# Alexander-H-Liu/End-to-end-ASR-Pytorch

Measured on AMD Instinct MI355X. Metric: audio frames/sec training (LAS+CTC, LibriSpeech 80-mel), higher is better.
Workload: dtype f32; 1 GPU; cfg3: {"B": 32, "T": 1600, "D": 80, "V": 5000, "L": 64}; global_batch=32, parallelism=dp1

## Files before the change

end-to-end-asr-pytorch_amd/_lib.py:

```python
import ctypes
import os

_HERE = os.path.dirname(os.path.abspath(__file__))
LIB_PATH = os.path.join(_HERE, "csrc", "libasrk.so")

c_int, c_i64, c_f32, c_vp, c_sz = (ctypes.c_int, ctypes.c_int64, ctypes.c_float, ctypes.c_void_p,
                                   ctypes.c_size_t)
c_f64 = ctypes.c_double

SIGNATURES = {
    "asrk_version": (c_int, []),
    "asrk_strerror": (ctypes.c_char_p, [c_int]),
    "asrk_init": (c_int, [c_int]),
    "asrk_profile_enable": (None, [c_int]),
    "asrk_profile_families": (None, [ctypes.c_uint]),
    "asrk_profile_reset": (None, []),
    "asrk_profile_get": (c_int, [c_int, ctypes.POINTER(ctypes.c_double), ctypes.POINTER(c_i64)]),
    "asrk_profile_get_work": (c_int, [c_int, ctypes.POINTER(ctypes.c_double)]),
    "asrk_gemm_f32": (c_int, [c_int, c_int, c_int, c_int, c_int, c_f32, c_vp, c_int, c_vp, c_int,
                              c_f32, c_vp, c_int, c_vp, c_vp, c_int, c_int, c_vp, c_sz, c_vp]),
    "asrk_gemm_ws_bytes": (c_sz, [c_int, c_int, c_int, c_int]),
    "asrk_gemm_takes_split": (c_int, [c_int, c_int, c_int, c_int]),
    "asrk_split_panel_bytes": (ctypes.c_size_t, [c_int, c_int, c_int]),
    "asrk_split_panel_f32": (c_int, [c_vp, c_int, c_int, c_int, c_int, c_vp, c_int, c_vp]),
    "asrk_gemm_panels_f32": (c_int, [c_int, c_int, c_int, c_f32, c_vp, c_int, c_int, c_int, c_int,
                                     c_vp, c_int, c_int, c_int, c_int, c_f32, c_vp, c_int, c_vp, c_vp, c_int, c_vp]),
    "asrk_gemm_panels_splitk_ws_bytes": (c_sz, [c_int, c_int, c_int]),
    "asrk_gemm_panels_splitk_f32": (c_int, [c_int, c_int, c_int, c_f32, c_vp, c_int, c_int, c_int, c_int,
                                            c_vp, c_int, c_int, c_int, c_int, c_f32, c_vp, c_int, c_vp, c_vp, c_int,
                                            c_vp, c_sz, c_int, c_vp]),
    "asrk_copy3d_f32": (c_int, [c_vp, c_vp, c_int, c_int, c_int, c_i64, c_i64, c_i64, c_i64, c_int,
                                c_vp]),
    "asrk_colsum_f32": (c_int, [c_vp, c_int, c_int, c_int, c_vp, c_int, c_vp]),
    "asrk_tanh_fwd_f32": (c_int, [c_vp, c_vp, c_i64, c_vp]),
    "asrk_tanh_bwd_f32": (c_int, [c_vp, c_vp, c_vp, c_i64, c_vp]),
    "asrk_log_softmax_fwd_f32": (c_int, [c_vp, c_vp, c_int, c_int, c_int, c_vp]),
    "asrk_log_softmax_bwd_f32": (c_int, [c_vp, c_vp, c_vp, c_int, c_int, c_int, c_vp]),
    "asrk_cross_entropy_fwd_f32": (c_int, [c_vp, c_int, c_int, c_int, c_vp, c_int, c_vp, c_vp, c_vp]),
    "asrk_cross_entropy_bwd_f32": (c_int, [c_vp, c_int, c_int, c_int, c_vp, c_int, c_vp, c_vp, c_vp,
                                           c_vp]),
    "asrk_ctc_prefix_score_f32": (c_int, [c_vp, c_vp, c_vp, c_vp, c_vp, c_vp, c_vp, c_int, c_int, c_int,
                                          c_int, c_int, c_int, c_f32, c_vp]),
    "asrk_ctc_prefix_score_multi_f32": (c_int, [c_vp, c_vp, c_vp, c_vp, c_vp, c_vp, c_vp, c_vp, c_vp, c_int, c_int,
                                                c_int, c_int, c_int, c_int, c_int, c_f32, c_vp]),
    "asrk_ctc_prefix_beam_ws_bytes": (c_sz, [c_int, c_int]),
    "asrk_ctc_prefix_beam_ws_offsets": (c_int, [c_int, c_int, c_int] + [ctypes.POINTER(c_i64)] * 6),
    "asrk_ctc_prefix_beam_f32": (c_int, [c_vp, c_int, c_int, c_vp, c_int, c_int, c_vp, c_f32, c_int, c_int, c_int,
                                         c_int, c_int, c_vp, c_sz, c_vp]),
    "asrk_ctc_prefix_beam_multi_ws_bytes": (c_sz, [c_int, c_int, c_int, ctypes.POINTER(c_sz)]),
    "asrk_ctc_prefix_beam_multi_f32": (c_int, [c_vp, c_i64, c_int, c_int, c_int, c_vp, c_int, c_int, c_vp, c_f32,
                                               c_vp, c_vp, c_int, c_vp, c_vp, c_vp, c_vp, c_sz, c_vp]),
    "asrk_fbank_frames_f32": (c_int, [c_vp, c_i64, c_vp, c_vp, c_int, c_int, c_int, c_int, c_f32, c_int,
                                      c_vp]),
    "asrk_power_spectrum_f32": (c_int, [c_vp, c_vp, c_i64, c_int, c_vp]),
    "asrk_log_floor_f32": (c_int, [c_vp, c_i64, c_f32, c_vp]),
    "asrk_delta_f32": (c_int, [c_vp, c_vp, c_vp, c_int, c_int, c_int, c_int, c_vp]),
    "asrk_cmvn_f32": (c_int, [c_vp, c_vp, c_int, c_int, c_f32, c_vp]),
    "asrk_transpose_f32": (c_int, [c_vp, c_vp, c_int, c_int, c_vp]),
    "asrk_fbank_frames_batch_f32": (c_int, [c_vp, c_int, c_i64, c_vp, c_vp, c_int, c_int, c_vp, c_vp, c_int, c_int,
                                            c_int, c_f32, c_f32, c_int, c_vp]),
    "asrk_delta_cmvn_batch_f32": (c_int, [c_vp, c_vp, c_int, c_int, c_vp, c_int, c_int, c_int, c_f32, c_vp, c_int,
                                          c_vp]),
    "asrk_fbank_logmel_batch_f32": (c_int, [c_vp, c_int, c_i64, c_vp, c_vp, c_int, c_int, c_vp, c_vp, c_vp, c_vp, c_vp,
                                            c_int, c_int, c_vp, c_int, c_int, c_int, c_f32, c_f32, c_int, c_f32, c_vp]),
    "asrk_spec_augment_f32": (c_int, [c_vp, c_vp, c_int, c_int, c_int, c_int, c_int, c_vp, c_vp, c_int, c_int, c_f32,
                                      c_vp]),
    "asrk_lstm_ws_bytes": (c_sz, []),
    "asrk_lstm_xchg_bytes": (c_sz, [c_int, c_int, c_int, c_int, c_int, c_int]),
    "asrk_lstm_plan_workgroups": (c_int, [c_int, c_int, c_int, c_int, c_int, c_int]),
    "asrk_lstm_rec_fwd_f32": (c_int, [c_vp, c_vp, c_vp, c_vp, c_vp, c_int, c_int, c_int, c_int,
                                      c_vp, c_int, c_vp, c_int, c_vp]),
    "asrk_lstm_rec_bwd_f32": (c_int, [c_vp, c_vp, c_vp, c_vp, c_vp, c_int, c_int, c_int, c_int,
                                      c_vp, c_int, c_vp, c_vp, c_int, c_vp]),
    "asrk_lstm_rec_fwd_pyr_f32": (c_int, [c_vp, c_vp, c_vp, c_vp, c_vp, c_int, c_int, c_int, c_int,
                                          c_vp, c_int, c_vp, c_vp, c_int, c_int, c_int, c_vp]),
    "asrk_lstm_rec_fwd_len_f32": (c_int, [c_vp, c_vp, c_vp, c_vp, c_vp, c_vp, c_int, c_int, c_int, c_int,
                                          c_vp, c_int, c_vp, c_vp, c_int, c_int, c_int, c_vp]),
    "asrk_lstm_rec_bwd_pyr_f32": (c_int, [c_vp, c_vp, c_vp, c_vp, c_vp, c_int, c_int, c_int, c_int,
                                          c_vp, c_int, c_vp, c_vp, c_int, c_int, c_int, c_vp]),
    "asrk_lstm_plan_is_bf": (c_int, [c_int, c_int, c_int, c_int, c_int, c_int]),
    "asrk_lstm_rec_fwd_pyr_panel_f32": (c_int, [c_vp, c_vp, c_vp, c_vp, c_vp, c_int, c_int, c_int, c_int,
                                                c_vp, c_int, c_vp, c_vp, c_int, c_int, c_vp, c_int, c_vp]),
    "asrk_lstm_rec_bwd_pyr_panel_f32": (c_int, [c_vp, c_vp, c_vp, c_vp, c_vp, c_int, c_int, c_int, c_int,
                                                c_vp, c_int, c_vp, c_vp, c_int, c_int, c_vp, c_vp, c_int, c_vp]),
    "asrk_gru_rec_fwd_f32": (c_int, [c_vp, c_vp, c_vp, c_vp, c_int, c_int, c_int, c_int,
                                     c_vp, c_int, c_vp, c_vp, c_int, c_int, c_int, c_vp]),
    "asrk_gru_rec_bwd_f32": (c_int, [c_vp, c_vp, c_vp, c_vp, c_vp, c_int, c_int, c_int, c_int,
                                     c_vp, c_int, c_vp, c_vp, c_int, c_int, c_int, c_vp]),
    "asrk_lstm_check_error": (c_int, [c_vp, c_vp]),
    "asrk_loc_conv_fwd_f32": (c_int, [c_vp, c_vp, c_vp, c_int, c_int, c_int, c_int, c_int, c_vp]),
    "asrk_loc_conv_bwd_f32": (c_int, [c_vp, c_vp, c_vp, c_vp, c_vp, c_int, c_int, c_int, c_int, c_int,
                                      c_vp]),
    "asrk_attn_energy_fwd_f32": (c_int, [c_int, c_vp, c_vp, c_vp, c_vp, c_vp, c_vp, c_vp, c_vp, c_vp,
                                         c_int, c_int, c_int, c_int, c_int, c_f32, c_vp]),
    "asrk_attn_energy_bwd_f32": (c_int, [c_int, c_vp, c_vp, c_vp, c_vp, c_vp, c_vp, c_vp, c_vp, c_vp,
                                         c_vp, c_vp, c_vp, c_vp, c_vp, c_int, c_int, c_int, c_int,
                                         c_int, c_f32, c_vp]),
    "asrk_attn_context_fwd_f32": (c_int, [c_vp, c_vp, c_vp, c_int, c_int, c_int, c_i64, c_vp]),
    "asrk_attn_context_bwd_f32": (c_int, [c_vp, c_vp, c_vp, c_int, c_int, c_int, c_i64, c_vp]),
    "asrk_lstm_cell_fwd_f32": (c_int, [c_vp, c_vp, c_vp, c_vp, c_int, c_int, c_vp]),
    "asrk_lstm_cell_bwd_f32": (c_int, [c_vp, c_vp, c_vp, c_vp, c_vp, c_vp, c_int, c_int, c_vp]),
    "asrk_gru_cell_fwd_f32": (c_int, [c_vp, c_vp, c_i64, c_i64, c_vp, c_i64, c_vp, c_i64, c_int, c_int, c_vp]),
    "asrk_gru_cell_bwd_f32": (c_int, [c_vp, c_vp, c_i64, c_i64, c_vp, c_i64, c_vp, c_i64, c_vp, c_vp, c_i64,
                                      c_int, c_int, c_vp]),
    "asrk_embedding_fwd_f32": (c_int, [c_vp, c_vp, c_vp, c_i64, c_int, c_int, c_vp]),
    "asrk_embedding_bwd_f32": (c_int, [c_vp, c_vp, c_vp, c_i64, c_int, c_int, c_vp]),
    "asrk_layer_norm_fwd_f32": (c_int, [c_vp, c_vp, c_vp, c_vp, c_vp, c_vp, c_int, c_int, c_f32, c_vp]),
    "asrk_layer_norm_bwd_f32": (c_int, [c_vp, c_vp, c_vp, c_vp, c_vp, c_vp, c_vp, c_vp, c_int, c_int,
                                        c_vp]),
    "asrk_dropout_f32": (c_int, [c_vp, c_vp, c_i64, c_f32, ctypes.c_uint64, ctypes.c_uint64, c_vp]),
    "asrk_adadelta_step_f32": (c_int, [c_vp, c_vp, c_vp, c_vp, c_i64, c_f64, c_f64, c_f64, c_vp, c_vp]),
    "asrk_adadelta_multi_f32": (c_int, [c_int, c_vp, c_vp, c_vp, c_vp, c_vp, c_f64, c_f64, c_f64, c_vp, c_vp]),
    "asrk_adam_multi_f32": (c_int, [c_int, c_vp, c_vp, c_vp, c_vp, c_vp, c_f64, c_f64, c_f64, c_f64, c_i64,
                                    c_vp, c_vp]),
    "asrk_adam_step_f32": (c_int, [c_vp, c_vp, c_vp, c_vp, c_i64, c_f64, c_f64, c_f64, c_f64, c_i64, c_vp,
                                   c_vp]),
    "asrk_token_crop_i64": (c_int, [c_vp, c_i64, c_int, c_int, c_i64, c_i64, c_int, c_vp, c_i64, c_vp, c_vp]),
    "asrk_edit_distance_i64": (c_int, [c_vp, c_i64, c_vp, c_vp, c_i64, c_vp, c_int, c_int, c_vp, c_vp]),
    "asrk_grad_norm_ws_bytes": (c_sz, [c_int, c_vp]),
    "asrk_grad_norm_multi_f32": (c_int, [c_int, c_vp, c_vp, c_f32, c_vp, c_vp, c_vp, c_sz, c_vp]),
    "asrk_fill_f32": (c_int, [c_vp, c_i64, c_f32, c_vp]),
    "asrk_topk_f32": (c_int, [c_vp, c_int, c_int, c_int, c_int, c_vp, c_vp, c_vp]),
    "asrk_beam_select_f32": (c_int, [c_vp] * 4 + [c_int] * 6 + [c_vp] * 19 + [c_vp]),
    "asrk_gather_rows_multi_f32": (c_int, [c_int, c_vp, c_vp, c_vp, c_vp, c_vp, c_vp, c_vp, c_int, c_vp]),
    "asrk_conv_out_size": (c_int, [c_int, c_int, c_int, c_int]),
    "asrk_im2col_f32": (c_int, [c_vp, c_vp] + [c_int] * 10 + [c_i64] * 4 + [c_vp]),
    "asrk_im2col_ld_f32": (c_int, [c_vp, c_vp] + [c_int] * 11 + [c_i64] * 4 + [c_vp]),
    "asrk_col2im_f32": (c_int, [c_vp, c_vp] + [c_int] * 10 + [c_i64] * 4 + [c_vp]),
    "asrk_im2col_cl_f32": (c_int, [c_vp, c_vp] + [c_int] * 10 + [c_i64] * 4 + [c_vp]),
    "asrk_col2im_cl_f32": (c_int, [c_vp, c_vp] + [c_int] * 10 + [c_i64] * 4 + [c_vp]),
    "asrk_conv_weight_reorder_f32": (c_int, [c_vp, c_vp, c_int, c_int, c_int, c_int, c_vp]),
    "asrk_conv3x3_supported": (c_int, [c_int] * 4),
    "asrk_conv3x3_weight_f32": (c_int, [c_vp, c_vp, c_int, c_int, c_int, c_vp]),
    "asrk_conv3x3_f32": (c_int, [c_vp] * 5 + [c_int] * 6 + [c_vp]),
    "asrk_conv3x3_wgrad_ws_bytes": (c_sz, [c_int] * 5),
    "asrk_conv3x3_wgrad_f32": (c_int, [c_vp] * 5 + [c_int] * 5 + [c_vp, c_sz, c_vp]),
    "asrk_conv3x3_first_supported": (c_int, [c_int] * 4),
    "asrk_conv3x3_first_f32": (c_int, [c_vp] * 4 + [c_int] * 5 + [c_i64] * 4 + [c_int, c_vp]),
    "asrk_conv3x3_len_f32": (c_int, [c_vp] * 5 + [c_int] * 6 + [c_vp]),
    "asrk_conv3x3_first_len_f32": (c_int, [c_vp] * 5 + [c_int] * 5 + [c_i64] * 4 + [c_int, c_vp]),
    "asrk_im2col_ld_len_f32": (c_int, [c_vp] * 3 + [c_int] * 11 + [c_i64] * 4 + [c_vp]),
    "asrk_im2col_cl_len_f32": (c_int, [c_vp] * 3 + [c_int] * 10 + [c_i64] * 4 + [c_vp]),
    "asrk_conv_zero_tail_f32": (c_int, [c_vp, c_vp, c_int, c_int, c_i64, c_vp]),
    "asrk_conv3x3_first_wgrad_ws_bytes": (c_sz, [c_int] * 5),
    "asrk_conv3x3_first_wgrad_f32": (c_int, [c_vp] * 5 + [c_int] * 5 + [c_i64] * 4 + [c_vp, c_sz, c_vp]),
    "asrk_relu_fwd_f32": (c_int, [c_vp, c_i64, c_vp]),
    "asrk_relu_bwd_f32": (c_int, [c_vp, c_vp, c_vp, c_i64, c_vp]),
    "asrk_maxpool2x2_fwd_f32": (c_int, [c_vp, c_vp, c_vp] + [c_int] * 4 + [c_i64] * 4 + [c_vp]),
    "asrk_maxpool2x2_bwd_f32": (c_int, [c_vp, c_vp, c_vp] + [c_int] * 4 + [c_i64] * 4 + [c_vp]),
    "asrk_speller_plan": (c_int, [c_vp, ctypes.POINTER(c_int), ctypes.POINTER(c_int)]),
    "asrk_speller_plan_info": (c_int, [c_vp, ctypes.POINTER(c_int)]),
    "asrk_speller_fwd_f32": (c_int, [c_vp, c_vp]),
    "asrk_speller_bwd_f32": (c_int, [c_vp, c_vp, c_vp]),
    "asrk_speller_step_f32": (c_int, [c_vp, c_int, c_vp, c_i64, c_vp, c_vp]),
    "asrk_speller_dvalue_f32": (c_int, [c_vp, c_i64, c_i64, c_vp, c_i64, c_i64, c_vp, c_int, c_int, c_int,
                                        c_int, c_vp]),
    "asrk_joint_score_f32": (c_int, [c_vp, c_vp, c_vp, c_vp, c_vp, c_vp, c_int, c_int, c_int, c_f64, c_f64,
                                     c_f64, c_vp]),
    "asrk_lstm_cell_fused_f32": (c_int, [c_vp, c_i64, c_int, c_vp, c_vp, c_vp, c_vp, c_vp, c_vp, c_vp, c_vp, c_int,
                                         c_int, c_vp]),
    "asrk_transpose_ld_f32": (c_int, [c_vp, c_i64, c_vp, c_i64, c_int, c_int, c_vp]),
    "asrk_flac_info": (c_int, [ctypes.c_char_p, ctypes.POINTER(c_int), ctypes.POINTER(c_int), ctypes.POINTER(c_int),
                               ctypes.POINTER(c_i64), c_vp]),
    "asrk_flac_decode_i32": (c_int, [ctypes.c_char_p, c_vp, c_i64, ctypes.POINTER(c_i64)]),
    "asrk_ctc_loss_fwd_f32": (c_int, [c_vp, c_i64, c_i64, c_int, c_int, c_int, c_vp, c_i64, c_int,
                                      c_vp, c_vp, c_int, c_vp, c_vp, c_vp, c_vp, c_vp]),
    "asrk_ctc_loss_bwd_f32": (c_int, [c_vp, c_i64, c_i64, c_int, c_int, c_int, c_vp, c_i64, c_int,
                                      c_vp, c_vp, c_int, c_vp, c_vp, c_vp, c_vp, c_vp, c_vp, c_i64,
                                      c_i64, c_vp]),
    "asrk_ctc_align_ws_bytes": (c_sz, [c_int, c_int, c_int, c_int]),
    "asrk_ctc_align_f32": (c_int, [c_vp, c_i64, c_i64, c_int, c_int, c_int, c_vp, c_i64, c_int, c_vp, c_vp, c_int,
                                   c_int, c_vp, c_vp, c_vp, c_vp, c_vp, c_vp, c_sz, c_vp]),
}

_lib = None


class AsrkError(RuntimeError):
    pass


def load():
    global _lib
    if _lib is not None:
        return _lib
    if not os.path.exists(LIB_PATH):
        raise AsrkError(
            "libasrk.so not found at %s - build it with `python __graft_entry__.py` "
            "(hipcc --offload-arch=gfx950). There is no CPU fallback for the product path." % LIB_PATH)
    try:
        import torch
    except ImportError:
        pass
    lib = ctypes.CDLL(LIB_PATH)
    for name, (res, args) in SIGNATURES.items():
        fn = getattr(lib, name)
        fn.restype = res
        fn.argtypes = args
    _lib = lib
    return lib


def strerror(rc):
    return load().asrk_strerror(int(rc)).decode()


def check(rc, what=""):
    if rc != 0:
        raise AsrkError("%s failed: %s (rc=%d)" % (what or "asrk call", strerror(rc), rc))
```

end-to-end-asr-pytorch_amd/csrc/core.cpp:

```cpp
#include "common.h"
#include "knobs.h"
#include <cstdlib>
#include <mutex>
#include <vector>

namespace {
struct DevInfo {
    int cu_count = 0;
    int lds_per_cu = 0;
    bool ok = false;
};
DevInfo g_dev[64];

struct ProfRec {
    hipEvent_t a, b;
    int id;
};
bool g_prof_on = false;
std::vector<ProfRec> g_pending;
double g_total_ms[PROF_NUM];
int64_t g_launches[PROF_NUM];
std::mutex g_mu;
hipEvent_t g_cur[PROF_NUM];
}

namespace {
AsrkKnobs g_knobs;
std::once_flag g_knobs_once;
int env_int(const char *name) {
    const char *e = getenv(name);
    return e ? atoi(e) : AsrkKnobs::UNSET;
}
int env_present(const char *name) { return getenv(name) ? 1 : AsrkKnobs::UNSET; }
void read_knobs() {
    AsrkKnobs &k = g_knobs;
    k.gemm_noskinny = env_present("ASRK_GEMM_NOSKINNY");
    k.skinny_sk = env_int("ASRK_SKINNY_SK");
    k.gemm_dbg = env_int("ASRK_GEMM_DBG");
    k.gemm_nofast = env_present("ASRK_GEMM_NOFAST");
    k.split_w256 = env_int("ASRK_SPLIT_W256");
    k.split_tail = env_int("ASRK_SPLIT_TAIL");
    k.fwd_mt = env_int("ASRK_FWD_MT");
    k.fwd_nt = env_int("ASRK_FWD_NT");
    k.rec_bf_mt4 = env_int("ASRK_REC_BF_MT4");
    k.bwd_ub = env_int("ASRK_BWD_UB");
    k.bwd_nt = env_int("ASRK_BWD_NT");
    k.fwd_poll = env_int("ASRK_FWD_POLL");
    k.fwd_presleep = env_int("ASRK_FWD_PRESLEEP");
    k.bwd_poll = env_int("ASRK_BWD_POLL");
    k.bwd_presleep = env_int("ASRK_BWD_PRESLEEP");
    k.dbg_noload = env_present("ASRK_DBG_NOLOAD");
    k.deterministic = env_int("ASRK_DETERMINISTIC");
}
}

const AsrkKnobs &asrk_knobs_() {
    std::call_once(g_knobs_once, read_knobs);
    return g_knobs;
}

extern "C" int asrk_version(void) { return 200; }

extern "C" const char *asrk_strerror(int rc) {
    switch (rc) {
        case ASRK_OK: return "ok";
        case ASRK_EINVAL: return "asrk: invalid argument";
        case ASRK_ESHAPE: return "asrk: shape not supported by the persistent gfx950 kernels";
        case ASRK_EWORKSPACE: return "asrk: workspace too small";
        case ASRK_EDEVICE: return "asrk: device lacks the CUs/LDS the persistent kernel needs";
        case ASRK_ETIMEOUT: return "asrk: in-kernel grid synchronisation timed out";
        default: break;
    }
    if (rc > 0) return hipGetErrorString((hipError_t)rc);
    return "asrk: unknown error";
}

extern "C" int asrk_init(int device) {
    if (device < 0 || device >= 64) return ASRK_EINVAL;
    (void)asrk_knobs_();
    if (!g_dev[device].ok) {
        hipDeviceProp_t prop;
        hipError_t e = hipGetDeviceProperties(&prop, device);
        if (e != hipSuccess) return (int)e > 0 ? -(1000 + (int)e) : ASRK_EDEVICE;
        g_dev[device].cu_count = prop.multiProcessorCount;
        g_dev[device].lds_per_cu = (int)prop.maxSharedMemoryPerMultiProcessor;
        g_dev[device].ok = true;
    }
    return g_dev[device].cu_count;
}

extern "C" int asrk_cu_count_(void) {
    int dev = 0;
    if (hipGetDevice(&dev) != hipSuccess) return 0;
    if (dev < 0 || dev >= 64) return 0;
    if (!g_dev[dev].ok) {
        if (asrk_init(dev) <= 0) return 0;
    }
    return g_dev[dev].cu_count;
}

static double g_work[PROF_NUM] = {0};

static unsigned g_prof_mask = 0xffffffffu;
extern "C" void asrk_profile_enable(int on) { g_prof_on = on != 0; }
extern "C" void asrk_profile_families(unsigned mask) { g_prof_mask = mask; }
static inline bool prof_live(int id) { return g_prof_on && id >= 0 && id < PROF_NUM && ((g_prof_mask >> id) & 1u); }

extern "C" void asrk_profile_reset(void) {
    std::lock_guard<std::mutex> lk(g_mu);
    for (auto &r : g_pending) {
        hipEventDestroy(r.a);
        hipEventDestroy(r.b);
    }
    g_pending.clear();
    for (int i = 0; i < PROF_NUM; ++i) {
        g_total_ms[i] = 0.0;
        g_launches[i] = 0;
        g_work[i] = 0.0;
    }
}

extern "C" void asrk_prof_work_(int id, double flops) {
    if (prof_live(id)) g_work[id] += flops;
}
extern "C" int asrk_profile_get_work(int id, double *flops) {
    if (id < 0 || id >= PROF_NUM || !flops) return ASRK_EINVAL;
    *flops = g_work[id];
    return ASRK_OK;
}

extern "C" void asrk_prof_begin_(int id, hipStream_t s) {
    if (!prof_live(id)) return;
    hipEvent_t a;
    if (hipEventCreate(&a) != hipSuccess) return;
    hipEventRecord(a, s);
    g_cur[id] = a;
}

extern "C" void asrk_prof_end_(int id, hipStream_t s) {
    if (!prof_live(id)) return;
    hipEvent_t b;
    if (hipEventCreate(&b) != hipSuccess) return;
    hipEventRecord(b, s);
    std::lock_guard<std::mutex> lk(g_mu);
    g_pending.push_back({g_cur[id], b, id});
}

extern "C" void asrk_prof_launches_(int id, int64_t n) {
    if (!prof_live(id)) return;
    std::lock_guard<std::mutex> lk(g_mu);
    g_launches[id] += n;
}

extern "C" int asrk_profile_get(int id, double *total_ms, int64_t *launches) {
    if (id < 0 || id >= PROF_NUM) return ASRK_EINVAL;
    std::lock_guard<std::mutex> lk(g_mu);
    for (auto &r : g_pending) {
        hipEventSynchronize(r.b);
        float ms = 0.f;
        if (hipEventElapsedTime(&ms, r.a, r.b) == hipSuccess) {
            g_total_ms[r.id] += ms;
            g_launches[r.id] += 1;
        }
        hipEventDestroy(r.a);
        hipEventDestroy(r.b);
    }
    g_pending.clear();
    if (total_ms) *total_ms = g_total_ms[id];
    if (launches) *launches = g_launches[id];
    return ASRK_OK;
}
```

end-to-end-asr-pytorch_amd/csrc/knobs.h:

```cpp
#pragma once

struct AsrkKnobs {
    static constexpr int UNSET = -0x7fffffff;
    int gemm_noskinny;
    int skinny_sk;
    int gemm_dbg;
    int gemm_nofast;
    int split_w256;
    int split_tail;
    int fwd_mt, fwd_nt;
    int rec_bf_mt4;
    int bwd_ub, bwd_nt;
    int fwd_poll, fwd_presleep;
    int bwd_poll, bwd_presleep;
    int dbg_noload;
    int deterministic;

    int get(int v, int dflt) const { return v == UNSET ? dflt : v; }
    bool is_set(int v) const { return v != UNSET; }
};

const AsrkKnobs &asrk_knobs_();
```

end-to-end-asr-pytorch_amd/csrc/speller.hip:

```cpp
#include "common.h"
#include "knobs.h"
#include <cstdlib>

namespace {

__device__ __forceinline__ float tanh_fast(float x) {
    const float e = __expf(2.f * x);
    return 1.f - __fdividef(2.f, e + 1.f);
}
__device__ __forceinline__ float sigmoid_fast(float x) { return __fdividef(1.f, 1.f + __expf(-x)); }

unsigned long long *g_sp_dbg = nullptr;
int g_sp_dbg_slots = 0;
inline unsigned long long *sp_slot(int step, int kid) {
    const long i = (long)step * 16 + kid;
    return (g_sp_dbg && i < g_sp_dbg_slots) ? g_sp_dbg + i * 16 : nullptr;
}
#define SP_STAMP(ph)                                                                                     \
    do {                                                                                                 \
        if (p.stamps && threadIdx.x == 0) {                                                              \
            if (blockIdx.x == 0 && blockIdx.y == 0) p.stamps[ph] = __builtin_readcyclecounter();         \
            else if (blockIdx.x == gridDim.x - 1 && blockIdx.y == gridDim.y - 1 && ((ph) == 0 || (ph) == 9)) \
                p.stamps[(ph) == 0 ? 12 : 13] = __builtin_readcyclecounter();                            \
        }                                                                                                \
    } while (0)

constexpr int SK_THREADS = 512, SK_WAVES = 8, SK_CH = 32;

struct SkSeg {
    const float *x;
    const float *w;
    long ldx, ldw;
    int klen;
    unsigned xbytes, wbytes;
};

enum { EPI_STORE = 0, EPI_TANH_BIAS = 1, EPI_LSTM_FWD = 2, EPI_LSTM_BWD = 3 };

struct SkArgs {
    SkSeg seg[3];
    int nseg, M, R, H;
    unsigned long long *stamps;
    float *out;
    long ldo;
    const float *bias;
    const float *pre, *b0, *b1;
    const float *c_prev;
    float *c_new, *h_new, *gates;
    float *h_bm;
    long h_bm_ld;
    const float *add0, *add1;
    long ld0, ld1;
    float *dG;
    const float *bc_prev, *bc_new;
    float *dc;
    int dc_valid;
    int gru;
};

template <int VEC>
__device__ __forceinline__ void load8(const float *row, int k, int klen, bool valid, float (&v)[8]) {
    if (VEC && valid && k + 8 <= klen) {
        const f32x4 a = *reinterpret_cast<const f32x4 *>(row + k);
        const f32x4 b = *reinterpret_cast<const f32x4 *>(row + k + 4);
        v[0] = a[0]; v[1] = a[1]; v[2] = a[2]; v[3] = a[3];
        v[4] = b[0]; v[5] = b[1]; v[6] = b[2]; v[7] = b[3];
        return;
    }
#pragma unroll
    for (int j = 0; j < 8; ++j) v[j] = (valid && k + j < klen) ? row[k + j] : 0.f;
}

template <int MT, int EPI, int VEC>
__global__ __launch_bounds__(SK_THREADS) void skinny_kernel(SkArgs p) {
    __shared__ float red[SK_WAVES][MT][4][64];
    const int tid = threadIdx.x, lane = tid & 63;
    const int wave = __builtin_amdgcn_readfirstlane(tid >> 6);
    const int slot = lane & 15, g = lane >> 4;
    SP_STAMP(0);
    int r;
    bool rvalid;
    if (EPI == EPI_LSTM_FWD) {
        const int u = blockIdx.x * 4 + (slot >> 2);
        r = (slot & 3) * p.H + u;
        rvalid = u < p.H;
    } else {
        r = blockIdx.x * 16 + slot;
        rvalid = r < p.R;
    }
    f32x4 acc[MT][2];
#pragma unroll
    for (int mt = 0; mt < MT; ++mt) acc[mt][0] = acc[mt][1] = f32x4{0.f, 0.f, 0.f, 0.f};

    float e_in[EPI == EPI_LSTM_BWD ? 36 : 13];
    const bool e_thr = tid < MT * 64;
    const int e_m = (tid >> 6) * 16 + (lane & 15);
    if (e_thr && e_m < p.M) {
        if (EPI == EPI_STORE || EPI == EPI_TANH_BIAS) {
#pragma unroll
            for (int q = 0; q < 4; ++q) {
                const int rr = blockIdx.x * 16 + (lane >> 4) * 4 + q;
                e_in[q] = (rr < p.R && p.bias) ? p.bias[rr] : 0.f;
            }
        } else if (EPI == EPI_LSTM_FWD) {
            const int u = blockIdx.x * 4 + (lane >> 4), H = p.H;
            if (u < H) {
#pragma unroll
                for (int q = 0; q < 4; ++q) {
                    const long col = (long)q * H + u;
                    e_in[q] = p.pre ? p.pre[(long)e_m * 4 * H + col] : 0.f;
                    e_in[4 + q] = p.b0 ? p.b0[col] : 0.f;
                    e_in[8 + q] = p.b1 ? p.b1[col] : 0.f;
                }
                e_in[12] = p.c_prev[(long)e_m * H + u];
            }
        } else {
            const int H = p.H;
#pragma unroll
            for (int q = 0; q < 4; ++q) {
                const int j = blockIdx.x * 16 + (lane >> 4) * 4 + q;
                if (j >= H) continue;
                const float *gr = p.dG + (long)e_m * 4 * H + j;
                e_in[q * 9 + 0] = p.add0 ? p.add0[(long)e_m * p.ld0 + j] : 0.f;
                e_in[q * 9 + 1] = p.add1 ? p.add1[(long)e_m * p.ld1 + j] : 0.f;
                e_in[q * 9 + 2] = gr[0];
                e_in[q * 9 + 3] = gr[H];
                e_in[q * 9 + 4] = gr[2 * (long)H];
                e_in[q * 9 + 5] = gr[3 * (long)H];
                e_in[q * 9 + 6] = p.bc_new[(long)e_m * H + j];
                e_in[q * 9 + 7] = p.dc_valid ? p.dc[(long)e_m * H + j] : 0.f;
                e_in[q * 9 + 8] = p.bc_prev[(long)e_m * H + j];
            }
        }
    }

    if (VEC == 2) {
        extern __shared__ __attribute__((aligned(16))) float stage_all[];
        constexpr int SROWS = 16 + MT * 16, SLD = 36, NX = 2 * MT;
        constexpr int NB = (MT <= 2 && EPI != EPI_LSTM_BWD) ? 4 : 2;
        constexpr unsigned OOB = 0x80000000u;
        float *st = stage_all + wave * SROWS * SLD;
        const int lrow = lane >> 3, lk = (lane & 7) * 4;
        const int n0 = (p.seg[0].klen + SK_CH - 1) / SK_CH;
        const int n1 = p.nseg > 1 ? (p.seg[1].klen + SK_CH - 1) / SK_CH : 0;
        const int n2 = p.nseg > 2 ? (p.seg[2].klen + SK_CH - 1) / SK_CH : 0;
        const int ntot = n0 + n1 + n2;
        const int mych = ntot > wave ? (ntot - wave + SK_WAVES - 1) / SK_WAVES : 0;
        auto sg = [](unsigned v) __attribute__((always_inline)) { return (unsigned)__builtin_amdgcn_readfirstlane((int)v); };
        auto sg64 = [sg](const float *ptr) __attribute__((always_inline)) {
            const unsigned long long a = reinterpret_cast<unsigned long long>(ptr);
            return ((unsigned long long)sg((unsigned)(a >> 32)) << 32) | sg((unsigned)a);
        };
        const bool has1 = p.nseg > 1, has2 = p.nseg > 2;
        const unsigned long long wp0 = sg64(p.seg[0].w), wp1 = sg64(p.seg[1].w), wp2 = sg64(p.seg[2].w);
        const unsigned long long xp0 = sg64(p.seg[0].x), xp1 = sg64(p.seg[1].x), xp2 = sg64(p.seg[2].x);
        const unsigned wb0 = sg(p.seg[0].wbytes), wb1 = sg(has1 ? p.seg[1].wbytes : 0u), wb2 = sg(has2 ? p.seg[2].wbytes : 0u);
        const unsigned xb0 = sg(p.seg[0].xbytes), xb1 = sg(has1 ? p.seg[1].xbytes : 0u), xb2 = sg(has2 ? p.seg[2].xbytes : 0u);
        const unsigned ldw0 = sg((unsigned)p.seg[0].ldw * 4u), ldw1 = sg((unsigned)p.seg[1].ldw * 4u), ldw2 = sg((unsigned)p.seg[2].ldw * 4u);
        const unsigned ldx0 = sg((unsigned)p.seg[0].ldx * 4u), ldx1 = sg((unsigned)p.seg[1].ldx * 4u), ldx2 = sg((unsigned)p.seg[2].ldx * 4u);
        const unsigned kl0 = sg((unsigned)p.seg[0].klen * 4u), kl1 = sg(has1 ? (unsigned)p.seg[1].klen * 4u : 0u),
                       kl2 = sg(has2 ? (unsigned)p.seg[2].klen * 4u : 0u);
        const int Mrows = (int)sg((unsigned)p.M);
        unsigned wrow[2];
        bool wok[2];
#pragma unroll
        for (int h = 0; h < 2; ++h) {
            const int sl = lrow + 8 * h;
            if (EPI == EPI_LSTM_FWD) {
                const int u = blockIdx.x * 4 + (sl >> 2);
                wrow[h] = (unsigned)((sl & 3) * p.H + u);
                wok[h] = u < p.H;
            } else {
                wrow[h] = (unsigned)(blockIdx.x * 16 + sl);
                wok[h] = (int)wrow[h] < p.R;
            }
        }
#define SK_ISSUE(i_, gw_, gx_)                                                                          \
    do {                                                                                                \
        const int c_ = wave + (i_) * SK_WAVES;                \
        const bool s1_ = c_ >= n0, s2_ = c_ >= n0 + n1;                                                 \
        const int base_ = s2_ ? n0 + n1 : (s1_ ? n0 : 0);                                               \
        const __amdgpu_buffer_rsrc_t rw_ = __builtin_amdgcn_make_buffer_rsrc(                           \
            reinterpret_cast<void *>(s2_ ? wp2 : (s1_ ? wp1 : wp0)), 0, (int)(s2_ ? wb2 : (s1_ ? wb1 : wb0)), 0x00020000); \
        const __amdgpu_buffer_rsrc_t rx_ = __builtin_amdgcn_make_buffer_rsrc(                           \
            reinterpret_cast<void *>(s2_ ? xp2 : (s1_ ? xp1 : xp0)), 0, (int)(s2_ ? xb2 : (s1_ ? xb1 : xb0)), 0x00020000); \
        const unsigned ldw_ = s2_ ? ldw2 : (s1_ ? ldw1 : ldw0), ldx_ = s2_ ? ldx2 : (s1_ ? ldx1 : ldx0); \
        const unsigned kl_ = s2_ ? kl2 : (s1_ ? kl1 : kl0);                                             \
        const unsigned kb_ = (unsigned)(c_ - base_) * (SK_CH * 4u) + (unsigned)lk * 4u;                 \
        const bool kin_ = kb_ < kl_;    \
        _Pragma("unroll") for (int h_ = 0; h_ < 2; ++h_) {                                              \
            const unsigned off_ = wrow[h_] * ldw_ + kb_;                                                \
            (gw_)[h_] = __builtin_amdgcn_raw_buffer_load_b128(rw_, (kin_ && wok[h_]) ? off_ : OOB, 0, 0); \
        }                                                                                               \
        _Pragma("unroll") for (int h_ = 0; h_ < NX; ++h_) {                                             \
            const unsigned m_ = (unsigned)(lrow + 8 * h_);                                              \
            const unsigned off_ = m_ * ldx_ + kb_;                                                      \
            (gx_)[h_] = __builtin_amdgcn_raw_buffer_load_b128(rx_, (kin_ && (int)m_ < Mrows) ? off_ : OOB, 0, 0); \
        }                                                                                               \
    } while (0)
        auto stage = [st, lrow, lk, slot, g](const u32x4 (&gw)[2], const u32x4 (&gx)[NX], f32x4 (&fw)[2], f32x4 (&fx)[MT][2]) __attribute__((always_inline)) {
            __builtin_amdgcn_wave_barrier();
#pragma unroll
            for (int h = 0; h < 2; ++h)
                *reinterpret_cast<u32x4 *>(st + (lrow + 8 * h) * SLD + lk) = gw[h];
#pragma unroll
            for (int h = 0; h < NX; ++h)
                *reinterpret_cast<u32x4 *>(st + (16 + lrow + 8 * h) * SLD + lk) = gx[h];
            __builtin_amdgcn_wave_barrier();
            fw[0] = *reinterpret_cast<const f32x4 *>(st + slot * SLD + 8 * g);
            fw[1] = *reinterpret_cast<const f32x4 *>(st + slot * SLD + 8 * g + 4);
#pragma unroll
            for (int mt = 0; mt < MT; ++mt) {
                fx[mt][0] = *reinterpret_cast<const f32x4 *>(st + (16 + mt * 16 + slot) * SLD + 8 * g);
                fx[mt][1] = *reinterpret_cast<const f32x4 *>(st + (16 + mt * 16 + slot) * SLD + 8 * g + 4);
            }
        };
        auto mfmas = [&acc](const f32x4 (&fw)[2], const f32x4 (&fx)[MT][2]) __attribute__((always_inline)) {
#pragma unroll
            for (int hh = 0; hh < 2; ++hh)
#pragma unroll
                for (int j = 0; j < 4; ++j)
#pragma unroll
                    for (int mt = 0; mt < MT; ++mt)
                        acc[mt][j & 1] = __builtin_amdgcn_mfma_f32_16x16x4f32(fw[hh][j], fx[mt][hh][j], acc[mt][j & 1], 0, 0, 0);
        };
        if (mych > 0) {
            u32x4 gw[NB][2], gx[NB][NX];
            f32x4 fw[2][2], fx[2][MT][2];
#pragma unroll
            for (int j = 0; j < NB; ++j) SK_ISSUE(j, gw[j], gx[j]);
            SP_STAMP(1);
            stage(gw[0], gx[0], fw[0], fx[0]);
            SP_STAMP(2);
            SK_ISSUE(NB, gw[0], gx[0]);
#define SK_STEP(u)                                                                                      \
    if (i0 + (u) >= mych) break;                                                                        \
    stage(gw[((u) + 1) % NB], gx[((u) + 1) % NB], fw[((u) + 1) & 1], fx[((u) + 1) & 1]);                \
    SK_ISSUE(i0 + (u) + 1 + NB, gw[((u) + 1) % NB], gx[((u) + 1) % NB]);                                \
    __builtin_amdgcn_sched_barrier(0);                                                                  \
    mfmas(fw[(u) & 1], fx[(u) & 1]);                                                                    \
    __builtin_amdgcn_sched_barrier(0);
            for (int i0 = 0; i0 < mych; i0 += NB) {
                SK_STEP(0)
                SK_STEP(1)
                if (NB > 2) {
                    SK_STEP(2)
                    SK_STEP(3)
                }
            }
#undef SK_STEP
#undef SK_ISSUE
        }
    } else {
    for (int s = 0; s < p.nseg; ++s) {
        const SkSeg sg = p.seg[s];
        const float *wrow = sg.w + (long)r * sg.ldw;
        const int nch = (sg.klen + SK_CH - 1) / SK_CH;
        for (int c = wave; c < nch; c += 2 * SK_WAVES) {
            const int k0 = c * SK_CH + 8 * g, k1 = k0 + SK_WAVES * SK_CH;
            float w0[8], w1[8], x0[MT][8], x1[MT][8];
            load8<VEC>(wrow, k0, sg.klen, rvalid, w0);
            load8<VEC>(wrow, k1, sg.klen, rvalid, w1);
#pragma unroll
            for (int mt = 0; mt < MT; ++mt) {
                const int m = mt * 16 + slot;
                load8<VEC>(sg.x + (long)m * sg.ldx, k0, sg.klen, m < p.M, x0[mt]);
                load8<VEC>(sg.x + (long)m * sg.ldx, k1, sg.klen, m < p.M, x1[mt]);
            }
#pragma unroll
            for (int j = 0; j < 8; ++j)
#pragma unroll
                for (int mt = 0; mt < MT; ++mt)
                    acc[mt][j & 1] = __builtin_amdgcn_mfma_f32_16x16x4f32(w0[j], x0[mt][j], acc[mt][j & 1], 0, 0, 0);
#pragma unroll
            for (int j = 0; j < 8; ++j)
#pragma unroll
                for (int mt = 0; mt < MT; ++mt)
                    acc[mt][j & 1] = __builtin_amdgcn_mfma_f32_16x16x4f32(w1[j], x1[mt][j], acc[mt][j & 1], 0, 0, 0);
        }
    }
    }
#pragma unroll
    for (int mt = 0; mt < MT; ++mt)
#pragma unroll
        for (int v = 0; v < 4; ++v) red[wave][mt][v][lane] = acc[mt][0][v] + acc[mt][1][v];
    SP_STAMP(3);
    __syncthreads();
    SP_STAMP(4);
    if (tid >= MT * 64) return;
    const int mt = tid >> 6;
    float v[4];
#pragma unroll
    for (int q = 0; q < 4; ++q) {
        float s = 0.f;
#pragma unroll
        for (int w = 0; w < SK_WAVES; ++w) s += red[w][mt][q][lane];
        v[q] = s;
    }
    const int m = mt * 16 + (lane & 15);
    if (m >= p.M) return;
    if (EPI == EPI_STORE || EPI == EPI_TANH_BIAS) {
#pragma unroll
        for (int q = 0; q < 4; ++q) {
            const int rr = blockIdx.x * 16 + (lane >> 4) * 4 + q;
            if (rr < p.R) {
                float y = v[q] + e_in[q];
                if (EPI == EPI_TANH_BIAS) y = tanh_fast(y);
                p.out[(long)m * p.ldo + rr] = y;
            }
        }
    } else if (EPI == EPI_LSTM_FWD) {
        const int u = blockIdx.x * 4 + (lane >> 4);
        if (u >= p.H) return;
        const int H = p.H;
        float a[4];
#pragma unroll
        for (int q = 0; q < 4; ++q) {
            const long col = (long)q * H + u;
            (void)col;
            a[q] = v[q] + e_in[q] + e_in[4 + q] + e_in[8 + q];
        }
        float hn;
        if (p.gru) {
            const float gr_ = sigmoid_fast(a[0]), gz = sigmoid_fast(a[1]), gn = tanh_fast(a[2] + gr_ * a[3]);
            hn = (1.f - gz) * gn + gz * e_in[12];
            if (p.gates) {
                float *gr = p.gates + (long)m * 4 * H + u;
                gr[0] = gr_; gr[H] = gz; gr[2 * (long)H] = gn; gr[3 * (long)H] = a[3];
            }
        } else {
            const float gi = sigmoid_fast(a[0]), gf = sigmoid_fast(a[1]), gg = tanh_fast(a[2]),
                        go = sigmoid_fast(a[3]);
            const float cn = gf * e_in[12] + gi * gg;
            hn = go * tanh_fast(cn);
            if (p.gates) {
                float *gr = p.gates + (long)m * 4 * H + u;
                gr[0] = gi; gr[H] = gf; gr[2 * (long)H] = gg; gr[3 * (long)H] = go;
            }
            p.c_new[(long)m * H + u] = cn;
        }
        p.h_new[(long)m * H + u] = hn;
        if (p.h_bm) p.h_bm[(long)m * p.h_bm_ld + u] = hn;
    } else {
        const int H = p.H;
#pragma unroll
        for (int q = 0; q < 4; ++q) {
            const int j = blockIdx.x * 16 + (lane >> 4) * 4 + q;
            if (j >= H) continue;
            float *gr = p.dG + (long)m * 4 * H + j;
            if (p.gru) {
                const float dh = v[q] + e_in[q * 9 + 0] + e_in[q * 9 + 1] + e_in[q * 9 + 7];
                const float r_ = e_in[q * 9 + 2], z_ = e_in[q * 9 + 3], n_ = e_in[q * 9 + 4], nh = e_in[q * 9 + 5];
                const float dnp = dh * (1.f - z_) * (1.f - n_ * n_);
                gr[0] = dnp * nh * r_ * (1.f - r_);
                gr[H] = dh * (e_in[q * 9 + 8] - n_) * z_ * (1.f - z_);
                gr[2 * (long)H] = dnp;
                gr[3 * (long)H] = dnp * r_;
                p.dc[(long)m * H + j] = dh * z_;
                continue;
            }
            const float dh = v[q] + e_in[q * 9 + 0] + e_in[q * 9 + 1];
            const float gi = e_in[q * 9 + 2], gf = e_in[q * 9 + 3], gg = e_in[q * 9 + 4], go = e_in[q * 9 + 5];
            const float tc = tanh_fast(e_in[q * 9 + 6]);
            const float dct = dh * go * (1.f - tc * tc) + e_in[q * 9 + 7];
            gr[0] = dct * gg * gi * (1.f - gi);
            gr[H] = dct * e_in[q * 9 + 8] * gf * (1.f - gf);
            gr[2 * (long)H] = dct * gi * (1.f - gg * gg);
            gr[3 * (long)H] = dh * tc * go * (1.f - go);
            p.dc[(long)m * H + j] = dct * gf;
        }
    }
    SP_STAMP(9);
}

inline bool al16(const void *q) { return (reinterpret_cast<uintptr_t>(q) & 15) == 0; }

template <int EPI>
int launch_skinny(const SkArgs &a, hipStream_t s) {
    if (a.M <= 0) return ASRK_OK;
    bool vec = true;
    for (int i = 0; i < a.nseg; ++i)
        vec = vec && al16(a.seg[i].x) && al16(a.seg[i].w) && a.seg[i].ldx % 4 == 0 && a.seg[i].ldw % 4 == 0 &&
              a.seg[i].klen % 4 == 0;
    const int blocks = (EPI == EPI_LSTM_FWD) ? asrk_div_up(a.H, 4) : asrk_div_up(a.R, 16);
    if (blocks <= 0) return ASRK_OK;
    for (int m0 = 0; m0 < a.M; m0 += 64) {
        SkArgs p = a;
        p.M = a.M - m0 < 64 ? a.M - m0 : 64;
        for (int i = 0; i < p.nseg; ++i) p.seg[i].x += (long)m0 * p.seg[i].ldx;
        bool small = true;
        const long wrows = (EPI == EPI_LSTM_FWD) ? 4L * p.H : (long)p.R;
        for (int i = 0; i < p.nseg; ++i) {
            const long wb = ((wrows - 1) * p.seg[i].ldw + p.seg[i].klen) * 4L;
            const long xb = ((long)(p.M - 1) * p.seg[i].ldx + p.seg[i].klen) * 4L;
            small = small && wb < (1L << 31) && xb < (1L << 31);
            p.seg[i].wbytes = (unsigned)wb;
            p.seg[i].xbytes = (unsigned)xb;
        }
        for (int i = p.nseg; i < 3; ++i) p.seg[i] = SkSeg{nullptr, nullptr, 0, 0, 0, 0u, 0u};
        if (p.out) p.out += (long)m0 * p.ldo;
        const long H4 = 4L * p.H, H1 = p.H;
        if (p.pre) p.pre += m0 * H4;
        if (p.c_prev) p.c_prev += m0 * H1;
        if (p.c_new) p.c_new += m0 * H1;
        if (p.h_new) p.h_new += m0 * H1;
        if (p.gates) p.gates += m0 * H4;
        if (p.h_bm) p.h_bm += (long)m0 * p.h_bm_ld;
        if (p.add0) p.add0 += (long)m0 * p.ld0;
        if (p.add1) p.add1 += (long)m0 * p.ld1;
        if (p.dG) p.dG += m0 * H4;
        if (p.bc_prev) p.bc_prev += m0 * H1;
        if (p.bc_new) p.bc_new += m0 * H1;
        if (p.dc) p.dc += m0 * H1;
        const int mt = p.M <= 16 ? 1 : (p.M <= 32 ? 2 : 4);
#define SK_LAUNCH_V(MT_, V_)                                                                        \
    do {                                                                                            \
        static AsrkLdsLatch latch_;                                                                 \
        const size_t lds = (size_t)SK_WAVES * (16 + MT_ * 16) * 36 * sizeof(float);                 \
        hipError_t e_ = asrk_max_lds_once(latch_, reinterpret_cast<const void *>(&skinny_kernel<MT_, EPI, V_>), (int)lds); \
        if (e_ != hipSuccess) return (int)e_;                                                       \
        hipLaunchKernelGGL((skinny_kernel<MT_, EPI, V_>), dim3(blocks), dim3(SK_THREADS), lds, s, p); \
    } while (0)
#define SK_LAUNCH(MT_)                                                                              \
    do {                                                                                            \
        if (vec && small) SK_LAUNCH_V(MT_, 2);                                                      \
        else hipLaunchKernelGGL((skinny_kernel<MT_, EPI, 0>), dim3(blocks), dim3(SK_THREADS), 0, s, p); \
    } while (0)
        if (mt == 1) SK_LAUNCH(1);
        else if (mt == 2) SK_LAUNCH(2);
        else SK_LAUNCH(4);
#undef SK_LAUNCH
#undef SK_LAUNCH_V
    }
    ASRK_LAUNCH_CHECK();
    return ASRK_OK;
}

__device__ __forceinline__ float maskf(float v, bool c) {
    return __uint_as_float(__float_as_uint(v) & (0u - (unsigned)c));
}
constexpr int RED_RS = 65;

struct AttArgs {
    const float *key, *q, *prev, *Wc, *Wp, *we, *be;
    const int64_t *lens;
    float *conv, *e;
    long prev_ld;
    int Te, A, K, ks, tpb, KP;
    float inv_temp;
    int kvb;
    const int *row_mem;
    unsigned long long *stamps;
};

__global__ __launch_bounds__(512) void attend_energy_kernel(AttArgs p) {
    extern __shared__ float sm[];
    const int b = blockIdx.x, t0 = blockIdx.y * p.tpb;
    const int nt = min(p.tpb, p.Te - t0);
    const int tid = threadIdx.x, lane = tid & 63, wave = __builtin_amdgcn_readfirstlane(tid >> 6);
    const int A = p.A, K = p.K, KP = p.KP, KW = 2 * p.ks + 1;
    float *s_prev = sm;
    float *s_wc = s_prev + p.tpb + 2 * p.ks;
    float *s_wp = s_wc + K * KW;
    float *s_c = s_wp + A * KP;
    float *s_q = s_c + p.tpb * K;
    float *s_we = s_q + A;
    const int bk = p.row_mem ? p.row_mem[b] : b * p.kvb;
    const int len = min((int)p.lens[bk], p.Te);
    for (int i = tid; i < nt + 2 * p.ks; i += 512) {
        const int t = t0 + i - p.ks;
        s_prev[i] = (t >= 0 && t < p.Te) ? p.prev[(long)b * p.prev_ld + t] : 0.f;
    }
    for (int i = tid; i < K * KW; i += 512) s_wc[i] = p.Wc[i];
    for (int i = tid; i < A * K; i += 512) {
        const int a = i / K, k = i - a * K;
        s_wp[a * KP + k] = p.Wp[i];
    }
    for (int i = tid; i < A; i += 512) {
        s_q[i] = p.q[(long)b * A + i];
        s_we[i] = p.we[i];
    }
    __syncthreads();
    for (int i = tid; i < nt * K; i += 512) {
        const int k = i / nt, tl = i - k * nt;
        const float *wr = s_wc + k * KW, *pr = s_prev + tl;
        float acc = 0.f;
        for (int j = 0; j < KW; ++j) acc += pr[j] * wr[j];
        s_c[tl * K + k] = acc;
        p.conv[((long)b * p.Te + t0 + tl) * K + k] = acc;
    }
    __syncthreads();
    const float be = p.be[0];
    constexpr int FRM = 4, NAM = 5;
    if (nt <= 8 * FRM && A <= 64 * NAM) {
        float kreg[FRM][NAM];
#pragma unroll
        for (int f = 0; f < FRM; ++f) {
            const int tl = wave + 8 * f, t = t0 + tl;
            const bool live = tl < nt && t < len;
            const float *kr = p.key + ((long)bk * p.Te + (live ? t : 0)) * A;
#pragma unroll
            for (int i = 0; i < NAM; ++i) {
                const int a = lane + 64 * i;
                kreg[f][i] = (live && a < A) ? kr[a] : 0.f;
            }
        }
#pragma unroll
        for (int f = 0; f < FRM; ++f) {
            const int tl = wave + 8 * f, t = t0 + tl;
            if (tl >= nt) break;
            if (t >= len) {
                if (lane == 0) p.e[(long)b * p.Te + t] = -INFINITY;
                continue;
            }
            const float *cr = s_c + tl * K;
            float part = 0.f;
#pragma unroll
            for (int i = 0; i < NAM; ++i) {
                const int a = lane + 64 * i;
                if (a < A) {
                    float u = 0.f;
                    for (int k = 0; k < K; ++k) u += s_wp[a * KP + k] * cr[k];
                    part += s_we[a] * tanh_fast(kreg[f][i] + s_q[a] + tanh_fast(u));
                }
            }
            part = wave_sum(part);
            if (lane == 0) p.e[(long)b * p.Te + t] = (part + be) * p.inv_temp;
        }
        return;
    }
    for (int tl = wave; tl < nt; tl += 8) {
        const int t = t0 + tl;
        if (t >= len) {
            if (lane == 0) p.e[(long)b * p.Te + t] = -INFINITY;
            continue;
        }
        const float *kr = p.key + ((long)bk * p.Te + t) * A;
        const float *cr = s_c + tl * K;
        float part = 0.f;
        for (int a = lane; a < A; a += 64) {
            float u = 0.f;
            for (int k = 0; k < K; ++k) u += s_wp[a * KP + k] * cr[k];
            part += s_we[a] * tanh_fast(kr[a] + s_q[a] + tanh_fast(u));
        }
        part = wave_sum(part);
        if (lane == 0) p.e[(long)b * p.Te + t] = (part + be) * p.inv_temp;
    }
}

__device__ __forceinline__ unsigned kdiv_of(int K) { return K > 1 ? 0xFFFFFFFFu / (unsigned)K + 1u : 0u; }
__device__ __forceinline__ int div_k(int i, unsigned kdiv) { return kdiv ? (int)__umulhi((unsigned)i, kdiv) : i; }

constexpr int AE_FR = 4, AE_NW = 4, AE_WPN = 8;
template <int NA, int KM>
__global__ __launch_bounds__(512) void attend_energy_kernel2(AttArgs p) {
    extern __shared__ float sm[];
    const int b = blockIdx.x, t0 = blockIdx.y * p.tpb;
    const int nt = min(p.tpb, p.Te - t0);
    const int tid = threadIdx.x, lane = tid & 63, wave = __builtin_amdgcn_readfirstlane(tid >> 6);
    const int A = p.A, K = p.K, KP = p.KP, Te = p.Te, ks = p.ks, KW = 2 * ks + 1, AK = A * K;
    float *s_wp = sm;
    float *red_w = s_wp + A * KP + wave * (16 * RED_RS + 16);
    float *cb_w = red_w + 16 * RED_RS;
    const unsigned kdiv = kdiv_of(K);
    const int bk = p.row_mem ? p.row_mem[b] : b * p.kvb;
    SP_STAMP(0);

    const int len_raw = (int)p.lens[bk];
    float kreg[AE_FR][NA], pw[AE_FR][AE_NW];
#pragma unroll
    for (int f = 0; f < AE_FR; ++f) {
// ... 191 lines not shown
        }
    }
#pragma unroll
    for (int j = 0; j < 4; ++j) s_part[wave * 256 + lane * 4 + j] = acc[j];
    SP_STAMP(3);
    __syncthreads();
    if (tid < 256) {
        const int d = blockIdx.y * 256 + tid;
        if (d < Dv) {
            float s = 0.f;
#pragma unroll
            for (int w = 0; w < 8; ++w) s += s_part[w * 256 + tid];
            p.ctx[(long)b * p.ctx_ld + d] = s;
        }
    }
    SP_STAMP(9);
}

constexpr int CG_MAXR = 4;
__global__ __launch_bounds__(512) void softmax_context_group_kernel(CtxArgs p, int RG) {
    extern __shared__ float sm[];
    const int g = blockIdx.x, tid = threadIdx.x, lane = tid & 63;
    const int wave = __builtin_amdgcn_readfirstlane(tid >> 6);
    const int Te = p.Te, Dv = p.Dv, TeP = (Te + 3) & ~3;
    const int b0 = g * RG;
    const int mem = p.row_mem ? p.row_mem[b0] : b0 * p.kvb;
    const int d0 = blockIdx.y * 256 + lane * 4;
    const float *vb = p.value + (long)mem * Te * Dv + min(d0, Dv - 4);
    int nr = 0;
    int rows[CG_MAXR];
#pragma unroll
    for (int j = 0; j < CG_MAXR; ++j) {
        rows[j] = wave + 8 * j;
        if (rows[j] < RG) nr = j + 1;
    }
#pragma unroll
    for (int j = 0; j < CG_MAXR; ++j) {
        if (j >= nr) break;
        const float *er = p.e + (long)(b0 + rows[j]) * Te;
        float *sa = sm + rows[j] * TeP;
        float mx = -INFINITY;
        for (int t = lane; t < Te; t += 64) mx = fmaxf(mx, er[t]);
        mx = wave_max(mx);
        float sum = 0.f;
        for (int t = lane; t < Te; t += 64) {
            const float x = __expf(er[t] - mx);
            sa[t] = x;
            sum += x;
        }
        sum = wave_sum(sum);
        const float inv = 1.f / sum;
        for (int t = lane; t < Te; t += 64) {
            const float a = sa[t] * inv;
            sa[t] = a;
            if (blockIdx.y == 0) p.attn[(long)(b0 + rows[j]) * p.attn_ld + t] = a;
        }
    }
    __builtin_amdgcn_wave_barrier();
    f32x4 acc[CG_MAXR];
#pragma unroll
    for (int j = 0; j < CG_MAXR; ++j) acc[j] = f32x4{0.f, 0.f, 0.f, 0.f};
    int t = 0;
    for (; t + 7 < Te; t += 8) {
        f32x4 v[8];
#pragma unroll
        for (int i = 0; i < 8; ++i) v[i] = *reinterpret_cast<const f32x4 *>(vb + (long)(t + i) * Dv);
#pragma unroll
        for (int j = 0; j < CG_MAXR; ++j) {
            if (j >= nr) break;
            const float *sa = sm + rows[j] * TeP + t;
#pragma unroll
            for (int i = 0; i < 8; ++i) {
                const float a = sa[i];
                acc[j][0] += a * v[i][0]; acc[j][1] += a * v[i][1]; acc[j][2] += a * v[i][2]; acc[j][3] += a * v[i][3];
            }
        }
    }
    for (; t < Te; ++t) {
        const f32x4 v = *reinterpret_cast<const f32x4 *>(vb + (long)t * Dv);
#pragma unroll
        for (int j = 0; j < CG_MAXR; ++j) {
            if (j >= nr) break;
            const float a = sm[rows[j] * TeP + t];
            acc[j][0] += a * v[0]; acc[j][1] += a * v[1]; acc[j][2] += a * v[2]; acc[j][3] += a * v[3];
        }
    }
    if (d0 < Dv) {
#pragma unroll
        for (int j = 0; j < CG_MAXR; ++j) {
            if (j >= nr) break;
            *reinterpret_cast<f32x4 *>(p.ctx + (long)(b0 + rows[j]) * p.ctx_ld + d0) = acc[j];
        }
    }
}

struct DattnArgs {
    const float *dctx, *value, *extra0, *extra1;
    const int64_t *lens;
    float *dattn;
    long dctx_ld, e0_ld, e1_ld;
    int Te, Dv;
    unsigned long long *stamps;
    int lens_div;
};

constexpr int DAT_ND = 8;
template <bool VEC>
__global__ __launch_bounds__(512) void dattn_kernel(DattnArgs p) {
    const int b = blockIdx.x, lane = threadIdx.x & 63;
    const int t = blockIdx.y * 8 + __builtin_amdgcn_readfirstlane(threadIdx.x >> 6);
    if (t >= p.Te) return;
    SP_STAMP(0);
    const int len_raw = (int)p.lens[b / (p.lens_div + 1)];
    const float *v = p.value + ((long)b * p.Te + t) * p.Dv;
    const float *g = p.dctx + (long)b * p.dctx_ld;
    float acc = 0.f;
    const float x0 = p.extra0 ? p.extra0[(long)b * p.e0_ld + t] : 0.f;
    const float x1 = p.extra1 ? p.extra1[(long)b * p.e1_ld + t] : 0.f;
    if (VEC) {
        f32x4 a[DAT_ND], c[DAT_ND];
#pragma unroll
        for (int i = 0; i < DAT_ND; ++i) {
            const int d = min(lane * 4 + 256 * i, p.Dv - 4);
            a[i] = *reinterpret_cast<const f32x4 *>(v + d);
            c[i] = *reinterpret_cast<const f32x4 *>(g + d);
        }
#pragma unroll
        for (int i = 0; i < DAT_ND; ++i)
            acc += maskf(a[i][0] * c[i][0] + a[i][1] * c[i][1] + a[i][2] * c[i][2] + a[i][3] * c[i][3],
                         lane * 4 + 256 * i < p.Dv);
        for (int d = lane * 4 + 256 * DAT_ND; d < p.Dv; d += 256) {
            const f32x4 aa = *reinterpret_cast<const f32x4 *>(v + d);
            const f32x4 cc = *reinterpret_cast<const f32x4 *>(g + d);
            acc += aa[0] * cc[0] + aa[1] * cc[1] + aa[2] * cc[2] + aa[3] * cc[3];
        }
    } else {
        for (int d = lane; d < p.Dv; d += 64) acc += v[d] * g[d];
    }
    SP_STAMP(1);
    acc = wave_sum(acc);
    SP_STAMP(2);
    if (lane == 0) p.dattn[(long)b * p.Te + t] = t < min(len_raw, p.Te) ? acc + x0 + x1 : 0.f;
    SP_STAMP(9);
}

struct EbArgs {
    const float *key, *q, *conv, *Wp, *we, *attn, *dattn;
    const int64_t *lens;
    float *dkey, *dconv, *dq_part, *dwe_part, *dWp_part, *dbe_part;
    long attn_ld;
    int Te, A, K, tpb, KP;
    float inv_temp;
    unsigned long long *stamps;
};

__global__ __launch_bounds__(512) void energy_bwd_kernel2(EbArgs p) {
    extern __shared__ float sm[];
    __shared__ float s_red[8];
    const int b = blockIdx.x, chunk = blockIdx.y, TC = gridDim.y, t0 = chunk * p.tpb;
    const int nt = min(p.tpb, p.Te - t0);
    const int tid = threadIdx.x, lane = tid & 63, wave = __builtin_amdgcn_readfirstlane(tid >> 6);
    const int A = p.A, K = p.K, KP = p.KP, Te = p.Te;
    float *s_q = sm;
    float *s_we = s_q + A;
    float *s_dwe = s_we + A;
    float *s_wp = s_dwe + A;
    float *s_c = s_wp + A * KP;
    float *s_de = s_c + p.tpb * K;
    float *s_du = s_de + p.tpb;
    float *s_dz = s_du + p.tpb * A;
    float *s_ez = s_dz + p.tpb * A;
    const int len = min((int)p.lens[b], Te);
    for (int i = tid; i < A; i += 512) {
        s_q[i] = p.q[(long)b * A + i];
        s_we[i] = p.we[i];
        s_dwe[i] = 0.f;
    }
    for (int i = tid; i < A * K; i += 512) {
        const int a = i / K, k = i - a * K;
        s_wp[a * KP + k] = p.Wp[i];
    }
    for (int i = tid; i < nt * K; i += 512) s_c[i] = p.conv[((long)b * Te + t0) * K + i];
    const float *ar = p.attn + (long)b * p.attn_ld, *dr = p.dattn + (long)b * Te;
    float dot = 0.f;
    for (int t = tid; t < len; t += 512) dot += ar[t] * dr[t];
    dot = wave_sum(dot);
    if (lane == 0) s_red[wave] = dot;
    __syncthreads();
    dot = 0.f;
#pragma unroll
    for (int w = 0; w < 8; ++w) dot += s_red[w];
    for (int i = tid; i < nt; i += 512) {
        const int t = t0 + i;
        s_de[i] = (t < len) ? ar[t] * (dr[t] - dot) * p.inv_temp : 0.f;
    }
    __syncthreads();
    const long blk = (long)b * TC + chunk;
    constexpr int WPN = 8;
    float old_wp[WPN], old_we = 0.f;
    const bool wp_regs = A * K <= 512 * WPN;
#pragma unroll
    for (int r = 0; r < WPN; ++r) {
        const int i = tid + 512 * r;
        old_wp[r] = (wp_regs && i < A * K) ? p.dWp_part[blk * A * K + i] : 0.f;
    }
    if (tid < A) old_we = p.dwe_part[blk * A + tid];
    for (int base = tid; base < nt * A; base += 512 * 4) {
        int tl4[4], a4[4];
        long ki4[4];
        bool ok4[4], live4[4];
        float kv[4], dk[4];
#pragma unroll
        for (int u = 0; u < 4; ++u) {
            const int i = base + 512 * u;
            ok4[u] = i < nt * A;
            tl4[u] = ok4[u] ? i / A : 0;
            a4[u] = ok4[u] ? i - tl4[u] * A : 0;
            live4[u] = ok4[u] && (t0 + tl4[u] < len);
            ki4[u] = ((long)b * Te + t0 + tl4[u]) * A + a4[u];
            kv[u] = live4[u] ? p.key[ki4[u]] : 0.f;
            dk[u] = live4[u] ? p.dkey[ki4[u]] : 0.f;
        }
#pragma unroll
        for (int u = 0; u < 4; ++u) {
            if (!ok4[u]) continue;
            const int i = base + 512 * u, tl = tl4[u], a = a4[u];
            float dz = 0.f, du = 0.f, ez = 0.f;
            if (live4[u]) {
                const float de = s_de[tl];
                const float *cr = s_c + tl * K;
                float uu = 0.f;
                for (int k = 0; k < K; ++k) uu += s_wp[a * KP + k] * cr[k];
                const float loc = tanh_fast(uu);
                const float z = tanh_fast(kv[u] + s_q[a] + loc);
                dz = de * s_we[a] * (1.f - z * z);
                du = dz * (1.f - loc * loc);
                p.dkey[ki4[u]] = dk[u] + dz;
                ez = de * z;
            }
            s_dz[i] = dz;
            s_du[i] = du;
            s_ez[i] = ez;
        }
    }
    __syncthreads();
    for (int i = tid; i < nt * K; i += 512) {
        const int tl = i / K, k = i - tl * K;
        const float *dur = s_du + tl * A;
        float acc = 0.f;
        for (int a = 0; a < A; ++a) acc += dur[a] * s_wp[a * KP + k];
        p.dconv[((long)b * Te + t0 + tl) * K + k] = acc;
    }
    if (wp_regs) {
#pragma unroll
        for (int r = 0; r < WPN; ++r) {
            const int i = tid + 512 * r;
            if (i < A * K) {
                const int a = i / K, k = i - a * K;
                float acc = 0.f;
                for (int tl = 0; tl < nt; ++tl) acc += s_du[tl * A + a] * s_c[tl * K + k];
                p.dWp_part[blk * A * K + i] = old_wp[r] + acc;
            }
        }
    } else {
        for (int i = tid; i < A * K; i += 512) {
            const int a = i / K, k = i - a * K;
            float acc = 0.f;
            for (int tl = 0; tl < nt; ++tl) acc += s_du[tl * A + a] * s_c[tl * K + k];
            p.dWp_part[blk * A * K + i] += acc;
        }
    }
    for (int a = tid; a < A; a += 512) {
        float acc = 0.f, ew = 0.f;
        for (int tl = 0; tl < nt; ++tl) {
            acc += s_dz[tl * A + a];
            ew += s_ez[tl * A + a];
        }
        p.dq_part[blk * A + a] = acc;
        p.dwe_part[blk * A + a] = (a == tid ? old_we : p.dwe_part[blk * A + a]) + ew;
    }
    if (tid == 0) {
        float acc = 0.f;
        for (int tl = 0; tl < nt; ++tl) acc += s_de[tl];
        p.dbe_part[blk] += acc;
    }
}

constexpr int EB_FR = 4, EB_WPN = 8, EB_NTE = 2;
template <int NA, int KM>
__global__ __launch_bounds__(512) void energy_bwd_kernel3(EbArgs p) {
    extern __shared__ float sm[];
    __shared__ float s_red8[8], s_be8[8];
    constexpr int AP = 64 * NA;
    const int b = blockIdx.x, chunk = blockIdx.y, TC = gridDim.y, t0 = chunk * p.tpb;
    const int nt = min(p.tpb, p.Te - t0);
    const int tid = threadIdx.x, lane = tid & 63, wave = __builtin_amdgcn_readfirstlane(tid >> 6);
    const int A = p.A, K = p.K, KP = p.KP, Te = p.Te, AK = A * K;
    float *s_wp = sm;
    float *s_c = s_wp + A * KP;
    float *s_du = s_c + p.tpb * KM;
    float *s_red = s_du + p.tpb * AP;
    const long blk = (long)b * TC + chunk;
    const unsigned kdiv = kdiv_of(K);

    SP_STAMP(0);
    const int len_raw = (int)p.lens[b];
    float kv[EB_FR][NA], dk[EB_FR][NA];
#pragma unroll
    for (int f = 0; f < EB_FR; ++f) {
        const int t = min(t0 + wave + 8 * f, Te - 1);
        const long row = ((long)b * Te + t) * A;
#pragma unroll
        for (int j = 0; j < NA; ++j) {
            const long idx = row + min(lane + 64 * j, A - 1);
            kv[f][j] = p.key[idx];
            dk[f][j] = p.dkey[idx];
        }
    }
    const float *ar = p.attn + (long)b * p.attn_ld, *dr = p.dattn + (long)b * Te;
    float a_e[EB_NTE], d_e[EB_NTE], a_f[EB_FR], d_f[EB_FR];
#pragma unroll
    for (int e = 0; e < EB_NTE; ++e) {
        const int t = min(tid + 512 * e, Te - 1);
        a_e[e] = ar[t];
        d_e[e] = dr[t];
    }
#pragma unroll
    for (int f = 0; f < EB_FR; ++f) {
        const int t = min(t0 + wave + 8 * f, Te - 1);
        a_f[f] = ar[t];
        d_f[f] = dr[t];
    }
    float wpst[EB_WPN], old_wp[EB_WPN];
#pragma unroll
    for (int r = 0; r < EB_WPN; ++r) {
        const int i = min(tid + 512 * r, AK - 1);
        wpst[r] = p.Wp[i];
        old_wp[r] = p.dWp_part[blk * AK + i];
    }
    const float old_we = p.dwe_part[blk * A + min(tid, A - 1)];
    const float old_be = p.dbe_part[blk];
    float cst;
    {
        const int tl = tid / KM, k = tid - tl * KM;
        cst = maskf(p.conv[((long)b * Te + min(t0 + tl, Te - 1)) * K + min(k, K - 1)], tl < nt && k < K);
    }
    float qv[NA], wev[NA];
#pragma unroll
    for (int j = 0; j < NA; ++j) {
        const int a = lane + 64 * j, ac = min(a, A - 1);
        qv[j] = p.q[(long)b * A + ac];
        wev[j] = maskf(p.we[ac], a < A);
    }
    SP_STAMP(1);
    const int len = min(len_raw, Te);
    float dot = 0.f;
#pragma unroll
    for (int e = 0; e < EB_NTE; ++e) dot += maskf(a_e[e] * d_e[e], tid + 512 * e < len);
    dot = wave_sum(dot);
    if (lane == 0) s_red8[wave] = dot;
#pragma unroll
    for (int r = 0; r < EB_WPN; ++r) {
        const int i = tid + 512 * r;
        if (i < AK) {
            const int a = div_k(i, kdiv), k = i - a * K;
            s_wp[a * KP + k] = wpst[r];
        }
    }
    if (tid < p.tpb * KM) s_c[tid] = cst;
    __syncthreads();
    SP_STAMP(2);
    dot = 0.f;
#pragma unroll
    for (int w = 0; w < 8; ++w) dot += s_red8[w];
    float de_f[EB_FR], de_sum = 0.f;
#pragma unroll
    for (int f = 0; f < EB_FR; ++f) {
        const int tl = wave + 8 * f;
        de_f[f] = maskf(a_f[f] * (d_f[f] - dot) * p.inv_temp, tl < nt && t0 + tl < len);
        de_sum += de_f[f];
    }
    if (lane == 0) s_be8[wave] = de_sum;
    float wp[NA][KM];
#pragma unroll
    for (int j = 0; j < NA; ++j) {
        const int ac = min(lane + 64 * j, A - 1);
#pragma unroll
        for (int k = 0; k < KM; ++k) {
            const float v = s_wp[ac * KP + min(k, K - 1)];
            wp[j][k] = (lane + 64 * j < A && k < K) ? v : 0.f;
        }
    }

    SP_STAMP(3);
    float dq_acc[NA], dwe_acc[NA];
#pragma unroll
    for (int j = 0; j < NA; ++j) dq_acc[j] = dwe_acc[j] = 0.f;
    float *red_w = s_red + wave * 16 * RED_RS;
#pragma unroll
    for (int f = 0; f < EB_FR; ++f) {
        const int tl = wave + 8 * f, t = t0 + tl;
        if (tl >= nt) break;
        const bool live = t < len;
        const float de = de_f[f];
        float c[KM], pk[KM];
#pragma unroll
        for (int k = 0; k < KM; ++k) {
            c[k] = s_c[tl * KM + k];
            pk[k] = 0.f;
        }
#pragma unroll
        for (int j = 0; j < NA; ++j) {
            const int a = lane + 64 * j;
            float uu = 0.f;
#pragma unroll
            for (int k = 0; k < KM; ++k) uu += wp[j][k] * c[k];
            const float loc = tanh_fast(uu);
            const float z = tanh_fast(kv[f][j] + qv[j] + loc);
            const float dz = de * wev[j] * (1.f - z * z);
            const float du = dz * (1.f - loc * loc);
            if (live && a < A) p.dkey[((long)b * Te + t) * A + a] = dk[f][j] + dz;
            dq_acc[j] += dz;
            dwe_acc[j] += (a < A) ? de * z : 0.f;
            s_du[tl * AP + a] = du;
#pragma unroll
            for (int k = 0; k < KM; ++k) pk[k] += du * wp[j][k];
        }
        __builtin_amdgcn_wave_barrier();
#pragma unroll
        for (int k = 0; k < KM; ++k) red_w[k * RED_RS + lane] = pk[k];
        __builtin_amdgcn_wave_barrier();
        const int rk = lane & 15, part = lane >> 4;
        float sum = 0.f;
        if (rk < KM) {
#pragma unroll
            for (int i = 0; i < 16; ++i) sum += red_w[rk * RED_RS + part * 16 + i];
        }
        sum += __shfl_xor(sum, 16, 64);
        sum += __shfl_xor(sum, 32, 64);
        if (lane < K) p.dconv[((long)b * Te + t) * K + lane] = sum;
    }
    SP_STAMP(4);
    __syncthreads();
    SP_STAMP(5);

    float *s_x = s_red;
#pragma unroll
    for (int j = 0; j < NA; ++j) {
        s_x[(wave * 2 + 0) * AP + lane + 64 * j] = dq_acc[j];
        s_x[(wave * 2 + 1) * AP + lane + 64 * j] = dwe_acc[j];
    }
#pragma unroll
    for (int r = 0; r < EB_WPN; ++r) {
        const int i = tid + 512 * r;
        if (i < AK) {
            const int a = div_k(i, kdiv), k = i - a * K;
            float acc = 0.f;
            for (int tl = 0; tl < nt; ++tl) acc += s_du[tl * AP + a] * s_c[tl * KM + k];
            p.dWp_part[blk * AK + i] = old_wp[r] + acc;
        }
    }
    SP_STAMP(6);
    __syncthreads();
    if (tid < A) {
        float dq = 0.f, dwe = 0.f;
#pragma unroll
        for (int w = 0; w < 8; ++w) {
            dq += s_x[(w * 2 + 0) * AP + tid];
            dwe += s_x[(w * 2 + 1) * AP + tid];
        }
        p.dq_part[blk * A + tid] = dq;
        p.dwe_part[blk * A + tid] = old_we + dwe;
    }
    if (tid == 0) {
        float acc = 0.f;
#pragma unroll
        for (int w = 0; w < 8; ++w) acc += s_be8[w];
        p.dbe_part[blk] = old_be + acc;
    }
    SP_STAMP(9);
}

struct DotArgs {
    const float *key, *q, *attn, *dattn;
    const int64_t *lens;
    float *e, *dkey, *dq_part;
    long attn_ld;
    int Te, A, lens_div, tpb;
    float inv_temp;
};

__global__ __launch_bounds__(512) void dot_energy_kernel(DotArgs p) {
    const int r = blockIdx.x, lane = threadIdx.x & 63;
    const int t = blockIdx.y * 8 + __builtin_amdgcn_readfirstlane(threadIdx.x >> 6);
    if (t >= p.Te) return;
    const int len_raw = (int)p.lens[r / p.lens_div];
    const float *k = p.key + ((long)r * p.Te + t) * p.A, *q = p.q + (long)r * p.A;
    float acc = 0.f;
    for (int a = lane; a < p.A; a += 64) acc += k[a] * q[a];
    acc = wave_sum(acc);
    if (lane == 0) p.e[(long)r * p.Te + t] = t < min(len_raw, p.Te) ? acc * p.inv_temp : -INFINITY;
}

constexpr int DOT_NA = 8;
__global__ __launch_bounds__(512) void dot_energy_bwd_kernel(DotArgs p) {
    __shared__ float s_red8[8];
    __shared__ float s_dq[8][64 * DOT_NA];
    const int r = blockIdx.x, chunk = blockIdx.y, TC = gridDim.y, t0 = chunk * p.tpb;
    const int nt = min(p.tpb, p.Te - t0);
    const int tid = threadIdx.x, lane = tid & 63, wave = __builtin_amdgcn_readfirstlane(tid >> 6);
    const int A = p.A, Te = p.Te;
    const int len = min((int)p.lens[r / p.lens_div], Te);
    const float *ar = p.attn + (long)r * p.attn_ld, *dr = p.dattn + (long)r * Te;
    float dot = 0.f;
    for (int t = tid; t < len; t += 512) dot += ar[t] * dr[t];
    dot = wave_sum(dot);
    if (lane == 0) s_red8[wave] = dot;
    __syncthreads();
    dot = 0.f;
#pragma unroll
    for (int w = 0; w < 8; ++w) dot += s_red8[w];
    float qv[DOT_NA], dq[DOT_NA];
#pragma unroll
    for (int j = 0; j < DOT_NA; ++j) {
        const int a = lane + 64 * j;
        qv[j] = a < A ? p.q[(long)r * A + a] : 0.f;
        dq[j] = 0.f;
    }
    for (int tl = wave; tl < nt; tl += 8) {
        const int t = t0 + tl;
        if (t >= len) continue;
        const float de = ar[t] * (dr[t] - dot) * p.inv_temp;
        const long row = ((long)r * Te + t) * A;
#pragma unroll
        for (int j = 0; j < DOT_NA; ++j) {
            const int a = lane + 64 * j;
            if (a < A) {
                dq[j] += de * p.key[row + a];
                p.dkey[row + a] += de * qv[j];
            }
        }
    }
#pragma unroll
    for (int j = 0; j < DOT_NA; ++j) s_dq[wave][lane + 64 * j] = dq[j];
    __syncthreads();
    for (int a = tid; a < A; a += 512) {
        float acc = 0.f;
#pragma unroll
        for (int w = 0; w < 8; ++w) acc += s_dq[w][a];
        p.dq_part[((long)r * TC + chunk) * A + a] = acc;
    }
}

struct CbArgs {
    const float *dconv, *prev, *Wc, *dq_part, *q;
    float *dprev, *dWc_part, *dq_pre;
    long prev_ld;
    int Te, K, ks, TC, A, nT, want_dprev;
    unsigned long long *stamps;
    int dq_only;
};

__global__ __launch_bounds__(256) void conv_bwd_kernel(CbArgs p) {
    extern __shared__ float sm[];
    const int b = blockIdx.x, y = p.dq_only ? p.nT + p.K : blockIdx.y, tid = threadIdx.x;
    const int Te = p.Te, K = p.K, ks = p.ks, KW = 2 * ks + 1;
    SP_STAMP(0);
    if (y < p.nT) {
        if (!p.want_dprev) return;
        const int s0 = y * 64, span = 64 + 2 * ks;
        float *sd = sm, *part = sm + K * span;
        float *s_w = part + 256;
        for (int i = tid; i < span * K; i += 256) {
            const int o = i / K, k = i - o * K;
            const int t = s0 + o - ks;
            sd[k * span + o] = (t >= 0 && t < Te) ? p.dconv[((long)b * Te + t) * K + k] : 0.f;
        }
        for (int i = tid; i < K * KW; i += 256) s_w[i] = p.Wc[i];
        __syncthreads();
        const int sl = tid & 63, w = __builtin_amdgcn_readfirstlane(tid >> 6);
        float acc = 0.f;
        for (int k = w; k < K; k += 4) {
            const float *wr = s_w + k * KW;
            const float *col = sd + k * span + sl + 2 * ks;
            for (int j = 0; j < KW; ++j) acc += col[-j] * wr[j];
        }
        part[w * 64 + sl] = acc;
        __syncthreads();
        if (tid < 64 && s0 + tid < Te)
            p.dprev[(long)b * Te + s0 + tid] = (part[tid] + part[64 + tid]) + (part[128 + tid] + part[192 + tid]);
        SP_STAMP(9);
    } else if (y < p.nT + K) {
        const int k = y - p.nT;
        float *s_dc = sm, *s_pv = sm + Te;
        float old[4];
#pragma unroll
        for (int r = 0; r < 4; ++r) {
            const int j = tid + 256 * r;
            old[r] = j < KW ? p.dWc_part[((long)b * K + k) * KW + j] : 0.f;
        }
        for (int t = tid; t < Te; t += 256) s_dc[t] = p.dconv[((long)b * Te + t) * K + k];
        for (int i = tid; i < Te + 2 * ks; i += 256) {
            const int t = i - ks;
            s_pv[i] = (t >= 0 && t < Te) ? p.prev[(long)b * p.prev_ld + t] : 0.f;
        }
        __syncthreads();
#pragma unroll
        for (int r = 0; r < 4; ++r) {
            const int j = tid + 256 * r;
            if (j < KW) {
                const float *pv = s_pv + j;
                float acc = 0.f;
                for (int t = 0; t < Te; ++t) acc += s_dc[t] * pv[t];
                p.dWc_part[((long)b * K + k) * KW + j] = old[r] + acc;
            }
        }
        for (int j = tid + 1024; j < KW; j += 256) {
            const float *pv = s_pv + j;
            float acc = 0.f;
            for (int t = 0; t < Te; ++t) acc += s_dc[t] * pv[t];
            p.dWc_part[((long)b * K + k) * KW + j] += acc;
        }
    } else {
        for (int a = tid; a < p.A; a += 256) {
            float acc = 0.f;
            for (int c = 0; c < p.TC; ++c) acc += p.dq_part[((long)b * p.TC + c) * p.A + a];
            const float qv = p.q[(long)b * p.A + a];
            p.dq_pre[(long)b * p.A + a] = acc * (1.f - qv * qv);
        }
        SP_STAMP(9);
    }
}

constexpr int DV_LC = 64;
__global__ __launch_bounds__(256) void dvalue_kernel(const float *__restrict__ attn, long attn_ld,
                                                     long attn_step, const float *__restrict__ dxh,
                                                     long step_ld, long row_ld, float *__restrict__ dvalue,
                                                     int L, int Te, int Dv) {
    extern __shared__ float s_at[];
    const int b = blockIdx.x, d = blockIdx.y * 256 + threadIdx.x;
    for (int l0 = 0; l0 < L; l0 += DV_LC) {
        const int nl = min(DV_LC, L - l0);
        __syncthreads();
        for (int i = threadIdx.x; i < nl * Te; i += 256) {
            const int l = i / Te, t = i - l * Te;
            s_at[i] = attn[(long)b * attn_ld + (long)(l0 + l) * attn_step + t];
        }
        for (int i = nl * Te + threadIdx.x; i < DV_LC * Te; i += 256) s_at[i] = 0.f;
        __syncthreads();
        if (d < Dv) {
            float g[DV_LC];
#pragma unroll
            for (int l = 0; l < DV_LC; ++l)
                g[l] = l < nl ? dxh[(long)(l0 + l) * step_ld + (long)b * row_ld + d] : 0.f;
            float *out = dvalue + (long)b * Te * Dv + d;
            for (int t = 0; t < Te; ++t) {
                float acc = 0.f;
#pragma unroll
                for (int l = 0; l < DV_LC; ++l) acc += s_at[l * Te + t] * g[l];
                if (l0 == 0) out[(long)t * Dv] = acc;
                else out[(long)t * Dv] += acc;
            }
        }
    }
}

__global__ __launch_bounds__(256) void joint_score_kernel(const float *__restrict__ att,
                                                          const int64_t *__restrict__ cand,
                                                          const float *__restrict__ psi,
                                                          const float *__restrict__ prev_ctc,
                                                          const float *__restrict__ lm, float *__restrict__ out,
                                                          int V, int C, float wa, float w_ctc, float w_lm,
                                                          float logzero) {
    const int r = blockIdx.x;
    const float *a = att + (long)r * V;
    const float *l = lm ? lm + (long)r * V : nullptr;
    float *o = out + (long)r * V;
    const bool ctc = cand != nullptr;
    const float wz = w_ctc * logzero;
    for (int v = threadIdx.x; v < V; v += 256) {
        float x = a[v];
        if (ctc) x = (v == 0) ? logzero : wa * x + wz;
        if (l) x = x + w_lm * l[v];
        o[v] = x;
    }
    if (!ctc) return;
    __syncthreads();
    for (int c = threadIdx.x; c < C; c += 256) {
        const int v = (int)cand[(long)r * C + c];
        if (v <= 0 || v >= V) continue;
        float x = wa * a[v] + w_ctc * (psi[(long)r * C + c] - prev_ctc[r]);
        if (l) x = x + w_lm * l[v];
        o[v] = x;
    }
}

__global__ __launch_bounds__(256) void transpose_ld_kernel(const float *__restrict__ in, long ldi,
                                                           float *__restrict__ out, long ldo, int rows,
                                                           int cols) {
    __shared__ float tile[32][33];
    const int tx = threadIdx.x & 31, ty = threadIdx.x >> 5;
    const int c0 = blockIdx.x * 32, r0 = blockIdx.y * 32;
    for (int i = ty; i < 32; i += 8)
        if (r0 + i < rows && c0 + tx < cols) tile[i][tx] = in[(long)(r0 + i) * ldi + c0 + tx];
    __syncthreads();
    for (int i = ty; i < 32; i += 8)
        if (c0 + i < cols && r0 + tx < rows) out[(long)(c0 + i) * ldo + r0 + tx] = tile[tx][i];
}

int pick_tpb(int B, int Te, int A, int K, size_t fixed_floats, size_t per_frame_floats, size_t budget, int wg_target = 512) {
    int tc = asrk_div_up(wg_target, B > 0 ? B : 1);
    if (tc > asrk_div_up(Te, 8)) tc = asrk_div_up(Te, 8);
    if (tc < 1) tc = 1;
    int tpb = asrk_div_up(Te, tc);
    if (tpb > 8) tpb = (tpb + 7) / 8 * 8;
    while (tpb > 1 && (fixed_floats + per_frame_floats * tpb) * sizeof(float) > budget) tpb = (tpb + 1) / 2;
    if ((fixed_floats + per_frame_floats * tpb) * sizeof(float) > budget) return 0;
    return tpb;
}

constexpr size_t LDS_BUDGET = 150 * 1024;

struct Plan {
    int tpb_f, tc_f, tpb_b, tc_b, KP, nT;
    size_t lds_f, lds_b, lds_ctx, lds_cb;
    int eb3_na, eb3_km;
    size_t lds_b3;
    int ae2_na, ae2_km;
    size_t lds_f2;
};

int make_plan(const asrk_speller_t &d, Plan &pl) {
    if (d.att_mode == 1) {
        pl = Plan{};
        pl.tpb_f = pl.tpb_b = 32;
        pl.tc_f = pl.tc_b = asrk_div_up(d.Te, 32);
        pl.KP = 1;
        pl.nT = asrk_div_up(d.Te, 64);
        pl.lds_ctx = ((size_t)std::max((d.Te + 3) & ~3, 8 * CTX_CF) + 8 * 256) * sizeof(float);
        pl.lds_cb = 256;
        return pl.lds_ctx > LDS_BUDGET ? ASRK_ESHAPE : ASRK_OK;
    }
    const int KW = 2 * d.ks + 1;
    pl.KP = (d.K % 2 == 0) ? d.K + 1 : d.K;
    const size_t fix_f = (size_t)2 * d.ks + (size_t)d.K * KW + (size_t)d.A * pl.KP + 2 * (size_t)d.A;
    const bool thin = d.A <= 320 && d.K <= 16 && d.A * d.K <= 512 * AE_WPN && 2 * d.ks + 1 <= 64 * AE_NW &&
                      d.Te <= 512 * EB_NTE;
    const int wg_dflt = thin ? 256 : 512;
    pl.tpb_f = pick_tpb(d.B, d.Te, d.A, d.K, fix_f, 1 + (size_t)d.K, LDS_BUDGET, wg_dflt);
    if (pl.tpb_f <= 0) return ASRK_ESHAPE;
    pl.tc_f = asrk_div_up(d.Te, pl.tpb_f);
    pl.lds_f = (fix_f + (size_t)(1 + d.K) * pl.tpb_f) * sizeof(float);
    const size_t fix_b = 3 * (size_t)d.A + (size_t)d.A * pl.KP;
    pl.tpb_b = pick_tpb(d.B, d.Te, d.A, d.K, fix_b, (size_t)d.K + 1 + 3 * (size_t)d.A, LDS_BUDGET, wg_dflt);
    if (pl.tpb_b <= 0) return ASRK_ESHAPE;
    pl.tc_b = asrk_div_up(d.Te, pl.tpb_b);
    pl.lds_b = (fix_b + ((size_t)d.K + 1 + 3 * (size_t)d.A) * pl.tpb_b) * sizeof(float);
    pl.ae2_na = pl.ae2_km = 0;
    pl.lds_f2 = 0;
    if (d.A <= 320 && d.K <= 16 && 2 * d.ks + 1 <= 64 * AE_NW && pl.tpb_f <= 8 * AE_FR && d.A * d.K <= 512 * AE_WPN) {
        pl.ae2_na = d.A <= 128 ? 2 : 5;
        pl.ae2_km = d.K <= 12 ? 12 : 16;
        pl.lds_f2 = ((size_t)d.A * pl.KP + 8 * (16 * RED_RS + 16)) * sizeof(float);
    }
    pl.eb3_na = pl.eb3_km = 0;
    pl.lds_b3 = 0;
    if (d.A <= 320 && d.K <= 16 && pl.tpb_b <= 8 * EB_FR && d.A * d.K <= 512 * EB_WPN && d.Te <= 512 * EB_NTE &&
        pl.tpb_b * (d.K <= 12 ? 12 : 16) <= 512) {
        pl.eb3_na = d.A <= 128 ? 2 : 5;
        pl.eb3_km = d.K <= 12 ? 12 : 16;
        pl.lds_b3 = ((size_t)d.A * pl.KP + (size_t)pl.tpb_b * (pl.eb3_km + 64 * pl.eb3_na) + 8 * 16 * RED_RS) * sizeof(float);
        if (pl.lds_b3 > LDS_BUDGET) pl.eb3_na = 0;
    }
    pl.lds_ctx = ((size_t)std::max((d.Te + 3) & ~3, 8 * CTX_CF) + 8 * 256) * sizeof(float);
    pl.nT = asrk_div_up(d.Te, 64);
    const size_t cb_data = ((size_t)d.K * (64 + 2 * d.ks) + 256 + (size_t)d.K * KW) * sizeof(float);
    const size_t cb_w = ((size_t)2 * d.Te + 2 * d.ks) * sizeof(float);
    pl.lds_cb = cb_data > cb_w ? cb_data : cb_w;
    if (pl.lds_ctx > LDS_BUDGET || pl.lds_cb > LDS_BUDGET) return ASRK_ESHAPE;
    return ASRK_OK;
}

static void launch_attend_energy(const AttArgs &a, const Plan &pl, int B, hipStream_t s) {
    const dim3 grid(B, pl.tc_f);
    if (!pl.ae2_na) hipLaunchKernelGGL(attend_energy_kernel, grid, dim3(512), pl.lds_f, s, a);
    else if (pl.ae2_na == 2 && pl.ae2_km == 12) hipLaunchKernelGGL((attend_energy_kernel2<2, 12>), grid, dim3(512), pl.lds_f2, s, a);
    else if (pl.ae2_na == 2) hipLaunchKernelGGL((attend_energy_kernel2<2, 16>), grid, dim3(512), pl.lds_f2, s, a);
    else if (pl.ae2_km == 12) hipLaunchKernelGGL((attend_energy_kernel2<5, 12>), grid, dim3(512), pl.lds_f2, s, a);
    else hipLaunchKernelGGL((attend_energy_kernel2<5, 16>), grid, dim3(512), pl.lds_f2, s, a);
}


int check_dims(const asrk_speller_t *d) {
    if (!d) return ASRK_EINVAL;
    if (d->B < 0 || d->Te <= 0 || d->A <= 0 || d->Dv <= 0 || (d->K <= 0 && d->att_mode == 0) || d->K < 0 ||
        d->ks < 0 || d->H <= 0 || d->E < 0 || d->L < 0 || d->temperature == 0.f)
        return ASRK_EINVAL;
    if (d->nlayer < 0 || d->nlayer > ASRK_SPELLER_MAX_LAYERS || (d->nlayer > 1 && d->cell != 0)) return ASRK_ESHAPE;
    if (d->att_mode != 0 && d->att_mode != 1) return ASRK_EINVAL;
    if (d->nhead < 0 || (d->nhead > 1 && d->att_mode != 1) || (d->att_mode == 1 && d->A > 64 * DOT_NA)) return ASRK_ESHAPE;
    return ASRK_OK;
}

inline int n_layers(const asrk_speller_t &d) { return d.nlayer > 1 ? d.nlayer : 1; }
inline int n_heads(const asrk_speller_t &d) { return d.nhead > 1 ? d.nhead : 1; }
inline float *h_of(const asrk_speller_t &d, int l) { return l == 0 ? d.h : d.hu[l - 1]; }
inline float *c_of(const asrk_speller_t &d, int l) { return l == 0 ? d.c : d.cu[l - 1]; }
inline float *g_of(const asrk_speller_t &d, int l) { return l == 0 ? d.gates : d.gu[l - 1]; }
inline bool upper_ok(const asrk_speller_t &d, bool fwd) {
    for (int l = 1; l < n_layers(d); ++l)
        if (!d.Wu_ih[l - 1] || !d.Wu_hh[l - 1] || !d.hu[l - 1] || !d.cu[l - 1] || !d.gu[l - 1] ||
            (fwd && (!d.bu_ih[l - 1] || !d.bu_hh[l - 1])))
            return false;
    return true;
}

template <typename T>
int set_lds(T kernel, size_t bytes) {
    ASRK_HIP(hipFuncSetAttribute(reinterpret_cast<const void *>(kernel),
                                 hipFuncAttributeMaxDynamicSharedMemorySize, (int)bytes));
    return ASRK_OK;
}

}

extern "C" void asrk_prof_launches_(int id, int64_t n);

extern "C" int asrk_transpose_ld_f32(const float *in, int64_t ldi, float *out, int64_t ldo, int rows,
                                     int cols, void *stream) {
    if (rows < 0 || cols < 0 || ldi < cols || ldo < rows) return ASRK_EINVAL;
    if (rows == 0 || cols == 0) return ASRK_OK;
    if (!in || !out) return ASRK_EINVAL;
    hipLaunchKernelGGL(transpose_ld_kernel, dim3(asrk_div_up(cols, 32), asrk_div_up(rows, 32)), dim3(256), 0,
                       (hipStream_t)stream, in, (long)ldi, out, (long)ldo, rows, cols);
    ASRK_LAUNCH_CHECK();
    return ASRK_OK;
}

extern "C" int asrk_speller_dvalue_f32(const float *attn, int64_t attn_ld, int64_t attn_step, const float *dxh,
                                       int64_t step_ld, int64_t row_ld, float *dvalue, int B, int L, int Te,
                                       int Dv, void *stream) {
    if (B < 0 || L <= 0 || Te <= 0 || Dv <= 0) return ASRK_EINVAL;
    if (B == 0) return ASRK_OK;
    if (!attn || !dxh || !dvalue) return ASRK_EINVAL;
    const size_t lds = (size_t)DV_LC * Te * sizeof(float);
    if (lds > LDS_BUDGET) return ASRK_ESHAPE;
    int rc = set_lds(dvalue_kernel, lds);
    if (rc) return rc;
    hipLaunchKernelGGL(dvalue_kernel, dim3(B, asrk_div_up(Dv, 256)), dim3(256), lds, (hipStream_t)stream, attn,
                       (long)attn_ld, (long)attn_step, dxh, (long)step_ld, (long)row_ld, dvalue, L, Te, Dv);
    ASRK_LAUNCH_CHECK();
    return ASRK_OK;
}

extern "C" void asrk_speller_set_debug_(void *buf, int slots) {
    g_sp_dbg = reinterpret_cast<unsigned long long *>(buf);
    g_sp_dbg_slots = slots;
}

extern "C" int asrk_speller_plan(const asrk_speller_t *d, int *tc_fwd, int *tc_bwd) {
    int rc = check_dims(d);
    if (rc) return rc;
    Plan pl;
    rc = make_plan(*d, pl);
    if (rc) return rc;
    if (tc_fwd) *tc_fwd = pl.tc_f;
    if (tc_bwd) *tc_bwd = pl.tc_b;
    return ASRK_OK;
}

extern "C" int asrk_speller_plan_info(const asrk_speller_t *d, int *info) {
    if (!info) return ASRK_EINVAL;
    int rc = check_dims(d);
    if (rc) return rc;
    Plan pl;
    rc = make_plan(*d, pl);
    if (rc) return rc;
    const int v[8] = {pl.ae2_na, pl.ae2_km, pl.eb3_na, pl.eb3_km, pl.tpb_f, pl.tpb_b, pl.KP, d->Dv % 4 == 0};
    for (int i = 0; i < 8; ++i) info[i] = v[i];
    return ASRK_OK;
}

static int speller_step_fwd(const asrk_speller_t &d, const Plan &pl, int t, const float *prev, long prev_ld,
                            const float *pre, const float *emb, hipStream_t s) {
    const int B = d.B, H = d.H, A = d.A, Te = d.Te, Dv = d.Dv, K = d.K;
    const long In = (long)d.E + Dv;
    const int NH = n_heads(d), BN = B * NH;
    float *q_t = d.q + (long)t * BN * A;
    const float *h_t = d.h + (long)t * B * H;
    if (d.Wq) {
        SkArgs a{};
        const int NL = n_layers(d);
        a.nseg = NL;
        for (int l = 0; l < NL; ++l)
            a.seg[l] = SkSeg{h_of(d, l) + (long)t * B * H, d.Wq + (long)l * H, (long)H, (long)NL * H, H};
        a.M = B; a.R = NH * A; a.H = H;
        a.out = q_t; a.ldo = (long)NH * A; a.bias = d.bq;
        a.stamps = sp_slot(t, 0);
        int rc = launch_skinny<EPI_TANH_BIAS>(a, s);
        if (rc) return rc;
    }
    if (d.att_mode == 1) {
        DotArgs a{d.key, q_t, nullptr, nullptr, d.lens, d.e_scratch, nullptr, nullptr, 0, Te, A, NH, 0,
                  1.f / d.temperature};
        hipLaunchKernelGGL(dot_energy_kernel, dim3(BN, asrk_div_up(Te, 8)), dim3(512), 0, s, a);
    } else {
        AttArgs a{d.key, q_t, prev, d.Wc, d.Wp, d.we, d.be, d.lens, d.conv + (long)t * B * Te * K, d.e_scratch,
                  prev_ld, Te, A, K, d.ks, pl.tpb_f, pl.KP, 1.f / d.temperature, d.shared_kv ? 0 : 1, d.row_mem};
        a.stamps = sp_slot(t, 1);
        launch_attend_energy(a, pl, B, s);
    }
    float *attn_t = d.attn + (long)t * d.attn_step;
    float *ctx_t = d.ctx + (long)t * B * Dv;
    float *ctxh_t = NH > 1 ? d.ctxh + (long)t * BN * Dv : ctx_t;
    {
        CtxArgs a{d.e_scratch, d.value, attn_t, ctxh_t, d.attn_ld, (long)Dv, Te, Dv, d.shared_kv ? 0 : 1, d.row_mem};
        a.stamps = sp_slot(t, 2);
        const bool vec = al16(d.value) && Dv % 4 == 0;
        const dim3 grid(BN, asrk_div_up(Dv, 256));
        const int RG = d.row_group;
        const size_t lds_g = (size_t)RG * ((Te + 3) & ~3) * sizeof(float);
        if (RG > 1 && RG <= 8 * CG_MAXR && NH == 1 && vec && B % RG == 0 && al16(ctxh_t) && Dv % 4 == 0 &&
            lds_g <= 64 * 1024 && !d.shared_kv && (B / RG) * asrk_div_up(Dv, 256) >= 64)
            hipLaunchKernelGGL(softmax_context_group_kernel, dim3(B / RG, asrk_div_up(Dv, 256)), dim3(512), lds_g, s, a, RG);
        else if (vec) hipLaunchKernelGGL(softmax_context_kernel<true>, grid, dim3(512), pl.lds_ctx, s, a);
        else hipLaunchKernelGGL(softmax_context_kernel<false>, grid, dim3(512), pl.lds_ctx, s, a);
    }
    if (NH > 1) {
        SkArgs a{};
        a.nseg = 1;
        a.seg[0] = SkSeg{ctxh_t, d.Wm, (long)NH * Dv, (long)NH * Dv, NH * Dv};
        a.M = B; a.R = Dv; a.H = H;
        a.out = ctx_t; a.ldo = Dv; a.bias = d.bm;
        int rc = launch_skinny<EPI_STORE>(a, s);
        if (rc) return rc;
    }
    if (!pre && !emb) return ASRK_OK;
    {
        SkArgs a{};
        int n = 0;
        if (emb) a.seg[n++] = SkSeg{emb, d.W_ih, (long)d.E, In, d.E};
        a.seg[n++] = SkSeg{ctx_t, d.W_ih + d.E, (long)Dv, In, Dv};
        a.seg[n++] = SkSeg{h_t, d.W_hh, (long)H, (long)H, H};
        a.nseg = n;
        a.M = B; a.R = 4 * H; a.H = H;
        a.pre = pre;
        a.b0 = emb ? d.b_ih : nullptr;
        a.b1 = emb ? d.b_hh : nullptr;
        a.gru = d.cell;
        a.c_prev = d.cell ? h_t : d.c + (long)t * B * H;
        a.c_new = d.cell ? nullptr : d.c + (long)(t + 1) * B * H;
        a.h_new = d.h + (long)(t + 1) * B * H;
        a.gates = d.gates ? d.gates + (long)t * B * 4 * H : nullptr;
        a.h_bm = (d.states && n_layers(d) == 1) ? d.states + (long)t * H : nullptr;
        a.h_bm_ld = (long)d.L * H;
        a.stamps = sp_slot(t, 3);
        int rc = launch_skinny<EPI_LSTM_FWD>(a, s);
        if (rc) return rc;
    }
    for (int l = 1; l < n_layers(d); ++l) {
        SkArgs a{};
        a.nseg = 2;
        a.seg[0] = SkSeg{h_of(d, l - 1) + (long)(t + 1) * B * H, d.Wu_ih[l - 1], (long)H, (long)H, H};
        a.seg[1] = SkSeg{h_of(d, l) + (long)t * B * H, d.Wu_hh[l - 1], (long)H, (long)H, H};
        a.M = B; a.R = 4 * H; a.H = H;
        a.b0 = d.bu_ih[l - 1];
        a.b1 = d.bu_hh[l - 1];
        a.c_prev = c_of(d, l) + (long)t * B * H;
        a.c_new = c_of(d, l) + (long)(t + 1) * B * H;
        a.h_new = h_of(d, l) + (long)(t + 1) * B * H;
        a.gates = g_of(d, l) + (long)t * B * 4 * H;
        a.h_bm = (d.states && l == n_layers(d) - 1) ? d.states + (long)t * H : nullptr;
        a.h_bm_ld = (long)d.L * H;
        int rc = launch_skinny<EPI_LSTM_FWD>(a, s);
        if (rc) return rc;
    }
    ASRK_LAUNCH_CHECK();
    return ASRK_OK;
}

static int prep_attrs(const Plan &pl) {
    int rc = set_lds(attend_energy_kernel, pl.lds_f);
    if (rc) return rc;
    if (pl.ae2_na) {
        rc = pl.ae2_na == 2 ? (pl.ae2_km == 12 ? set_lds(attend_energy_kernel2<2, 12>, pl.lds_f2) : set_lds(attend_energy_kernel2<2, 16>, pl.lds_f2))
                            : (pl.ae2_km == 12 ? set_lds(attend_energy_kernel2<5, 12>, pl.lds_f2) : set_lds(attend_energy_kernel2<5, 16>, pl.lds_f2));
        if (rc) return rc;
    }
    rc = set_lds(softmax_context_kernel<true>, pl.lds_ctx);
    if (rc) return rc;
    rc = set_lds(softmax_context_kernel<false>, pl.lds_ctx);
    if (rc) return rc;
    rc = set_lds(energy_bwd_kernel2, pl.lds_b);
    if (rc) return rc;
    if (pl.eb3_na) {
        rc = pl.eb3_na == 2 ? (pl.eb3_km == 12 ? set_lds(energy_bwd_kernel3<2, 12>, pl.lds_b3) : set_lds(energy_bwd_kernel3<2, 16>, pl.lds_b3))
                            : (pl.eb3_km == 12 ? set_lds(energy_bwd_kernel3<5, 12>, pl.lds_b3) : set_lds(energy_bwd_kernel3<5, 16>, pl.lds_b3));
        if (rc) return rc;
    }
    return set_lds(conv_bwd_kernel, pl.lds_cb);
}

extern "C" int asrk_speller_fwd_f32(const asrk_speller_t *d, void *stream) {
    int rc = check_dims(d);
    if (rc) return rc;
    if (d->B == 0 || d->L == 0) return ASRK_OK;
    const bool loc = d->att_mode == 0;
    if (!d->key || !d->value || !d->lens || !d->Wq || !d->W_ih ||
        !d->W_hh || !d->eproj || !d->q || !d->attn || !d->ctx || !d->h || (!d->c && !d->cell) ||
        !d->e_scratch || (d->cell != 0 && d->cell != 1) || !upper_ok(*d, true))
        return ASRK_EINVAL;
    if (loc && (!d->Wc || !d->Wp || !d->we || !d->be || !d->conv || !d->prev0)) return ASRK_EINVAL;
    if (n_heads(*d) > 1 && (!d->Wm || !d->ctxh)) return ASRK_EINVAL;
    if (!loc && (d->shared_kv || d->row_mem)) return ASRK_EINVAL;
    Plan pl;
    rc = make_plan(*d, pl);
    if (rc) return rc;
    rc = prep_attrs(pl);
    if (rc) return rc;
    hipStream_t s = (hipStream_t)stream;
    asrk_prof_begin_(PROF_SPELLER, s);
    for (int t = 0; t < d->L; ++t) {
        const float *prev = t == 0 ? d->prev0 : d->attn + (long)(t - 1) * d->attn_step;
        const long prev_ld = t == 0 ? d->Te : d->attn_ld;
        rc = speller_step_fwd(*d, pl, t, prev, prev_ld, d->eproj + (long)t * d->B * 4 * d->H, nullptr, s);
        if (rc) return rc;
    }
    asrk_prof_end_(PROF_SPELLER, s);
    asrk_prof_launches_(PROF_SPELLER, (3L + n_layers(*d) + (n_heads(*d) > 1)) * d->L - 1);
    return ASRK_OK;
}

extern "C" int asrk_speller_step_f32(const asrk_speller_t *d, int slot, const float *prev_att,
                                     int64_t prev_ld, const float *emb, void *stream) {
    int rc = check_dims(d);
    if (rc) return rc;
    if (d->B == 0) return ASRK_OK;
    if (slot < 0 || slot >= d->L) return ASRK_EINVAL;
    if (d->nlayer > 1 || d->att_mode != 0 || d->nhead > 1) return ASRK_ESHAPE;
    if (!d->key || !d->value || !d->lens || !d->Wc || !d->Wp || !d->we || !d->be || !d->q || !d->conv ||
        !d->attn || !d->ctx || !d->h || !d->e_scratch || !prev_att || (d->cell != 0 && d->cell != 1) || d->row_group < 0)
        return ASRK_EINVAL;
    if (!d->Wq && emb) return ASRK_EINVAL;
    if (emb && (!d->W_ih || !d->W_hh || !d->b_ih || !d->b_hh || (!d->c && !d->cell))) return ASRK_EINVAL;
    Plan pl;
    rc = make_plan(*d, pl);
    if (rc) return rc;
    rc = prep_attrs(pl);
    if (rc) return rc;
    hipStream_t s = (hipStream_t)stream;
    asrk_prof_begin_(PROF_SPELLER, s);
    rc = speller_step_fwd(*d, pl, slot, prev_att, (long)prev_ld, nullptr, emb, s);
    asrk_prof_end_(PROF_SPELLER, s);
    asrk_prof_launches_(PROF_SPELLER, 3);
    return rc;
}

extern "C" int asrk_joint_score_f32(const float *att_logp, const int64_t *cand, const float *psi,
                                    const float *prev_ctc, const float *lm_logp, float *out, int n, int V,
                                    int C, double ctc_weight, double lm_weight, double logzero, void *stream) {
    if (n < 0 || V <= 0 || C < 0) return ASRK_EINVAL;
    if (n == 0) return ASRK_OK;
    if (!att_logp || !out || out == att_logp) return ASRK_EINVAL;
    if (cand && (!psi || !prev_ctc)) return ASRK_EINVAL;
    hipLaunchKernelGGL(joint_score_kernel, dim3(n), dim3(256), 0, (hipStream_t)stream, att_logp, cand, psi,
                       prev_ctc, lm_logp, out, V, C, (float)(1.0 - ctc_weight), (float)ctc_weight,
                       (float)lm_weight, (float)logzero);
    ASRK_LAUNCH_CHECK();
    return ASRK_OK;
}

extern "C" int asrk_lstm_cell_fused_f32(const float *x, int64_t ldx, int In, const float *h, const float *c,
                                        const float *W_ih, const float *W_hh, const float *b_ih,
                                        const float *b_hh, float *h_out, float *c_out, int B, int H,
                                        void *stream) {
    if (B < 0 || H <= 0 || In <= 0 || ldx < In) return ASRK_EINVAL;
    if (B == 0) return ASRK_OK;
    if (!x || !h || !c || !W_ih || !W_hh || !h_out || !c_out) return ASRK_EINVAL;
    SkArgs a{};
    a.nseg = 2;
    a.seg[0] = SkSeg{x, W_ih, (long)ldx, (long)In, In};
    a.seg[1] = SkSeg{h, W_hh, (long)H, (long)H, H};
    a.M = B; a.R = 4 * H; a.H = H;
    a.b0 = b_ih; a.b1 = b_hh;
    a.c_prev = c; a.c_new = c_out; a.h_new = h_out;
    hipStream_t s = (hipStream_t)stream;
    asrk_prof_begin_(PROF_CELL, s);
    const int rc = launch_skinny<EPI_LSTM_FWD>(a, s);
    asrk_prof_end_(PROF_CELL, s);
    return rc;
}

extern "C" int asrk_speller_bwd_f32(const asrk_speller_t *d, const asrk_speller_bwd_t *g, void *stream) {
    int rc = check_dims(d);
    if (rc) return rc;
    if (!g) return ASRK_EINVAL;
    if (d->B == 0 || d->L == 0) return ASRK_OK;
    const bool loc = d->att_mode == 0;
    if (!d->key || !d->value || !d->lens || !d->Wq || !d->q ||
        !d->attn || !d->gates || !d->h || (!d->c && !d->cell) || (d->cell != 0 && d->cell != 1) ||
        !g->dstates || !g->WT || !g->WqT ||
        !g->dkey || !g->dxh || !g->dq_pre || !g->dattn || !g->dq_part || !g->dc || !upper_ok(*d, false))
        return ASRK_EINVAL;
    if (loc && (!d->Wc || !d->Wp || !d->we || !d->conv || !d->prev0 || !g->dprev || !g->dconv || !g->dwe_part ||
                !g->dWp_part || !g->dbe_part || !g->dWc_part))
        return ASRK_EINVAL;
    if (n_heads(*d) > 1 && (!g->WmT || !g->dctxh)) return ASRK_EINVAL;
    for (int l = 1; l < n_layers(*d); ++l)
        if (!g->WuT[l - 1] || !g->dxu[l - 1] || !g->dcu[l - 1]) return ASRK_EINVAL;
    if (d->shared_kv || d->row_mem) return ASRK_EINVAL;
    Plan pl;
    rc = make_plan(*d, pl);
    if (rc) return rc;
    if (g->tc != pl.tc_b) return ASRK_EWORKSPACE;
    rc = prep_attrs(pl);
    if (rc) return rc;
    hipStream_t s = (hipStream_t)stream;
    const int B = d->B, H = d->H, A = d->A, Te = d->Te, Dv = d->Dv, K = d->K, L = d->L;
    const long XH = (long)Dv + H;
    asrk_prof_begin_(PROF_SPELLER, s);
    const int NL = n_layers(*d), top = NL - 1, NH = n_heads(*d), BN = B * NH;
    auto cell_bwd = [&](int l, int st, const float *dq_pre_next, const float *add0, long ld0, int stamp_t) {
        SkArgs a{};
        a.nseg = dq_pre_next ? 1 : 0;
        if (dq_pre_next) a.seg[0] = SkSeg{dq_pre_next, g->WqT + (long)l * H * NH * A, (long)NH * A, (long)NH * A, NH * A};
        a.M = B; a.R = H; a.H = H;
        a.add0 = add0; a.ld0 = ld0;
        if (l == top) { a.add1 = g->dstates + (long)st * H; a.ld1 = (long)L * H; }
        else { a.add1 = g->dxu[l] + (long)st * B * 2 * H; a.ld1 = 2L * H; }
        a.dG = g_of(*d, l) + (long)st * B * 4 * H;
        a.gru = d->cell;
        a.bc_prev = (d->cell ? d->h : c_of(*d, l)) + (long)st * B * H;
        a.bc_new = d->cell ? a.bc_prev : c_of(*d, l) + (long)(st + 1) * B * H;
        a.dc = l == 0 ? g->dc : g->dcu[l - 1];
        a.dc_valid = dq_pre_next ? 1 : 0;
        if (stamp_t >= 0 && l == 0) a.stamps = sp_slot(stamp_t, 8);
        return launch_skinny<EPI_LSTM_BWD>(a, s);
    };
    auto upper_dx = [&](int l, int st) {
        SkArgs a{};
        a.nseg = 1;
        a.seg[0] = SkSeg{g_of(*d, l) + (long)st * B * 4 * H, g->WuT[l - 1], 4L * H, 4L * H, 4 * H};
        a.M = B; a.R = 2 * H; a.H = H;
        a.out = g->dxu[l - 1] + (long)st * B * 2 * H; a.ldo = 2L * H;
        return launch_skinny<EPI_STORE>(a, s);
    };
    for (int l = top; l >= 0; --l) {
        rc = cell_bwd(l, L - 1, nullptr, nullptr, 0, -1);
        if (rc) return rc;
        if (l >= 1) {
            rc = upper_dx(l, L - 1);
            if (rc) return rc;
        }
    }
    for (int t = L - 1; t >= 0; --t) {
        float *dG_t = d->gates + (long)t * B * 4 * H;
        float *dxh_t = g->dxh + (long)t * B * XH;
        {
            SkArgs a{};
            a.nseg = 1;
            a.seg[0] = SkSeg{dG_t, g->WT, 4L * H, 4L * H, 4 * H};
            a.M = B; a.R = (int)XH; a.H = H;
            a.out = dxh_t; a.ldo = XH;
            a.stamps = sp_slot(t, 4);
            rc = launch_skinny<EPI_STORE>(a, s);
            if (rc) return rc;
        }
        const float *attn_t = d->attn + (long)t * d->attn_step;
        const float *dctx_rows = dxh_t;
        long dctx_ld = XH;
        if (NH > 1) {
            SkArgs a{};
            a.nseg = 1;
            a.seg[0] = SkSeg{dxh_t, g->WmT, XH, (long)Dv, Dv};
            a.M = B; a.R = NH * Dv; a.H = H;
            float *dctxh_t = g->dctxh + (long)t * BN * Dv;
            a.out = dctxh_t; a.ldo = (long)NH * Dv;
            rc = launch_skinny<EPI_STORE>(a, s);
            if (rc) return rc;
            dctx_rows = dctxh_t;
            dctx_ld = Dv;
        }
        {
            DattnArgs a{dctx_rows, d->value, g->dattn_seq ? g->dattn_seq + (long)t * d->attn_step : nullptr,
                        (loc && t + 1 < L) ? g->dprev : nullptr, d->lens, g->dattn, dctx_ld, d->attn_ld, (long)Te, Te, Dv};
            a.stamps = sp_slot(t, 5);
            a.lens_div = NH - 1;
            const bool vec = al16(d->value) && al16(dctx_rows) && Dv % 4 == 0 && dctx_ld % 4 == 0;
            const dim3 grid(BN, asrk_div_up(Te, 8));
            if (vec) hipLaunchKernelGGL(dattn_kernel<true>, grid, dim3(512), 0, s, a);
            else hipLaunchKernelGGL(dattn_kernel<false>, grid, dim3(512), 0, s, a);
        }
        const float *q_t = d->q + (long)t * BN * A;
        float *dq_pre_t = g->dq_pre + (long)t * BN * A;
        if (!loc) {
            DotArgs a{d->key, q_t, attn_t, g->dattn, d->lens, nullptr, g->dkey, g->dq_part, d->attn_ld, Te, A, NH,
                      pl.tpb_b, 1.f / d->temperature};
            hipLaunchKernelGGL(dot_energy_bwd_kernel, dim3(BN, pl.tc_b), dim3(512), 0, s, a);
            CbArgs c{nullptr, nullptr, nullptr, g->dq_part, q_t, nullptr, nullptr, dq_pre_t, 0, Te, 0, 0, pl.tc_b, A,
                     0, 0};
            c.dq_only = 1;
            hipLaunchKernelGGL(conv_bwd_kernel, dim3(BN, 1), dim3(256), pl.lds_cb, s, c);
        } else {
        const float *conv_t = d->conv + (long)t * B * Te * K;
        {
            EbArgs a{d->key, q_t, conv_t, d->Wp, d->we, attn_t, g->dattn, d->lens, g->dkey, g->dconv,
                     g->dq_part, g->dwe_part, g->dWp_part, g->dbe_part, d->attn_ld, Te, A, K, pl.tpb_b,
                     pl.KP, 1.f / d->temperature};
            a.stamps = sp_slot(t, 6);
            const dim3 grid(B, pl.tc_b);
            if (!pl.eb3_na) hipLaunchKernelGGL(energy_bwd_kernel2, grid, dim3(512), pl.lds_b, s, a);
            else if (pl.eb3_na == 2 && pl.eb3_km == 12) hipLaunchKernelGGL((energy_bwd_kernel3<2, 12>), grid, dim3(512), pl.lds_b3, s, a);
            else if (pl.eb3_na == 2) hipLaunchKernelGGL((energy_bwd_kernel3<2, 16>), grid, dim3(512), pl.lds_b3, s, a);
            else if (pl.eb3_km == 12) hipLaunchKernelGGL((energy_bwd_kernel3<5, 12>), grid, dim3(512), pl.lds_b3, s, a);
            else hipLaunchKernelGGL((energy_bwd_kernel3<5, 16>), grid, dim3(512), pl.lds_b3, s, a);
        }
        {
            const float *prev = t == 0 ? d->prev0 : d->attn + (long)(t - 1) * d->attn_step;
            CbArgs a{g->dconv, prev, d->Wc, g->dq_part, q_t, g->dprev, g->dWc_part, dq_pre_t,
                     t == 0 ? (long)Te : d->attn_ld, Te, K, d->ks, pl.tc_b, A, pl.nT, t > 0 ? 1 : 0};
            a.stamps = sp_slot(t, 7);
            hipLaunchKernelGGL(conv_bwd_kernel, dim3(B, pl.nT + K + 1), dim3(256), pl.lds_cb, s, a);
        }
        }
        if (t > 0) {
            for (int l = top; l >= 0; --l) {
                const float *hh = l == 0 ? dxh_t + Dv : g->dxu[l - 1] + (long)t * B * 2 * H + H;
                rc = cell_bwd(l, t - 1, dq_pre_t, hh, l == 0 ? XH : 2L * H, t);
                if (rc) return rc;
                if (l >= 1) {
                    rc = upper_dx(l, t - 1);
                    if (rc) return rc;
                }
            }
        }
        ASRK_LAUNCH_CHECK();
    }
    asrk_prof_end_(PROF_SPELLER, s);
    asrk_prof_launches_(PROF_SPELLER, (5L + 2 * (NL - 1) + (NH > 1)) * L - 1);
    return ASRK_OK;
}
```

end-to-end-asr-pytorch_amd/speller_ops.py:

```python
import ctypes
import os

import torch
from torch.autograd import Function

from . import _lib
from . import ops
from .ops import _L, _p, _stream, _f32c, _require_gpu, gemm, colsum, copy3d

c_int, c_i64, c_f32, c_vp = ctypes.c_int, ctypes.c_int64, ctypes.c_float, ctypes.c_void_p


class SpellerT(ctypes.Structure):
    _fields_ = ([(n, c_int) for n in ("B", "Te", "A", "Dv", "K", "ks", "H", "E", "L")]
                + [("temperature", c_f32), ("shared_kv", c_int)]
                + [(n, c_vp) for n in ("key", "value", "lens", "Wq", "bq", "Wc", "Wp", "we", "be", "W_ih",
                                       "W_hh", "b_ih", "b_hh", "eproj", "q", "conv", "attn")]
                + [("attn_ld", c_i64), ("attn_step", c_i64)]
                + [(n, c_vp) for n in ("ctx", "gates", "h", "c", "states", "e_scratch", "prev0", "row_mem")]
                + [("cell", c_int), ("nlayer", c_int)]
                + [(n, c_vp * 2) for n in ("Wu_ih", "Wu_hh", "bu_ih", "bu_hh", "hu", "cu", "gu")]
                + [("att_mode", c_int), ("nhead", c_int), ("Wm", c_vp), ("bm", c_vp), ("ctxh", c_vp)]
                + [("row_group", c_int)])


class SpellerBwdT(ctypes.Structure):
    _fields_ = ([(n, c_vp) for n in ("dstates", "dattn_seq", "WT", "WqT", "dkey", "dxh", "dq_pre", "dattn",
                                     "dprev", "dconv", "dq_part", "dwe_part", "dWp_part", "dbe_part",
                                     "dWc_part", "dc")]
                + [("tc", c_int)]
                + [(n, c_vp * 2) for n in ("WuT", "dxu", "dcu")]
                + [("WmT", c_vp), ("dctxh", c_vp)])


def _ptr(t):
    return t.data_ptr() if t is not None else None


MAX_LOOP_LAYERS = 3


def supported_train_loop(attention, decoder, training):
    if supported_loop(attention, decoder):
        return True
    if os.environ.get('ASRK_SPELLER', '1') == '0':
        return False
    att_ok = (attention.mode == 'loc' and attention.num_head == 1) or (attention.mode == 'dot' and attention.dim <= 512)
    dec_ok = decoder.layer == 1 or (decoder.enable_cell and decoder.layer <= MAX_LOOP_LAYERS
                                    and not (training and decoder.dropout > 0))
    return att_ok and dec_ok


def _set_slots(field, tensors):
    for i, t in enumerate(tensors):
        field[i] = _ptr(t)


def supported_loop(attention, decoder):
    if os.environ.get('ASRK_SPELLER', '1') == '0':
        return False
    return attention.mode == 'loc' and attention.num_head == 1 and decoder.layer == 1


def stack_gru_params(w_ih, w_hh, b_ih, b_hh):
    H = w_hh.shape[1]
    z = lambda *shape: torch.zeros(shape, dtype=w_ih.dtype, device=w_ih.device)
    return (torch.cat([w_ih, z(H, w_ih.shape[1])], 0), torch.cat([w_hh[:2 * H], z(H, H), w_hh[2 * H:]], 0),
            torch.cat([b_ih, z(H)], 0), torch.cat([b_hh[:2 * H], z(H), b_hh[2 * H:]], 0))


def uniform_attention(lens, Te):
    idx = torch.arange(Te, device=lens.device).unsqueeze(0)
    valid = (idx < lens.unsqueeze(1)).to(torch.float32)
    return (valid / lens.clamp(min=1).to(torch.float32).unsqueeze(1)).contiguous()


def transpose_into(src, ldi, rows, cols, dst, ldo):
    _lib.check(_L().asrk_transpose_ld_f32(_p(src), ldi, _p(dst), ldo, rows, cols, _stream()), "transpose")


class SpellerLoopFn(Function):

    @staticmethod
    def forward(ctx, key, value, lens, sos_emb, teacher_emb, Wq, bq, Wc, Wp, we, be, W_ih, W_hh, b_ih,
                b_hh, L, temperature, cell=0, nhead=1, Wm=None, bm=None, *upper):
        _require_gpu(key)
        lib = _L()
        dev = key.device
        key, value = _f32c(key), _f32c(value)
        NH = int(nhead)
        dot = Wc is None
        BN, Te, A = key.shape
        B = BN // NH
        Dv = value.shape[2]
        Wq, bq = _f32c(Wq), _f32c(bq)
        Wc, Wp, we, be = (None,) * 4 if dot else tuple(_f32c(t) for t in (Wc, Wp, we, be))
        Wm, bm = (_f32c(Wm), _f32c(bm)) if NH > 1 else (None, None)
        W_ih, W_hh, b_ih, b_hh = (_f32c(t) for t in (W_ih, W_hh, b_ih, b_hh))
        H = W_hh.shape[1]
        E = W_ih.shape[1] - Dv
        K, ks = (0, 0) if dot else (Wc.shape[0], (Wc.shape[2] - 1) // 2)
        upper = [_f32c(t) for t in upper]
        NL = 1 + len(upper) // 4
        if ((not dot and (Wc.shape[1] != 1 or Wp.shape != (A, K) or we.numel() != A or NH != 1))
                or BN != B * NH or value.shape[0] != BN or Wq.shape != (NH * A, NL * H) or E <= 0
                or (NH > 1 and Wm.shape != (Dv, NH * Dv))
                or len(upper) % 4 or NL > MAX_LOOP_LAYERS or (NL > 1 and cell != 0)
                or any(upper[4 * i].shape != (4 * H, H) or upper[4 * i + 1].shape != (4 * H, H) for i in range(NL - 1))):
            raise _lib.AsrkError("speller loop: unsupported attention/decoder shapes")
        lens = lens.to(device=dev, dtype=torch.int64).contiguous()
        f = dict(dtype=torch.float32, device=dev)
        emb_tm = torch.empty((L, B, E), **f)
        copy3d(_f32c(sos_emb), emb_tm, 1, B, E, 0, E, 0, E)
        if L > 1:
            te = _f32c(teacher_emb)
            copy3d(te, emb_tm[1:], L - 1, B, E, E, te.shape[1] * E, B * E, E)
        eproj = torch.empty((L * B, 4 * H), **f)
        gemm(0, 1, L * B, 4 * H, E, emb_tm, E, W_ih, E + Dv, eproj, 4 * H, bias=b_ih, bias2=b_hh)

        tape = dict(q=torch.empty((L, B, NH * A), **f), conv=torch.empty((L, B, Te, K) if not dot else (1,), **f),
                    ctxh=torch.empty((L, B, NH * Dv) if NH > 1 else (1,), **f),
                    ctx=torch.empty((L, B, Dv), **f), gates=torch.empty((L, B, 4 * H), **f),
                    h=torch.empty((L + 1, B, H), **f),
                    c=torch.empty((L + 1, B, H) if cell == 0 else (1,), **f))
        _lib.check(_L().asrk_fill_f32(_p(tape['h'][0]), tape['h'][0].numel(), 0.0, _stream()), 'fill')
        if cell == 0:
            _lib.check(_L().asrk_fill_f32(_p(tape['c'][0]), tape['c'][0].numel(), 0.0, _stream()), 'fill')
        up_tape = [dict(h=torch.empty((L + 1, B, H), **f), c=torch.empty((L + 1, B, H), **f),
                        g=torch.empty((L, B, 4 * H), **f)) for _ in range(NL - 1)]
        for ut in up_tape:
            for n_ in ('h', 'c'):
                _lib.check(_L().asrk_fill_f32(_p(ut[n_][0]), ut[n_][0].numel(), 0.0, _stream()), 'fill')
        states = torch.empty((B, L, H), **f)
        att_seq = torch.empty((B, NH, L, Te), **f)
        e_scratch = torch.empty((BN, Te), **f)
        prev0 = uniform_attention(lens, Te) if not dot else torch.empty((1,), **f)
        d = SpellerT(B, Te, A, Dv, K, ks, H, E, L, float(temperature), 0,
                     _ptr(key), _ptr(value), _ptr(lens), _ptr(Wq), _ptr(bq), _ptr(Wc), _ptr(Wp), _ptr(we),
                     _ptr(be), _ptr(W_ih), _ptr(W_hh), _ptr(b_ih), _ptr(b_hh), _ptr(eproj), _ptr(tape['q']),
                     _ptr(tape['conv']), _ptr(att_seq), L * Te, Te, _ptr(tape['ctx']), _ptr(tape['gates']),
                     _ptr(tape['h']), _ptr(tape['c']) if cell == 0 else None, _ptr(states), _ptr(e_scratch),
                     _ptr(prev0))
        d.cell = int(cell)
        d.nlayer = NL
        d.att_mode, d.nhead = (1 if dot else 0), NH
        d.Wm, d.bm, d.ctxh = _ptr(Wm), _ptr(bm), (_ptr(tape['ctxh']) if NH > 1 else None)
        _set_slots(d.Wu_ih, upper[0::4]); _set_slots(d.Wu_hh, upper[1::4])
        _set_slots(d.bu_ih, upper[2::4]); _set_slots(d.bu_hh, upper[3::4])
        _set_slots(d.hu, [u['h'] for u in up_tape]); _set_slots(d.cu, [u['c'] for u in up_tape])
        _set_slots(d.gu, [u['g'] for u in up_tape])
        _lib.check(lib.asrk_speller_fwd_f32(ctypes.byref(d), _stream()), "speller_fwd")
        ctx.cell = int(cell)
        ctx.nlayer = NL
        ctx.nhead, ctx.dot = NH, dot
        ctx.merge = (Wm, tape['ctxh']) if NH > 1 else None
        ctx.dims = (B, Te, A, Dv, K, ks, H, E, L, float(temperature), teacher_emb.shape[1])
        ctx.save_for_backward(key, value, lens, emb_tm, Wq, bq, Wc, Wp, we, be, W_ih, W_hh, tape['q'],
                              tape['conv'], tape['ctx'], tape['gates'], tape['h'], tape['c'], att_seq, prev0,
                              *upper[0::4], *upper[1::4], *[u[n_] for n_ in ('h', 'c', 'g') for u in up_tape])
        ctx.weight_refs = tuple(t_ for t_ in (Wq, bq, Wc, Wp, we, be, W_ih, W_hh, b_ih, b_hh, Wm, bm) + tuple(upper)
                                if t_ is not None)
        ctx.consumed = False
        return states, att_seq

    @staticmethod
    def backward(ctx, dstates, datt_seq):
        lib = _L()
        saved = ctx.saved_tensors
        (key, value, lens, emb_tm, Wq, bq, Wc, Wp, we, be, W_ih, W_hh, q, conv, ctx_all, gates, h, c,
         att_seq, prev0) = saved[:20]
        NL = ctx.nlayer
        nu = NL - 1
        Wu_ih, Wu_hh = saved[20:20 + nu], saved[20 + nu:20 + 2 * nu]
        hu, cu, gu = (saved[20 + (2 + i) * nu:20 + (3 + i) * nu] for i in range(3))
        if ctx.consumed:
            raise RuntimeError("SpellerLoopFn: backward twice (the gate tape is reused in place)")
        ctx.consumed = True
        B, Te, A, Dv, K, ks, H, E, L, temperature, Lt = ctx.dims
        NH, dot = ctx.nhead, ctx.dot
        BN, NA = B * NH, NH * A
        dev = key.device
        f = dict(dtype=torch.float32, device=dev)
        In, XH, KW = E + Dv, Dv + H, 2 * ks + 1
        dstates = _f32c(dstates) if dstates is not None else ops.zeros((B, L, H), dev)
        datt = _f32c(datt_seq) if datt_seq is not None else None
        d = SpellerT(B, Te, A, Dv, K, ks, H, E, L, temperature, 0,
                     _ptr(key), _ptr(value), _ptr(lens), _ptr(Wq), _ptr(bq), _ptr(Wc), _ptr(Wp), _ptr(we),
                     _ptr(be), _ptr(W_ih), _ptr(W_hh), None, None, None, _ptr(q), _ptr(conv), _ptr(att_seq),
                     L * Te, Te, _ptr(ctx_all), _ptr(gates), _ptr(h), _ptr(c) if ctx.cell == 0 else None, None, None,
                     _ptr(prev0))
        d.cell = ctx.cell
        d.nlayer = NL
        d.att_mode, d.nhead = (1 if dot else 0), NH
        _set_slots(d.Wu_ih, Wu_ih); _set_slots(d.Wu_hh, Wu_hh)
        _set_slots(d.hu, hu); _set_slots(d.cu, cu); _set_slots(d.gu, gu)
        tc = c_int(0)
        _lib.check(lib.asrk_speller_plan(ctypes.byref(d), None, ctypes.byref(tc)), "speller_plan")
        tc = tc.value
        WT = torch.empty((XH, 4 * H), **f)
        transpose_into(W_ih[:, E:], In, 4 * H, Dv, WT, 4 * H)
        transpose_into(W_hh, H, 4 * H, H, WT[Dv:], 4 * H)
        WqT = torch.empty((NL * H, NA), **f)
        transpose_into(Wq, NL * H, NA, NL * H, WqT, NA)
        WmT = dctxh = None
        if NH > 1:
            Wm, ctxh_all = ctx.merge
            WmT = torch.empty((NH * Dv, Dv), **f)
            transpose_into(Wm, NH * Dv, Dv, NH * Dv, WmT, Dv)
            dctxh = torch.empty((L, B, NH * Dv), **f)
        WuT = []
        for l in range(nu):
            wt = torch.empty((2 * H, 4 * H), **f)
            transpose_into(Wu_ih[l], H, 4 * H, H, wt, 4 * H)
            transpose_into(Wu_hh[l], H, 4 * H, H, wt[H:], 4 * H)
            WuT.append(wt)
        dxu = [torch.empty((L, B, 2 * H), **f) for _ in range(nu)]
        dcu = [torch.empty((B, H), **f) for _ in range(nu)]
        dkey = ops.zeros((BN, Te, A), dev)
        dwe_part = dWp_part = dbe_part = dWc_part = None
        if not dot:
            dwe_part = ops.zeros((B * tc, A), dev)
            dWp_part = ops.zeros((B * tc, A * K), dev)
            dbe_part = ops.zeros((B * tc,), dev)
            dWc_part = ops.zeros((B, K * KW), dev)
        dxh = torch.empty((L, B, XH), **f)
        dq_pre = torch.empty((L, B, NA), **f)
        scratch = [torch.empty(s, **f) for s in ((BN, Te), (B, Te), (B, Te, max(K, 1)), (BN * tc, A), (B, H))]
        g = SpellerBwdT(_ptr(dstates), _ptr(datt), _ptr(WT), _ptr(WqT), _ptr(dkey), _ptr(dxh), _ptr(dq_pre),
                        _ptr(scratch[0]), _ptr(scratch[1]), _ptr(scratch[2]), _ptr(scratch[3]),
                        _ptr(dwe_part), _ptr(dWp_part), _ptr(dbe_part), _ptr(dWc_part), _ptr(scratch[4]), tc)
        _set_slots(g.WuT, WuT); _set_slots(g.dxu, dxu); _set_slots(g.dcu, dcu)
        g.WmT, g.dctxh = _ptr(WmT), _ptr(dctxh)
        _lib.check(lib.asrk_speller_bwd_f32(ctypes.byref(d), ctypes.byref(g), _stream()), "speller_bwd")
        dG = gates.view(L * B, 4 * H)
        LB = L * B

        dvalue = torch.empty((BN, Te, Dv), **f)
        dcr, dcr_step, dcr_ld = (dxh, B * XH, XH) if NH == 1 else (dctxh, BN * Dv, Dv)
        rc = lib.asrk_speller_dvalue_f32(_p(att_seq), L * Te, Te, _p(dcr), dcr_step, dcr_ld, _p(dvalue), BN, L, Te,
                                         Dv, _stream())
        if rc == -2:
            att_rows = att_seq.view(BN, L, Te)
            for r in range(BN):
                src = dxh[:, r] if NH == 1 else dctxh.view(L, BN, Dv)[:, r]
                gemm(1, 0, Te, Dv, L, att_rows[r], Te, src, dcr_step, dvalue[r], Dv)
        else:
            _lib.check(rc, "speller_dvalue")
        demb = torch.empty((L, B, E), **f)
        gemm(0, 0, LB, E, 4 * H, dG, 4 * H, W_ih, In, demb, E)
        dsos = demb[0]
        dteacher = ops.zeros((B, Lt, E), dev)
        if L > 1:
            copy3d(demb[1:], dteacher, L - 1, B, E, B * E, E, E, Lt * E)

        def weight_grads():
            dW_ih = torch.empty((4 * H, In), **f)
            gemm(1, 0, 4 * H, E, LB, dG, 4 * H, emb_tm, E, dW_ih, In)
            gemm(1, 0, 4 * H, Dv, LB, dG, 4 * H, ctx_all, Dv, dW_ih[:, E:], In)
            dW_hh = torch.empty((4 * H, H), **f)
            gemm(1, 0, 4 * H, H, LB, dG, 4 * H, h, H, dW_hh, H)
            db = torch.empty((4 * H,), **f)
            colsum(dG, LB, 4 * H, 4 * H, db)
            dWq = torch.empty((NA, NL * H), **f)
            for l, hl in enumerate((h,) + tuple(hu)):
                gemm(1, 0, NA, H, LB, dq_pre, NA, hl, H, dWq[:, l * H:], NL * H)
            dbq = torch.empty((NA,), **f)
            colsum(dq_pre, LB, NA, NA, dbq)
            if dot:
                dWc = dWp = dwe = dbe = None
            else:
                dWp = torch.empty((A * K,), **f)
                colsum(dWp_part, B * tc, A * K, A * K, dWp)
                dwe = torch.empty((A,), **f)
                colsum(dwe_part, B * tc, A, A, dwe)
                dbe = torch.empty((1,), **f)
                colsum(dbe_part, B * tc, 1, 1, dbe)
                dWc = torch.empty((K * KW,), **f)
                colsum(dWc_part, B, K * KW, K * KW, dWc)
                dWc, dWp, dwe = dWc.view(K, 1, KW), dWp.view(A, K), dwe.view(we.shape)
            dWm = dbm = None
            if NH > 1:
                dWm = torch.empty((Dv, NH * Dv), **f)
                gemm(1, 0, Dv, NH * Dv, LB, dxh, XH, ctxh_all, NH * Dv, dWm, NH * Dv)
                dbm = torch.empty((Dv,), **f)
                colsum(dxh, LB, Dv, XH, dbm)
            out = [dWq, dbq, dWc, dWp, dwe, dbe, dW_ih, dW_hh, db, db.clone(), dWm, dbm]
            for l in range(nu):
                dGl = gu[l].view(LB, 4 * H)
                below = (h if l == 0 else hu[l - 1])[1:]
                dWi = torch.empty((4 * H, H), **f)
                gemm(1, 0, 4 * H, H, LB, dGl, 4 * H, below, H, dWi, H)
                dWh = torch.empty((4 * H, H), **f)
                gemm(1, 0, 4 * H, H, LB, dGl, 4 * H, hu[l], H, dWh, H)
                dbl = torch.empty((4 * H,), **f)
                colsum(dGl, LB, 4 * H, 4 * H, dbl)
                out += [dWi, dWh, dbl, dbl.clone()]
            return out

        if ops._can_defer(*ctx.weight_refs) and ops._defer_beside_bptt():
            used = tuple(t_ for t_ in (dG, emb_tm, ctx_all, h, dq_pre, dWp_part, dwe_part, dbe_part, dWc_part, dxh)
                         if t_ is not None) + tuple(hu) + tuple(gu) + ((ctx.merge[1],) if NH > 1 else ())
            with ops._SideStream(dev, used, background=False) as side:
                wg = weight_grads()
                side.keep(*[t_ for t_ in wg if t_ is not None])
        else:
            wg = weight_grads()
        return (dkey, dvalue, None, dsos, dteacher, *wg[:10], None, None, None, None, wg[10], wg[11], *wg[12:])


class SpellerStepper:

    def __init__(self, attention, decoder, key, value, lens, n, shared):
        _require_gpu(key)
        al = attention.att_layer
        self.key, self.value = _f32c(key), _f32c(value)
        self.lens = lens.to(device=key.device, dtype=torch.int64).contiguous()
        params = [p.detach() for p in decoder.layers.layer_params(0)]
        self.gru = not decoder.enable_cell
        if self.gru:
            params = stack_gru_params(*params)
        w_ih, w_hh, b_ih, b_hh = (_f32c(p) for p in params)
        self.w = [_f32c(t.detach()) for t in (attention.proj_q.weight, attention.proj_q.bias, al.loc_conv.weight,
                                              al.loc_proj.weight, al.gen_energy.weight, al.gen_energy.bias)]
        self.w += [w_ih, w_hh, b_ih, b_hh]
        _, Te, A = self.key.shape
        Dv, H = self.value.shape[2], w_hh.shape[1]
        E = w_ih.shape[1] - Dv
        K, ks = self.w[2].shape[0], (self.w[2].shape[2] - 1) // 2
        f = dict(dtype=torch.float32, device=key.device)
        self.n, self.Te, self.H, self.Dv = n, Te, H, Dv
        self.q = torch.empty((1, n, A), **f)
        self.conv = torch.empty((1, n, Te, K), **f)
        self.attn = torch.empty((n, 1, Te), **f)
        self.ctx = torch.empty((1, n, Dv), **f)
        self.h = torch.empty((2, n, H), **f)
        self.c = torch.empty((2, n, H), **f)
        self.e = torch.empty((n, Te), **f)
        self.d = SpellerT(n, Te, A, Dv, K, ks, H, E, 1, float(al.temperature), 1 if shared else 0,
                          _ptr(self.key), _ptr(self.value), _ptr(self.lens), *[_ptr(t) for t in self.w], None,
                          _ptr(self.q), _ptr(self.conv), _ptr(self.attn), Te, Te, _ptr(self.ctx), None,
                          _ptr(self.h), _ptr(self.c), None, _ptr(self.e), None)
        self.d.cell = 1 if self.gru else 0

    def step(self, emb, prev_att):
        emb, prev = _f32c(emb), _f32c(prev_att)
        _lib.check(_L().asrk_speller_step_f32(ctypes.byref(self.d), 0, _p(prev), self.Te, _p(emb), _stream()),
                   "speller_step")
        return self.attn, self.ctx[0], self.h[1], self.c[1]


class MultiSpellerStepper:

    def __init__(self, attention, decoder, key, value, lens, capacity, row_group=0):
        _require_gpu(key)
        al = attention.att_layer
        self.key, self.value = _f32c(key), _f32c(value)
        self.lens = lens.to(device=key.device, dtype=torch.int64).contiguous()
        params = [p.detach() for p in decoder.layers.layer_params(0)]
        self.gru = not decoder.enable_cell
        if self.gru:
            params = stack_gru_params(*params)
        w_ih, w_hh, b_ih, b_hh = (_f32c(p) for p in params)
        self.w = [_f32c(t.detach()) for t in (attention.proj_q.weight, attention.proj_q.bias, al.loc_conv.weight,
                                              al.loc_proj.weight, al.gen_energy.weight, al.gen_energy.bias)]
        self.w += [w_ih, w_hh, b_ih, b_hh]
        _, Te, A = self.key.shape
        Dv, H = self.value.shape[2], w_hh.shape[1]
        E = w_ih.shape[1] - Dv
        K, ks = self.w[2].shape[0], (self.w[2].shape[2] - 1) // 2
        f = dict(dtype=torch.float32, device=key.device)
        n = capacity
        self.cap, self.Te, self.H, self.Dv = n, Te, H, Dv
        self.q = torch.empty((n, A), **f)
        self.conv = torch.empty((n, Te, K), **f)
        self.ctx = torch.empty((n, Dv), **f)
        self.e = torch.empty((n, Te), **f)
        self.d = SpellerT(n, Te, A, Dv, K, ks, H, E, 1, float(al.temperature), 0,
                          _ptr(self.key), _ptr(self.value), _ptr(self.lens), *[_ptr(t) for t in self.w], None,
                          _ptr(self.q), _ptr(self.conv), None, Te, Te, _ptr(self.ctx), None,
                          None, None, None, _ptr(self.e), None, None)
        self.d.cell = 1 if self.gru else 0
        self.d.row_group = int(row_group)

    def step(self, row_mem, emb, prev_att, h_in, c_in, parent=None, state=None):
        n = int(row_mem.shape[0])
        if n > self.cap:
# ... 67 lines not shown
```

include/asrk.h:

```cpp
#ifndef ASRK_H
#define ASRK_H

#include <stddef.h>
#include <stdint.h>

#ifdef __cplusplus
extern "C" {
#endif

#define ASRK_OK 0
#define ASRK_EINVAL (-1)
#define ASRK_ESHAPE (-2)
#define ASRK_EWORKSPACE (-3)
#define ASRK_EDEVICE (-4)
#define ASRK_ETIMEOUT (-5)

int asrk_version(void);
const char *asrk_strerror(int rc);
int asrk_init(int device);

void asrk_profile_enable(int on);
void asrk_profile_families(unsigned mask);
void asrk_profile_reset(void);
int asrk_profile_get(int id, double *total_ms, int64_t *launches);
// ... 35 lines not shown
                                int a_row0, int a_k0, const void *B_panel, int b_rows, int b_K, int b_row0, int b_k0,
                                float beta, float *C, int ldc, const float *bias, const float *bias2, int splitk,
                                void *ws, size_t ws_bytes, int flags, void *stream);

int asrk_copy3d_f32(const float *src, float *dst, int n0, int n1, int n2,
                    int64_t s_stride0, int64_t s_stride1, int64_t d_stride0, int64_t d_stride1,
                    int accumulate, void *stream);

int asrk_colsum_f32(const float *X, int M, int N, int ldx, float *out, int accumulate,
                    void *stream);

int asrk_tanh_fwd_f32(const float *x, float *y, int64_t n, void *stream);
int asrk_tanh_bwd_f32(const float *y, const float *dy, float *dx, int64_t n, void *stream);

int asrk_log_softmax_fwd_f32(const float *x, float *y, int rows, int cols, int ld,
                             void *stream);
int asrk_log_softmax_bwd_f32(const float *y, const float *dy, float *dx, int rows, int cols,
                             int ld, void *stream);

int asrk_topk_f32(const float *x, int rows, int cols, int ld, int k, float *values,
                  int64_t *indices, void *stream);

int asrk_token_crop_i64(const int64_t *ids, int64_t ld, int B, int T, int64_t pad_idx, int64_t eos_idx,
                        int ignore_repeat, int64_t *out, int64_t ld_out, int32_t *out_len, void *stream);
int asrk_edit_distance_i64(const int64_t *a, int64_t lda, const int32_t *a_len, const int64_t *b, int64_t ldb,
                           const int32_t *b_len, int B, int max_b_len, int32_t *dist, void *stream);

int asrk_cross_entropy_fwd_f32(const float *logits, int rows, int V, int ld,
                               const int64_t *targets, int ignore_index, float *row_lse,
                               float *sums, void *stream);
int asrk_cross_entropy_bwd_f32(const float *logits, int rows, int V, int ld,
                               const int64_t *targets, int ignore_index, const float *row_lse,
                               const float *gscale, float *dlogits, void *stream);

size_t asrk_lstm_ws_bytes(void);
#define ASRK_REC_F32_MFMA 1
#define ASRK_REC_REARM 2
#define ASRK_REC_BWD_NO_DG 4
size_t asrk_lstm_xchg_bytes(int T, int B, int H, int ndir, int backward, int flags);
int asrk_lstm_plan_workgroups(int T, int B, int H, int ndir, int backward, int flags);
int asrk_lstm_rec_fwd_f32(float *G, const float *whh_f, const float *whh_r, float *Y, float *C,
                          int T, int B, int H, int ndir, void *xchg, int xchg_prefilled, void *ws,
                          int flags, void *stream);
int asrk_lstm_rec_fwd_pyr_f32(float *G, const float *whh_f, const float *whh_r, float *Y, float *C,
                              int T, int B, int H, int ndir, void *xchg, int xchg_prefilled, void *ws,
                              float *Y2, int pyr_mode, int pyr_rate, int flags, void *stream);
int asrk_lstm_rec_bwd_pyr_f32(float *gates, const float *whh_f, const float *whh_r, const float *C,
                              const float *dY, int T, int B, int H, int ndir, void *xchg,
                              int xchg_prefilled, void *ws, float *db, int pyr_mode, int pyr_rate,
                              int flags, void *stream);
int asrk_lstm_plan_is_bf(int T, int B, int H, int ndir, int backward, int flags);
int asrk_lstm_rec_fwd_pyr_panel_f32(float *G, const float *whh_f, const float *whh_r, float *Y, float *C,
                                    int T, int B, int H, int ndir, void *xchg, int xchg_prefilled, void *ws,
                                    float *Y2, int pyr_mode, int pyr_rate, void *x2_panel, int flags, void *stream);
int asrk_lstm_rec_bwd_pyr_panel_f32(float *gates, const float *whh_f, const float *whh_r, const float *C,
                                    const float *dY, int T, int B, int H, int ndir, void *xchg,
                                    int xchg_prefilled, void *ws, float *db, int pyr_mode, int pyr_rate,
                                    void *dg_panel, void *dgt_panel, int flags, void *stream);
int asrk_lstm_rec_fwd_len_f32(float *G, const float *whh_f, const float *whh_r, float *Y, float *C,
                              const int64_t *lens, int T, int B, int H, int ndir, void *xchg,
                              int xchg_prefilled, void *ws, float *Y2, int pyr_mode, int pyr_rate, int flags,
                              void *stream);
int asrk_gru_rec_fwd_f32(float *G, const float *whh_f, const float *whh_r, float *Y, int T, int B, int H,
                         int ndir, void *xchg, int xchg_prefilled, void *ws, float *Y2, int pyr_mode,
                         int pyr_rate, int flags, void *stream);
int asrk_gru_rec_bwd_f32(float *gates, const float *whh_f, const float *whh_r, const float *Y,
                         const float *dY, int T, int B, int H, int ndir, void *xchg, int xchg_prefilled,
                         void *ws, float *db, int pyr_mode, int pyr_rate, int flags, void *stream);
int asrk_lstm_rec_bwd_f32(float *gates, const float *whh_f, const float *whh_r, const float *C,
                          const float *dY, int T, int B, int H, int ndir, void *xchg,
                          int xchg_prefilled, void *ws, float *db, int flags, void *stream);
int asrk_lstm_check_error(void *ws, void *stream);

size_t asrk_ctc_prefix_beam_ws_bytes(int beam, int T);
int asrk_ctc_prefix_beam_ws_offsets(int beam, int T, int buf, int64_t *nb_off, int64_t *len_off, int64_t *tok_off,
                                    int64_t *parent_off, int64_t *last_off, int64_t *gidx_off);
int asrk_ctc_prefix_beam_f32(const float *ctc, int T, int V, const unsigned char *allowed, int beam, int cand,
                             const float *lm, float lm_weight, int t0, int t1, int cur_buf, int init,
                             int lm_step_follows, void *ws, size_t ws_bytes, void *stream);
size_t asrk_ctc_prefix_beam_multi_ws_bytes(int U, int beam, int Tmax, size_t *slab_stride);
int asrk_ctc_prefix_beam_multi_f32(const float *ctc, int64_t ctc_row_stride, int U, int Tmax, int V,
                                   const unsigned char *allowed, int beam, int cand, const float *lm, float lm_weight,
                                   const int *frames, const int *t_start, int j, int *out_parent, int *out_last,
                                   int *out_gidx, void *ws, size_t ws_bytes, void *stream);

int asrk_loc_conv_fwd_f32(const float *prev_att, const float *Wc, float *c, int B, int N, int T,
                          int K, int ks, void *stream);
int asrk_loc_conv_bwd_f32(const float *dc, const float *prev_att, const float *Wc,
                          float *dprev_att, float *dWc_acc, int B, int N, int T, int K, int ks,
                          void *stream);
int asrk_attn_energy_fwd_f32(int loc, const float *key, const float *q, const float *c,
                             const float *Wp, const float *we, const float *be,
                             const int64_t *lens, float *attn, float *e_scratch, int B, int N, int T,
                             int A, int K, float temperature, void *stream);
int asrk_attn_energy_bwd_f32(int loc, const float *key, const float *q, const float *c,
                             const float *Wp, const float *we, const int64_t *lens,
                             const float *attn, const float *dattn, float *dkey_acc, float *dq,
                             float *dc, float *dWp_acc, float *dwe_acc, float *dbe_acc, int B,
                             int N, int T, int A, int K, float temperature, void *stream);
int asrk_attn_context_fwd_f32(const float *attn, const float *value, float *ctx, int BN, int T,
                              int Dv, int64_t ctx_stride, void *stream);
int asrk_attn_context_bwd_f32(const float *dctx, const float *value, float *dattn, int BN, int T,
                              int Dv, int64_t dctx_stride, void *stream);

int asrk_lstm_cell_fwd_f32(float *gates, const float *c_prev, float *c, float *h, int B, int H,
                           void *stream);
int asrk_lstm_cell_bwd_f32(float *gates, const float *c_prev, const float *c, const float *dh,
                           const float *dc_in, float *dc_prev, int B, int H, void *stream);

int asrk_gru_cell_fwd_f32(float *gi, const float *gh, int64_t ldi, int64_t ldh, const float *h_prev,
                          int64_t ldp, float *h_new, int64_t ldn, int B, int H, void *stream);
int asrk_gru_cell_bwd_f32(float *gi, float *gh, int64_t ldi, int64_t ldh, const float *h_prev,
                          int64_t ldp, const float *dh, int64_t ldd, const float *dh2, float *dh_prev,
                          int64_t ldo, int B, int H, void *stream);

int asrk_embedding_fwd_f32(const int64_t *idx, const float *W, float *out, int64_t n, int D, int V,
                           void *stream);
int asrk_embedding_bwd_f32(const int64_t *idx, const float *dout, float *dW_acc, int64_t n, int D,
                           int V, void *stream);

typedef struct asrk_speller {
    int B, Te, A, Dv, K, ks, H, E, L;
    float temperature;
    int shared_kv;
    const float *key, *value;
    const int64_t *lens;
    const float *Wq, *bq, *Wc, *Wp, *we, *be, *W_ih, *W_hh, *b_ih, *b_hh;
    const float *eproj;
    float *q, *conv, *attn;
    int64_t attn_ld, attn_step;
    float *ctx, *gates, *h, *c, *states, *e_scratch;
    const float *prev0;
    const int *row_mem;
    int cell;
    int nlayer;
    const float *Wu_ih[2], *Wu_hh[2], *bu_ih[2], *bu_hh[2];
    float *hu[2], *cu[2], *gu[2];
    int att_mode, nhead;
    const float *Wm, *bm;
    float *ctxh;
    int row_group;
} asrk_speller_t;
#define ASRK_SPELLER_MAX_LAYERS 3

typedef struct asrk_speller_bwd {
    const float *dstates, *dattn_seq, *WT, *WqT;
    float *dkey, *dxh, *dq_pre, *dattn, *dprev, *dconv, *dq_part, *dwe_part, *dWp_part, *dbe_part,
        *dWc_part, *dc;
    int tc;
    const float *WuT[2];
    float *dxu[2], *dcu[2];
    const float *WmT;
    float *dctxh;
} asrk_speller_bwd_t;

int asrk_speller_plan(const asrk_speller_t *dims, int *tc_fwd, int *tc_bwd);
int asrk_speller_plan_info(const asrk_speller_t *dims, int *info);
int asrk_speller_fwd_f32(const asrk_speller_t *p, void *stream);
int asrk_speller_bwd_f32(const asrk_speller_t *p, const asrk_speller_bwd_t *g, void *stream);
int asrk_speller_step_f32(const asrk_speller_t *p, int slot, const float *prev_att, int64_t prev_ld,
                          const float *emb, void *stream);
int asrk_speller_dvalue_f32(const float *attn, int64_t attn_ld, int64_t attn_step, const float *dxh,
                            int64_t step_ld, int64_t row_ld, float *dvalue, int B, int L, int Te, int Dv,
                            void *stream);
int asrk_joint_score_f32(const float *att_logp, const int64_t *cand, const float *psi,
                         const float *prev_ctc, const float *lm_logp, float *out, int n, int V, int C,
                         double ctc_weight, double lm_weight, double logzero, void *stream);
int asrk_lstm_cell_fused_f32(const float *x, int64_t ldx, int In, const float *h, const float *c,
                             const float *W_ih, const float *W_hh, const float *b_ih,
                             const float *b_hh, float *h_out, float *c_out, int B, int H, void *stream);
int asrk_transpose_ld_f32(const float *in, int64_t ldi, float *out, int64_t ldo, int rows, int cols,
                          void *stream);

int asrk_layer_norm_fwd_f32(const float *x, const float *weight, const float *bias, float *y,
                            float *mean, float *rstd, int rows, int cols, float eps, void *stream);
int asrk_layer_norm_bwd_f32(const float *x, const float *weight, const float *dy, const float *mean,
                            const float *rstd, float *dx, float *dweight, float *dbias, int rows,
                            int cols, void *stream);
int asrk_dropout_f32(const float *x, float *y, int64_t n, float p, uint64_t seed, uint64_t offset,
                     void *stream);

int asrk_beam_select_f32(const float *topv, const int64_t *topi, const float *psi, const int64_t *cand, int U, int B, int C,
                         int t, int lmax, int fcap, const int *min_len, const int *max_len, int *alive, double *ssum,
                         int *utt_done, int64_t *prev_token, int64_t *parent, int64_t *col, float *pctc, int *hist_tok,
                         float *hist_sc, int *hist_par, int *fin_count, int *fin_kind, int *fin_t, int *fin_row,
                         float *fin_term, double *fin_ssum, int *live_utts, void *stream);

int asrk_gather_rows_multi_f32(int nseg, const float *const *src, float *const *dst, const int *row_floats, const int *mul,
                               const int *use_col, const int64_t *parent, const int64_t *col, int n, void *stream);

int asrk_conv_out_size(int in, int k, int stride, int pad);
int asrk_im2col_f32(const float *x, float *col, int B, int H, int W, int C, int KH, int KW, int SH, int SW,
                    int PH, int PW, int64_t sb, int64_t sh, int64_t sw, int64_t sc, void *stream);
int asrk_col2im_f32(const float *dcol, float *dx, int B, int H, int W, int C, int KH, int KW, int SH,
                    int SW, int PH, int PW, int64_t sb, int64_t sh, int64_t sw, int64_t sc, void *stream);
int asrk_im2col_ld_f32(const float *x, float *col, int ldcol, int B, int H, int W, int C, int KH, int KW, int SH, int SW,
                       int PH, int PW, int64_t sb, int64_t sh, int64_t sw, int64_t sc, void *stream);
int asrk_im2col_cl_f32(const float *x, float *col, int B, int H, int W, int C, int KH, int KW, int SH, int SW,
                       int PH, int PW, int64_t sb, int64_t sh, int64_t sw, int64_t sc, void *stream);
int asrk_col2im_cl_f32(const float *dcol, float *dx, int B, int H, int W, int C, int KH, int KW, int SH,
                       int SW, int PH, int PW, int64_t sb, int64_t sh, int64_t sw, int64_t sc, void *stream);
int asrk_conv_weight_reorder_f32(const float *src, float *dst, int Cout, int Cin, int KK, int inverse, void *stream);
int asrk_conv3x3_supported(int H, int W, int C, int Cout);
int asrk_conv3x3_weight_f32(const float *w, float *wf, int Cout, int Cin, int transpose, void *stream);
int asrk_conv3x3_f32(const float *x, const float *xmask, const float *wf, const float *bias, float *y, int B, int H, int W,
                     int C, int Cout, int relu, void *stream);
size_t asrk_conv3x3_wgrad_ws_bytes(int B, int H, int W, int C, int Cout);
int asrk_conv3x3_wgrad_f32(const float *x, const float *dy, const float *ymask, float *dw, float *db, int B, int H, int W,
                           int C, int Cout, void *ws, size_t ws_bytes, void *stream);
int asrk_conv3x3_first_supported(int H, int W, int C, int Cout);
int asrk_conv3x3_first_f32(const float *x, const float *w, const float *bias, float *y, int B, int H, int W, int C, int Cout,
                           int64_t sb, int64_t sh, int64_t sw, int64_t sc, int relu, void *stream);
size_t asrk_conv3x3_first_wgrad_ws_bytes(int B, int H, int W, int C, int Cout);
int asrk_conv3x3_first_wgrad_f32(const float *x, const float *dy, const float *ymask, float *dw, float *db, int B, int H,
                                 int W, int C, int Cout, int64_t sb, int64_t sh, int64_t sw, int64_t sc, void *ws,
                                 size_t ws_bytes, void *stream);
int asrk_conv3x3_len_f32(const float *x, const float *wf, const float *bias, float *y, const int64_t *hlen, int B, int H,
                         int W, int C, int Cout, int relu, void *stream);
int asrk_conv3x3_first_len_f32(const float *x, const float *w, const float *bias, float *y, const int64_t *hlen, int B, int H,
                               int W, int C, int Cout, int64_t sb, int64_t sh, int64_t sw, int64_t sc, int relu,
                               void *stream);
int asrk_im2col_ld_len_f32(const float *x, float *col, const int64_t *hlen, int ldcol, int B, int H, int W, int C, int KH,
                           int KW, int SH, int SW, int PH, int PW, int64_t sb, int64_t sh, int64_t sw, int64_t sc,
                           void *stream);
int asrk_im2col_cl_len_f32(const float *x, float *col, const int64_t *hlen, int B, int H, int W, int C, int KH, int KW,
                           int SH, int SW, int PH, int PW, int64_t sb, int64_t sh, int64_t sw, int64_t sc, void *stream);
int asrk_conv_zero_tail_f32(float *y, const int64_t *hlen, int B, int H, int64_t row, void *stream);
int asrk_relu_fwd_f32(float *x, int64_t n, void *stream);
int asrk_relu_bwd_f32(const float *y, const float *dy, float *dx, int64_t n, void *stream);
int asrk_maxpool2x2_fwd_f32(const float *x, float *y, uint8_t *idx, int B, int H, int W, int C,
                            int64_t osb, int64_t osh, int64_t osw, int64_t osc, void *stream);
int asrk_maxpool2x2_bwd_f32(const float *dy, const uint8_t *idx, float *dx, int B, int H, int W, int C,
                            int64_t osb, int64_t osh, int64_t osw, int64_t osc, void *stream);

int asrk_adadelta_step_f32(float *param, const float *grad, float *square_avg, float *acc_delta,
                           int64_t n, double lr, double rho, double eps, const float *clip_coef,
                           void *stream);
int asrk_adam_step_f32(float *param, const float *grad, float *exp_avg, float *exp_avg_sq, int64_t n,
                       double lr, double beta1, double beta2, double eps, int64_t step,
                       const float *clip_coef, void *stream);
int asrk_adadelta_multi_f32(int count, float *const *params, const float *const *grads,
                            float *const *square_avg, float *const *acc_delta, const int64_t *numel,
                            double lr, double rho, double eps, const float *clip_coef, void *stream);
int asrk_adam_multi_f32(int count, float *const *params, const float *const *grads,
                        float *const *exp_avg, float *const *exp_avg_sq, const int64_t *numel,
                        double lr, double beta1, double beta2, double eps, int64_t step,
                        const float *clip_coef, void *stream);

size_t asrk_grad_norm_ws_bytes(int count, const int64_t *numel);
int asrk_grad_norm_multi_f32(int count, const float *const *grads, const int64_t *numel, float max_norm,
                             float *norm_out, float *coef_out, void *ws, size_t ws_bytes, void *stream);
int asrk_fill_f32(float *x, int64_t n, float value, void *stream);

int asrk_fbank_frames_f32(const float *wave, int64_t n_samples, const float *window, float *frames,
                          int m, int win, int shift, int ldf, float preemph, int remove_dc,
                          void *stream);
int asrk_power_spectrum_f32(const float *spec, float *power, int64_t m, int nb, void *stream);
int asrk_log_floor_f32(float *x, int64_t n, float eps, void *stream);
int asrk_delta_f32(const float *x, const float *filters, float *y, int C, int D, int T, int L,
                   void *stream);
int asrk_cmvn_f32(const float *x, float *y, int rows, int T, float eps, void *stream);
int asrk_transpose_f32(const float *x, float *y, int rows, int cols, void *stream);
int asrk_fbank_frames_batch_f32(const void *wave, int sample_bytes, int64_t ld_wave, const int64_t *n_samples_host,
                                const int64_t *frame_off, int B, int max_m, const float *window, float *frames,
                                int win, int shift, int ldf, float scale, float preemph, int remove_dc,
                                void *stream);
int asrk_delta_cmvn_batch_f32(const float *mel, const int64_t *frame_off, int B, int D, const float *filters, int C,
                              int L, int apply_cmvn, float eps, float *out, int Tmax, void *stream);
int asrk_fbank_logmel_batch_f32(const void *wave, int sample_bytes, int64_t ld_wave, const int64_t *n_samples_host,
                                const int64_t *frame_off, int B, int max_m, const float *window, const float *tw_fft,
                                const float *tw_unpack, const float *melT, const int *mel_range, int nmel, int ld_mel,
                                float *mel, int win, int shift, int log2n, float scale, float preemph, int remove_dc,
                                float eps, void *stream);

int asrk_spec_augment_f32(const float *x, float *y, int B, int T, int ld, int D, int C, const int64_t *lens,
                          const int32_t *params, int n_fmask, int n_tmask, float fill, void *stream);

int asrk_ctc_loss_fwd_f32(const float *lp, int64_t stride_t, int64_t stride_b, int T, int B,
                          int V, const int64_t *targets, int64_t tgt_stride, int Lmax,
                          const int64_t *input_lengths, const int64_t *target_lengths,
                          int blank, float *alpha, float *beta, float *lpg, float *nll,
                          void *stream);
int asrk_ctc_loss_bwd_f32(const float *lp, int64_t stride_t, int64_t stride_b, int T, int B,
                          int V, const int64_t *targets, int64_t tgt_stride, int Lmax,
                          const int64_t *input_lengths, const int64_t *target_lengths,
                          int blank, const float *alpha, const float *beta, const float *lpg,
                          const float *nll, const float *gscale, float *grad, int64_t g_stride_t,
                          int64_t g_stride_b, void *stream);

#define ASRK_ALIGN_BP_AUTO 0
#define ASRK_ALIGN_BP_LDS 1
#define ASRK_ALIGN_BP_GLOBAL 2
size_t asrk_ctc_align_ws_bytes(int B, int T, int Lmax, int flags);
int asrk_ctc_align_f32(const float *lp, int64_t stride_t, int64_t stride_b, int T, int B, int V,
                       const int64_t *targets, int64_t tgt_stride, int Lmax, const int64_t *input_lengths,
                       const int64_t *target_lengths, int blank, int flags, int32_t *states, int32_t *tokens,
                       int32_t *spans, float *score, int64_t *stamps, void *ws, size_t ws_bytes, void *stream);

int asrk_ctc_prefix_score_f32(const float *x, const float *r_prev, const int *prefix_len,
                              const int *last_char, const int *candidates, float *psi,
                              float *r_out, int n, int C, int T, int V, int blank, int eos,
                              float logzero, void *stream);
int asrk_ctc_prefix_score_multi_f32(const float *x, const int *row_mem, const int *mem_len, const float *r_prev,
                                    const int *prefix_len, const int *last_char, const int *candidates,
                                    float *psi, float *r_out, int n, int C, int T, int V, int U, int blank,
                                    int eos, float logzero, void *stream);

int asrk_flac_info(const char *path, int *sample_rate, int *channels, int *bits_per_sample,
                   int64_t *total_samples, uint8_t *md5_16);
int asrk_flac_decode_i32(const char *path, int32_t *out, int64_t capacity_samples,
// ... 7 lines not shown
```

Before: 532,300 frames/s.

## Fuse speller backward dattn into energy-bwd and LSTM cell into conv-bwd kernel

Folds the per-step dattn computation (value·dctx dot products) into energy_bwd_kernel3 through a FUSE template path. It also merges the LSTM cell backward skinny GEMM with conv_bwd into a single cell_conv_kernel launch, using ticket counters to finish dq_pre in the last block. The aim is to cut per-timestep kernel launches and intermediate dattn traffic in the sequential speller backward loop. In exchange it adds ticket-based cross-block coordination, more register pressure in the fused kernels, and a fallback knob.

Result: no change. 534,700 frames/s, median of 6 (+0.5%).

```diff
diff --git a/end-to-end-asr-pytorch_amd/_lib.py b/end-to-end-asr-pytorch_amd/_lib.py
--- a/end-to-end-asr-pytorch_amd/_lib.py
+++ b/end-to-end-asr-pytorch_amd/_lib.py
@@ -150,6 +150,7 @@
     "asrk_maxpool2x2_bwd_f32": (c_int, [c_vp, c_vp, c_vp] + [c_int] * 4 + [c_i64] * 4 + [c_vp]),
     "asrk_speller_plan": (c_int, [c_vp, ctypes.POINTER(c_int), ctypes.POINTER(c_int)]),
     "asrk_speller_plan_info": (c_int, [c_vp, ctypes.POINTER(c_int)]),
+    "asrk_speller_bwd_plan_info": (c_int, [c_vp, ctypes.POINTER(c_int)]),
     "asrk_speller_fwd_f32": (c_int, [c_vp, c_vp]),
     "asrk_speller_bwd_f32": (c_int, [c_vp, c_vp, c_vp]),
     "asrk_speller_step_f32": (c_int, [c_vp, c_int, c_vp, c_i64, c_vp, c_vp]),
diff --git a/end-to-end-asr-pytorch_amd/csrc/core.cpp b/end-to-end-asr-pytorch_amd/csrc/core.cpp
--- a/end-to-end-asr-pytorch_amd/csrc/core.cpp
+++ b/end-to-end-asr-pytorch_amd/csrc/core.cpp
@@ -50,6 +50,7 @@
     k.bwd_poll = env_int("ASRK_BWD_POLL");
     k.bwd_presleep = env_int("ASRK_BWD_PRESLEEP");
     k.dbg_noload = env_present("ASRK_DBG_NOLOAD");
+    k.speller_bwd_fuse = env_int("ASRK_SPELLER_BWD_FUSE");
     k.deterministic = env_int("ASRK_DETERMINISTIC");
 }
 }
diff --git a/end-to-end-asr-pytorch_amd/csrc/knobs.h b/end-to-end-asr-pytorch_amd/csrc/knobs.h
--- a/end-to-end-asr-pytorch_amd/csrc/knobs.h
+++ b/end-to-end-asr-pytorch_amd/csrc/knobs.h
@@ -14,6 +14,7 @@
     int fwd_poll, fwd_presleep;
     int bwd_poll, bwd_presleep;
     int dbg_noload;
+    int speller_bwd_fuse;
     int deterministic;
 
     int get(int v, int dflt) const { return v == UNSET ? dflt : v; }
diff --git a/end-to-end-asr-pytorch_amd/csrc/speller.hip b/end-to-end-asr-pytorch_amd/csrc/speller.hip
--- a/end-to-end-asr-pytorch_amd/csrc/speller.hip
+++ b/end-to-end-asr-pytorch_amd/csrc/speller.hip
@@ -16,14 +16,16 @@
     const long i = (long)step * 16 + kid;
     return (g_sp_dbg && i < g_sp_dbg_slots) ? g_sp_dbg + i * 16 : nullptr;
 }
-#define SP_STAMP(ph)                                                                                     \
+#define SP_STAMP_AT(ph, first_, last_)                                                                   \
     do {                                                                                                 \
         if (p.stamps && threadIdx.x == 0) {                                                              \
-            if (blockIdx.x == 0 && blockIdx.y == 0) p.stamps[ph] = __builtin_readcyclecounter();         \
-            else if (blockIdx.x == gridDim.x - 1 && blockIdx.y == gridDim.y - 1 && ((ph) == 0 || (ph) == 9)) \
+            if (first_) p.stamps[ph] = __builtin_readcyclecounter();                                     \
+            else if ((last_) && ((ph) == 0 || (ph) == 9))                                                \
                 p.stamps[(ph) == 0 ? 12 : 13] = __builtin_readcyclecounter();                            \
         }                                                                                                \
     } while (0)
+#define SP_STAMP(ph) \
+    SP_STAMP_AT(ph, blockIdx.x == 0 && blockIdx.y == 0, blockIdx.x == gridDim.x - 1 && blockIdx.y == gridDim.y - 1)
 
 constexpr int SK_THREADS = 512, SK_WAVES = 8, SK_CH = 32;
 
@@ -71,21 +73,22 @@
     for (int j = 0; j < 8; ++j) v[j] = (valid && k + j < klen) ? row[k + j] : 0.f;
 }
 
+#define SK_STAMP(ph) SP_STAMP_AT(ph, bx == 0, bx == nbx - 1)
 template <int MT, int EPI, int VEC>
-__global__ __launch_bounds__(SK_THREADS) void skinny_kernel(SkArgs p) {
+__device__ __forceinline__ void skinny_body(const SkArgs &p, const int bx, const int nbx) {
     __shared__ float red[SK_WAVES][MT][4][64];
     const int tid = threadIdx.x, lane = tid & 63;
     const int wave = __builtin_amdgcn_readfirstlane(tid >> 6);
     const int slot = lane & 15, g = lane >> 4;
-    SP_STAMP(0);
+    SK_STAMP(0);
     int r;
     bool rvalid;
     if (EPI == EPI_LSTM_FWD) {
-        const int u = blockIdx.x * 4 + (slot >> 2);
+        const int u = bx * 4 + (slot >> 2);
         r = (slot & 3) * p.H + u;
         rvalid = u < p.H;
     } else {
-        r = blockIdx.x * 16 + slot;
+        r = bx * 16 + slot;
         rvalid = r < p.R;
     }
     f32x4 acc[MT][2];
@@ -99,11 +102,11 @@
         if (EPI == EPI_STORE || EPI == EPI_TANH_BIAS) {
 #pragma unroll
             for (int q = 0; q < 4; ++q) {
-                const int rr = blockIdx.x * 16 + (lane >> 4) * 4 + q;
+                const int rr = bx * 16 + (lane >> 4) * 4 + q;
                 e_in[q] = (rr < p.R && p.bias) ? p.bias[rr] : 0.f;
             }
         } else if (EPI == EPI_LSTM_FWD) {
-            const int u = blockIdx.x * 4 + (lane >> 4), H = p.H;
+            const int u = bx * 4 + (lane >> 4), H = p.H;
             if (u < H) {
 #pragma unroll
                 for (int q = 0; q < 4; ++q) {
@@ -118,7 +121,7 @@
             const int H = p.H;
 #pragma unroll
             for (int q = 0; q < 4; ++q) {
-                const int j = blockIdx.x * 16 + (lane >> 4) * 4 + q;
+                const int j = bx * 16 + (lane >> 4) * 4 + q;
                 if (j >= H) continue;
                 const float *gr = p.dG + (long)e_m * 4 * H + j;
                 e_in[q * 9 + 0] = p.add0 ? p.add0[(long)e_m * p.ld0 + j] : 0.f;
@@ -167,11 +170,11 @@
         for (int h = 0; h < 2; ++h) {
             const int sl = lrow + 8 * h;
             if (EPI == EPI_LSTM_FWD) {
-                const int u = blockIdx.x * 4 + (sl >> 2);
+                const int u = bx * 4 + (sl >> 2);
                 wrow[h] = (unsigned)((sl & 3) * p.H + u);
                 wok[h] = u < p.H;
             } else {
-                wrow[h] = (unsigned)(blockIdx.x * 16 + sl);
+                wrow[h] = (unsigned)(bx * 16 + sl);
                 wok[h] = (int)wrow[h] < p.R;
             }
         }
@@ -229,9 +232,9 @@
             f32x4 fw[2][2], fx[2][MT][2];
 #pragma unroll
             for (int j = 0; j < NB; ++j) SK_ISSUE(j, gw[j], gx[j]);
-            SP_STAMP(1);
+            SK_STAMP(1);
             stage(gw[0], gx[0], fw[0], fx[0]);
-            SP_STAMP(2);
+            SK_STAMP(2);
             SK_ISSUE(NB, gw[0], gx[0]);
 #define SK_STEP(u)                                                                                      \
     if (i0 + (u) >= mych) break;                                                                        \
@@ -284,9 +287,9 @@
     for (int mt = 0; mt < MT; ++mt)
 #pragma unroll
         for (int v = 0; v < 4; ++v) red[wave][mt][v][lane] = acc[mt][0][v] + acc[mt][1][v];
-    SP_STAMP(3);
+    SK_STAMP(3);
     __syncthreads();
-    SP_STAMP(4);
+    SK_STAMP(4);
     if (tid >= MT * 64) return;
     const int mt = tid >> 6;
     float v[4];
@@ -302,7 +305,7 @@
     if (EPI == EPI_STORE || EPI == EPI_TANH_BIAS) {
 #pragma unroll
         for (int q = 0; q < 4; ++q) {
-            const int rr = blockIdx.x * 16 + (lane >> 4) * 4 + q;
+            const int rr = bx * 16 + (lane >> 4) * 4 + q;
             if (rr < p.R) {
                 float y = v[q] + e_in[q];
                 if (EPI == EPI_TANH_BIAS) y = tanh_fast(y);
@@ -310,7 +313,7 @@
             }
         }
     } else if (EPI == EPI_LSTM_FWD) {
-        const int u = blockIdx.x * 4 + (lane >> 4);
+        const int u = bx * 4 + (lane >> 4);
         if (u >= p.H) return;
         const int H = p.H;
         float a[4];
@@ -345,7 +348,7 @@
         const int H = p.H;
 #pragma unroll
         for (int q = 0; q < 4; ++q) {
-            const int j = blockIdx.x * 16 + (lane >> 4) * 4 + q;
+            const int j = bx * 16 + (lane >> 4) * 4 + q;
             if (j >= H) continue;
             float *gr = p.dG + (long)m * 4 * H + j;
             if (p.gru) {
@@ -370,53 +373,73 @@
             p.dc[(long)m * H + j] = dct * gf;
         }
     }
-    SP_STAMP(9);
+    SK_STAMP(9);
+}
+#undef SK_STAMP
+
+template <int MT, int EPI, int VEC>
+__global__ __launch_bounds__(SK_THREADS) void skinny_kernel(SkArgs p) {
+    skinny_body<MT, EPI, VEC>(p, blockIdx.x, gridDim.x);
 }
 
 inline bool al16(const void *q) { return (reinterpret_cast<uintptr_t>(q) & 15) == 0; }
 
-template <int EPI>
-int launch_skinny(const SkArgs &a, hipStream_t s) {
-    if (a.M <= 0) return ASRK_OK;
+inline bool sk_vec_ok(const SkArgs &a) {
     bool vec = true;
     for (int i = 0; i < a.nseg; ++i)
         vec = vec && al16(a.seg[i].x) && al16(a.seg[i].w) && a.seg[i].ldx % 4 == 0 && a.seg[i].ldw % 4 == 0 &&
               a.seg[i].klen % 4 == 0;
+    return vec;
+}
+
+template <int EPI>
+bool sk_pass_args(const SkArgs &a, int m0, SkArgs &p) {
+    p = a;
+    p.M = a.M - m0 < 64 ? a.M - m0 : 64;
+    for (int i = 0; i < p.nseg; ++i) p.seg[i].x += (long)m0 * p.seg[i].ldx;
+    bool small = true;
+    const long wrows = (EPI == EPI_LSTM_FWD) ? 4L * p.H : (long)p.R;
+    for (int i = 0; i < p.nseg; ++i) {
+        const long wb = ((wrows - 1) * p.seg[i].ldw + p.seg[i].klen) * 4L;
+        const long xb = ((long)(p.M - 1) * p.seg[i].ldx + p.seg[i].klen) * 4L;
+        small = small && wb < (1L << 31) && xb < (1L << 31);
+        p.seg[i].wbytes = (unsigned)wb;
+        p.seg[i].xbytes = (unsigned)xb;
+    }
+    for (int i = p.nseg; i < 3; ++i) p.seg[i] = SkSeg{nullptr, nullptr, 0, 0, 0, 0u, 0u};
+    if (p.out) p.out += (long)m0 * p.ldo;
+    const long H4 = 4L * p.H, H1 = p.H;
+    if (p.pre) p.pre += m0 * H4;
+    if (p.c_prev) p.c_prev += m0 * H1;
+    if (p.c_new) p.c_new += m0 * H1;
+    if (p.h_new) p.h_new += m0 * H1;
+    if (p.gates) p.gates += m0 * H4;
+    if (p.h_bm) p.h_bm += (long)m0 * p.h_bm_ld;
+    if (p.add0) p.add0 += (long)m0 * p.ld0;
+    if (p.add1) p.add1 += (long)m0 * p.ld1;
+    if (p.dG) p.dG += m0 * H4;
+    if (p.bc_prev) p.bc_prev += m0 * H1;
+    if (p.bc_new) p.bc_new += m0 * H1;
+    if (p.dc) p.dc += m0 * H1;
+    return small;
+}
+inline int sk_mt(int M) { return M <= 16 ? 1 : (M <= 32 ? 2 : 4); }
+inline size_t sk_lds(int mt) { return (size_t)SK_WAVES * (16 + mt * 16) * 36 * sizeof(float); }
+
+template <int EPI>
+int launch_skinny(const SkArgs &a, hipStream_t s) {
+    if (a.M <= 0) return ASRK_OK;
+    const bool vec = sk_vec_ok(a);
     const int blocks = (EPI == EPI_LSTM_FWD) ? asrk_div_up(a.H, 4) : asrk_div_up(a.R, 16);
     if (blocks <= 0) return ASRK_OK;
     for (int m0 = 0; m0 < a.M; m0 += 64) {
-        SkArgs p = a;
-        p.M = a.M - m0 < 64 ? a.M - m0 : 64;
-        for (int i = 0; i < p.nseg; ++i) p.seg[i].x += (long)m0 * p.seg[i].ldx;
-        bool small = true;
-        const long wrows = (EPI == EPI_LSTM_FWD) ? 4L * p.H : (long)p.R;
-        for (int i = 0; i < p.nseg; ++i) {
-            const long wb = ((wrows - 1) * p.seg[i].ldw + p.seg[i].klen) * 4L;
-            const long xb = ((long)(p.M - 1) * p.seg[i].ldx + p.seg[i].klen) * 4L;
-            small = small && wb < (1L << 31) && xb < (1L << 31);
-            p.seg[i].wbytes = (unsigned)wb;
-            p.seg[i].xbytes = (unsigned)xb;
-        }
-        for (int i = p.nseg; i < 3; ++i) p.seg[i] = SkSeg{nullptr, nullptr, 0, 0, 0, 0u, 0u};
-        if (p.out) p.out += (long)m0 * p.ldo;
-        const long H4 = 4L * p.H, H1 = p.H;
-        if (p.pre) p.pre += m0 * H4;
-        if (p.c_prev) p.c_prev += m0 * H1;
-        if (p.c_new) p.c_new += m0 * H1;
-        if (p.h_new) p.h_new += m0 * H1;
-        if (p.gates) p.gates += m0 * H4;
-        if (p.h_bm) p.h_bm += (long)m0 * p.h_bm_ld;
-        if (p.add0) p.add0 += (long)m0 * p.ld0;
-        if (p.add1) p.add1 += (long)m0 * p.ld1;
-        if (p.dG) p.dG += m0 * H4;
-        if (p.bc_prev) p.bc_prev += m0 * H1;
-        if (p.bc_new) p.bc_new += m0 * H1;
-        if (p.dc) p.dc += m0 * H1;
-        const int mt = p.M <= 16 ? 1 : (p.M <= 32 ? 2 : 4);
+        SkArgs p;
+        const bool small = sk_pass_args<EPI>(a, m0, p);
+        const int mt = sk_mt(p.M);
 #define SK_LAUNCH_V(MT_, V_)                                                                        \
     do {                                                                                            \
         static AsrkLdsLatch latch_;                                                                 \
-        const size_t lds = (size_t)SK_WAVES * (16 + MT_ * 16) * 36 * sizeof(float);                 \
+        const size_t lds = sk_lds(MT_);                                                             \
         hipError_t e_ = asrk_max_lds_once(latch_, reinterpret_cast<const void *>(&skinny_kernel<MT_, EPI, V_>), (int)lds); \
         if (e_ != hipSuccess) return (int)e_;                                                       \
         hipLaunchKernelGGL((skinny_kernel<MT_, EPI, V_>), dim3(blocks), dim3(SK_THREADS), lds, s, p); \
@@ -914,7 +937,35 @@
     int Te, A, K, tpb, KP;
     float inv_temp;
     unsigned long long *stamps;
+    const float *dctx, *value, *ctx, *extra0, *extra1;
+    long dctx_ld, e0_ld, e1_ld;
+    int Dv, has0, has1;
+    int *tickets;
+    float *dq_pre;
 };
+
+__device__ __forceinline__ void dq_pre_store(const float *dq_part, const float *q, float *dq_pre, int b, int TC, int A, int a) {
+    float acc = 0.f;
+    for (int c = 0; c < TC; ++c) acc += dq_part[((long)b * TC + c) * A + a];
+    const float qv = q[(long)b * A + a];
+    dq_pre[(long)b * A + a] = acc * (1.f - qv * qv);
+}
+
+__device__ __forceinline__ void vrow_load(const float *v, int lane, int Dv, f32x4 (&a)[8]) {
+#pragma unroll
+    for (int i = 0; i < 8; ++i) a[i] = *reinterpret_cast<const f32x4 *>(v + min(lane * 4 + 256 * i, Dv - 4));
+}
+__device__ __forceinline__ float dot4(const f32x4 a, const f32x4 c) {
+    return __builtin_fmaf(a[3], c[3], __builtin_fmaf(a[2], c[2], __builtin_fmaf(a[1], c[1], a[0] * c[0])));
+}
+__device__ __forceinline__ float vrow_dot(const f32x4 (&a)[8], const f32x4 (&c)[8], const float *v, const float *g, int lane, int Dv) {
+    float acc = 0.f;
+#pragma unroll
+    for (int i = 0; i < 8; ++i) acc += maskf(dot4(a[i], c[i]), lane * 4 + 256 * i < Dv);
+    for (int d = lane * 4 + 256 * 8; d < Dv; d += 256)
+        acc += dot4(*reinterpret_cast<const f32x4 *>(v + d), *reinterpret_cast<const f32x4 *>(g + d));
+    return wave_sum(acc);
+}
 
 __global__ __launch_bounds__(512) void energy_bwd_kernel2(EbArgs p) {
     extern __shared__ float sm[];
@@ -1048,11 +1099,13 @@
     }
 }
 
-constexpr int EB_FR = 4, EB_WPN = 8, EB_NTE = 2;
-template <int NA, int KM>
+constexpr int EB_FR = 4, EB_WPN = 8, EB_NTE = 2, EB_VF = 2;
+static_assert(DAT_ND == 8, "vrow_load / vrow_dot stage 8 pieces per lane");
+template <int NA, int KM, bool FUSE>
 __global__ __launch_bounds__(512) void energy_bwd_kernel3(EbArgs p) {
     extern __shared__ float sm[];
     __shared__ float s_red8[8], s_be8[8];
+    __shared__ int s_last;
     constexpr int AP = 64 * NA;
     const int b = blockIdx.x, chunk = blockIdx.y, TC = gridDim.y, t0 = chunk * p.tpb;
     const int nt = min(p.tpb, p.Te - t0);
@@ -1066,6 +1119,17 @@
     const unsigned kdiv = kdiv_of(K);
 
     SP_STAMP(0);
+    constexpr int NROW = EB_FR + 1;
+    const float *gp = p.dctx + (long)b * p.dctx_ld;
+    f32x4 cg[DAT_ND], vr[EB_VF][DAT_ND];
+    float rdot[NROW];
+#define EB_VROW(r_) ((r_) == 0 ? p.ctx + (long)b * p.Dv \
+                             : p.value + ((long)b * p.Te + min(t0 + wave + 8 * ((r_) - 1), p.Te - 1)) * p.Dv)
+    if (FUSE) {
+        vrow_load(gp, lane, p.Dv, cg);
+#pragma unroll
+        for (int r = 0; r < EB_VF; ++r) vrow_load(EB_VROW(r), lane, p.Dv, vr[r]);
+    }
     const int len_raw = (int)p.lens[b];
     float kv[EB_FR][NA], dk[EB_FR][NA];
 #pragma unroll
@@ -1079,19 +1143,43 @@
             dk[f][j] = p.dkey[idx];
         }
     }
-    const float *ar = p.attn + (long)b * p.attn_ld, *dr = p.dattn + (long)b * Te;
+    const float *ar = p.attn + (long)b * p.attn_ld;
     float a_e[EB_NTE], d_e[EB_NTE], a_f[EB_FR], d_f[EB_FR];
-#pragma unroll
-    for (int e = 0; e < EB_NTE; ++e) {
-        const int t = min(tid + 512 * e, Te - 1);
-        a_e[e] = ar[t];
-        d_e[e] = dr[t];
-    }
-#pragma unroll
-    for (int f = 0; f < EB_FR; ++f) {
-        const int t = min(t0 + wave + 8 * f, Te - 1);
-        a_f[f] = ar[t];
-        d_f[f] = dr[t];
+    if (FUSE) {
+        const float *x0 = p.extra0 + (long)b * p.e0_ld, *x1 = p.extra1 + (long)b * p.e1_ld;
+        float u_e[EB_NTE], u_f[EB_FR];
+#pragma unroll
+        for (int e = 0; e < EB_NTE; ++e) {
+            const int t = min(tid + 512 * e, Te - 1);
+            a_e[e] = ar[t];
+            d_e[e] = x0[t];
+            u_e[e] = x1[t];
+        }
+#pragma unroll
+        for (int f = 0; f < EB_FR; ++f) {
+            const int t = min(t0 + wave + 8 * f, Te - 1);
+            a_f[f] = ar[t];
+            d_f[f] = x0[t];
+            u_f[f] = x1[t];
+        }
+#pragma unroll
+        for (int e = 0; e < EB_NTE; ++e) d_e[e] = maskf(d_e[e], p.has0 != 0) + maskf(u_e[e], p.has1 != 0);
+#pragma unroll
+        for (int f = 0; f < EB_FR; ++f) d_f[f] = maskf(d_f[f], p.has0 != 0) + maskf(u_f[f], p.has1 != 0);
+    } else {
+        const float *dr = p.dattn + (long)b * Te;
+#pragma unroll
+        for (int e = 0; e < EB_NTE; ++e) {
+            const int t = min(tid + 512 * e, Te - 1);
+            a_e[e] = ar[t];
+            d_e[e] = dr[t];
+        }
+#pragma unroll
+        for (int f = 0; f < EB_FR; ++f) {
+            const int t = min(t0 + wave + 8 * f, Te - 1);
+            a_f[f] = ar[t];
+            d_f[f] = dr[t];
+        }
     }
     float wpst[EB_WPN], old_wp[EB_WPN];
 #pragma unroll
@@ -1114,6 +1202,16 @@
         qv[j] = p.q[(long)b * A + ac];
         wev[j] = maskf(p.we[ac], a < A);
     }
+    if (FUSE) {
+#pragma unroll
+        for (int r = 0; r < NROW; ++r) {
+            rdot[r] = vrow_dot(vr[r % EB_VF], cg, EB_VROW(r), gp, lane, p.Dv);
+            if (r + EB_VF < NROW) vrow_load(EB_VROW(r + EB_VF), lane, p.Dv, vr[r % EB_VF]);
+        }
+#undef EB_VROW
+#pragma unroll
+        for (int f = 0; f < EB_FR; ++f) d_f[f] = rdot[1 + f] + d_f[f];
+    }
     SP_STAMP(1);
     const int len = min(len_raw, Te);
     float dot = 0.f;
@@ -1135,6 +1233,7 @@
     dot = 0.f;
 #pragma unroll
     for (int w = 0; w < 8; ++w) dot += s_red8[w];
+    if (FUSE) dot = rdot[0] + dot;
     float de_f[EB_FR], de_sum = 0.f;
 #pragma unroll
     for (int f = 0; f < EB_FR; ++f) {
@@ -1239,6 +1338,25 @@
 #pragma unroll
         for (int w = 0; w < 8; ++w) acc += s_be8[w];
         p.dbe_part[blk] = old_be + acc;
+    }
+    if (FUSE && p.tickets) {
+        asm volatile("s_waitcnt vmcnt(0)" ::: "memory");
+        __syncthreads();
+        if (tid == 0) {
+            __builtin_amdgcn_fence(__ATOMIC_RELEASE, "agent");
+            asm volatile("s_waitcnt vmcnt(0)" ::: "memory");
+            const int tk = __hip_atomic_fetch_add(p.tickets + b, 1, __ATOMIC_RELAXED, __HIP_MEMORY_SCOPE_AGENT);
+            if (tk == TC - 1) {
+                __builtin_amdgcn_fence(__ATOMIC_ACQUIRE, "agent");
+                asm volatile("s_waitcnt vmcnt(0)" ::: "memory");
+            }
+            s_last = tk == TC - 1;
+        }
+        __syncthreads();
+        if (s_last) {
+            if (tid < A) dq_pre_store(p.dq_part, p.q, p.dq_pre, b, TC, A, tid);
+            if (tid == 0) __hip_atomic_store(p.tickets + b, 0, __ATOMIC_RELAXED, __HIP_MEMORY_SCOPE_AGENT);
+        }
     }
     SP_STAMP(9);
 }
@@ -1323,11 +1441,11 @@
     int dq_only;
 };
 
-__global__ __launch_bounds__(256) void conv_bwd_kernel(CbArgs p) {
-    extern __shared__ float sm[];
-    const int b = blockIdx.x, y = p.dq_only ? p.nT + p.K : blockIdx.y, tid = threadIdx.x;
+#define CB_STAMP(ph) SP_STAMP_AT(ph, first, last)
+__device__ __forceinline__ void conv_bwd_body(const CbArgs &p, float *sm, const int b, const int y, const bool first, const bool last) {
+    const int tid = threadIdx.x < 256 ? (int)threadIdx.x : (1 << 28);
     const int Te = p.Te, K = p.K, ks = p.ks, KW = 2 * ks + 1;
-    SP_STAMP(0);
+    CB_STAMP(0);
     if (y < p.nT) {
         if (!p.want_dprev) return;
         const int s0 = y * 64, span = 64 + 2 * ks;
@@ -1340,18 +1458,18 @@
         }
         for (int i = tid; i < K * KW; i += 256) s_w[i] = p.Wc[i];
         __syncthreads();
-        const int sl = tid & 63, w = __builtin_amdgcn_readfirstlane(tid >> 6);
+        const int sl = threadIdx.x & 63, w = __builtin_amdgcn_readfirstlane(threadIdx.x >> 6);
         float acc = 0.f;
-        for (int k = w; k < K; k += 4) {
+        for (int k = w < 4 ? w : K; k < K; k += 4) {
             const float *wr = s_w + k * KW;
             const float *col = sd + k * span + sl + 2 * ks;
             for (int j = 0; j < KW; ++j) acc += col[-j] * wr[j];
         }
-        part[w * 64 + sl] = acc;
+        if (w < 4) part[w * 64 + sl] = acc;
         __syncthreads();
         if (tid < 64 && s0 + tid < Te)
             p.dprev[(long)b * Te + s0 + tid] = (part[tid] + part[64 + tid]) + (part[128 + tid] + part[192 + tid]);
-        SP_STAMP(9);
+        CB_STAMP(9);
     } else if (y < p.nT + K) {
         const int k = y - p.nT;
         float *s_dc = sm, *s_pv = sm + Te;
@@ -1384,13 +1502,26 @@
             p.dWc_part[((long)b * K + k) * KW + j] += acc;
         }
     } else {
-        for (int a = tid; a < p.A; a += 256) {
-            float acc = 0.f;
-            for (int c = 0; c < p.TC; ++c) acc += p.dq_part[((long)b * p.TC + c) * p.A + a];
-            const float qv = p.q[(long)b * p.A + a];
-            p.dq_pre[(long)b * p.A + a] = acc * (1.f - qv * qv);
-        }
-        SP_STAMP(9);
+        for (int a = tid; a < p.A; a += 256) dq_pre_store(p.dq_part, p.q, p.dq_pre, b, p.TC, p.A, a);
+        CB_STAMP(9);
+    }
+}
+#undef CB_STAMP
+
+__global__ __launch_bounds__(256) void conv_bwd_kernel(CbArgs p) {
+    extern __shared__ float sm[];
+    conv_bwd_body(p, sm, blockIdx.x, p.dq_only ? p.nT + p.K : blockIdx.y, blockIdx.x == 0 && blockIdx.y == 0,
+                  blockIdx.x == gridDim.x - 1 && blockIdx.y == gridDim.y - 1);
+}
+
+template <int MT, int VEC>
+__global__ __launch_bounds__(SK_THREADS) void cell_conv_kernel(SkArgs p, CbArgs c, int n_sk, int B) {
+    if ((int)blockIdx.x < n_sk) {
+        skinny_body<MT, EPI_LSTM_BWD, VEC>(p, blockIdx.x, n_sk);
+    } else {
+        extern __shared__ float sm[];
+        const int r = blockIdx.x - n_sk, y = r / B;
+        conv_bwd_body(c, sm, r - y * B, y, r == 0, blockIdx.x == gridDim.x - 1);
     }
 }
 
@@ -1490,7 +1621,21 @@
     size_t lds_b3;
     int ae2_na, ae2_km;
     size_t lds_f2;
+    int bwd_fuse;
 };
+
+int bwd_fuse_of(const asrk_speller_t &d, const Plan &pl) {
+    const int want = asrk_knobs_().get(asrk_knobs_().speller_bwd_fuse, 1);
+    if (want <= 0 || d.att_mode != 0 || d.nhead > 1 || d.nlayer > 1 || !pl.eb3_na || d.Dv % 4 != 0 ||
+        ((long)d.Dv + d.H) % 4 != 0 || d.B > 64)
+        return 0;
+    return want == 2 ? 2 : 1;
+}
+inline int bwd_launches_per_step(const asrk_speller_t &d, int fuse) {
+    if (fuse == 1) return 3;
+    if (fuse == 2) return 4;
+    return 5 + 2 * ((d.nlayer > 1 ? d.nlayer : 1) - 1) + (d.nhead > 1 ? 1 : 0);
+}
 
 int make_plan(const asrk_speller_t &d, Plan &pl) {
     if (d.att_mode == 1) {
@@ -1501,6 +1646,7 @@
         pl.nT = asrk_div_up(d.Te, 64);
         pl.lds_ctx = ((size_t)std::max((d.Te + 3) & ~3, 8 * CTX_CF) + 8 * 256) * sizeof(float);
         pl.lds_cb = 256;
+        pl.bwd_fuse = 0;
         return pl.lds_ctx > LDS_BUDGET ? ASRK_ESHAPE : ASRK_OK;
     }
     const int KW = 2 * d.ks + 1;
@@ -1540,6 +1686,7 @@
     const size_t cb_w = ((size_t)2 * d.Te + 2 * d.ks) * sizeof(float);
     pl.lds_cb = cb_data > cb_w ? cb_data : cb_w;
     if (pl.lds_ctx > LDS_BUDGET || pl.lds_cb > LDS_BUDGET) return ASRK_ESHAPE;
+    pl.bwd_fuse = bwd_fuse_of(d, pl);
     return ASRK_OK;
 }
 
@@ -1640,6 +1787,18 @@
     if (rc) return rc;
     const int v[8] = {pl.ae2_na, pl.ae2_km, pl.eb3_na, pl.eb3_km, pl.tpb_f, pl.tpb_b, pl.KP, d->Dv % 4 == 0};
     for (int i = 0; i < 8; ++i) info[i] = v[i];
+    return ASRK_OK;
+}
+
+extern "C" int asrk_speller_bwd_plan_info(const asrk_speller_t *d, int *info) {
+    if (!info) return ASRK_EINVAL;
+    int rc = check_dims(d);
+    if (rc) return rc;
+    Plan pl;
+    rc = make_plan(*d, pl);
+    if (rc) return rc;
+    info[0] = pl.bwd_fuse;
+    info[1] = bwd_launches_per_step(*d, pl.bwd_fuse);
     return ASRK_OK;
 }
 
@@ -1756,8 +1915,13 @@
     rc = set_lds(energy_bwd_kernel2, pl.lds_b);
     if (rc) return rc;
     if (pl.eb3_na) {
-        rc = pl.eb3_na == 2 ? (pl.eb3_km == 12 ? set_lds(energy_bwd_kernel3<2, 12>, pl.lds_b3) : set_lds(energy_bwd_kernel3<2, 16>, pl.lds_b3))
-                            : (pl.eb3_km == 12 ? set_lds(energy_bwd_kernel3<5, 12>, pl.lds_b3) : set_lds(energy_bwd_kernel3<5, 16>, pl.lds_b3));
+        rc = pl.eb3_na == 2 ? (pl.eb3_km == 12 ? set_lds(energy_bwd_kernel3<2, 12, false>, pl.lds_b3) : set_lds(energy_bwd_kernel3<2, 16, false>, pl.lds_b3))
+                            : (pl.eb3_km == 12 ? set_lds(energy_bwd_kernel3<5, 12, false>, pl.lds_b3) : set_lds(energy_bwd_kernel3<5, 16, false>, pl.lds_b3));
+        if (rc) return rc;
+    }
+    if (pl.eb3_na && pl.bwd_fuse) {
+        rc = pl.eb3_na == 2 ? (pl.eb3_km == 12 ? set_lds(energy_bwd_kernel3<2, 12, true>, pl.lds_b3) : set_lds(energy_bwd_kernel3<2, 16, true>, pl.lds_b3))
+                            : (pl.eb3_km == 12 ? set_lds(energy_bwd_kernel3<5, 12, true>, pl.lds_b3) : set_lds(energy_bwd_kernel3<5, 16, true>, pl.lds_b3));
         if (rc) return rc;
     }
     return set_lds(conv_bwd_kernel, pl.lds_cb);
@@ -1875,14 +2039,34 @@
     rc = make_plan(*d, pl);
     if (rc) return rc;
     if (g->tc != pl.tc_b) return ASRK_EWORKSPACE;
+    int fuse = g->no_fuse == 1 ? 0 : (g->no_fuse == 2 && pl.bwd_fuse ? 2 : pl.bwd_fuse);
+    if (g->no_fuse < 0 || g->no_fuse > 2) return ASRK_EINVAL;
+    if (fuse && (!d->ctx || (fuse == 1 && !g->tickets))) return ASRK_EINVAL;
+    if (fuse && !(al16(d->value) && al16(g->dxh) && al16(d->ctx))) fuse = 0;
+    pl.bwd_fuse = fuse;
     rc = prep_attrs(pl);
     if (rc) return rc;
     hipStream_t s = (hipStream_t)stream;
     const int B = d->B, H = d->H, A = d->A, Te = d->Te, Dv = d->Dv, K = d->K, L = d->L;
     const long XH = (long)Dv + H;
+    const int sk_mt_b = sk_mt(B), n_sk = asrk_div_up(H, 16);
+    const size_t lds_cc = std::max(sk_lds(sk_mt_b), pl.lds_cb);
+    if (fuse == 1 && L > 1) {
+#define CC_ATTR(MT_)                                                                     \
+    do {                                                                                 \
+        rc = set_lds(cell_conv_kernel<MT_, 2>, lds_cc);                                  \
+        if (!rc) rc = set_lds(cell_conv_kernel<MT_, 0>, pl.lds_cb);                      \
+    } while (0)
+        if (sk_mt_b == 1) CC_ATTR(1);
+        else if (sk_mt_b == 2) CC_ATTR(2);
+        else CC_ATTR(4);
+#undef CC_ATTR
+        if (rc) return rc;
+    }
     asrk_prof_begin_(PROF_SPELLER, s);
     const int NL = n_layers(*d), top = NL - 1, NH = n_heads(*d), BN = B * NH;
-    auto cell_bwd = [&](int l, int st, const float *dq_pre_next, const float *add0, long ld0, int stamp_t) {
+    long nlaunch = 0;
+    auto cell_args = [&](int l, int st, const float *dq_pre_next, const float *add0, long ld0, int stamp_t) {
         SkArgs a{};
         a.nseg = dq_pre_next ? 1 : 0;
         if (dq_pre_next) a.seg[0] = SkSeg{dq_pre_next, g->WqT + (long)l * H * NH * A, (long)NH * A, (long)NH * A, NH * A};
@@ -1897,7 +2081,11 @@
         a.dc = l == 0 ? g->dc : g->dcu[l - 1];
         a.dc_valid = dq_pre_next ? 1 : 0;
         if (stamp_t >= 0 && l == 0) a.stamps = sp_slot(stamp_t, 8);
-        return launch_skinny<EPI_LSTM_BWD>(a, s);
+        return a;
+    };
+    auto cell_bwd = [&](int l, int st, const float *dq_pre_next, const float *add0, long ld0, int stamp_t) {
+        nlaunch += asrk_div_up(B, 64);
+        return launch_skinny<EPI_LSTM_BWD>(cell_args(l, st, dq_pre_next, add0, ld0, stamp_t), s);
     };
     auto upper_dx = [&](int l, int st) {
         SkArgs a{};
@@ -1905,6 +2093,7 @@
         a.seg[0] = SkSeg{g_of(*d, l) + (long)st * B * 4 * H, g->WuT[l - 1], 4L * H, 4L * H, 4 * H};
         a.M = B; a.R = 2 * H; a.H = H;
         a.out = g->dxu[l - 1] + (long)st * B * 2 * H; a.ldo = 2L * H;
+        nlaunch += asrk_div_up(B, 64);
         return launch_skinny<EPI_STORE>(a, s);
     };
     for (int l = top; l >= 0; --l) {
@@ -1925,6 +2114,7 @@
             a.M = B; a.R = (int)XH; a.H = H;
             a.out = dxh_t; a.ldo = XH;
             a.stamps = sp_slot(t, 4);
+            nlaunch += asrk_div_up(B, 64);
             rc = launch_skinny<EPI_STORE>(a, s);
             if (rc) return rc;
         }
@@ -1938,20 +2128,23 @@
             a.M = B; a.R = NH * Dv; a.H = H;
             float *dctxh_t = g->dctxh + (long)t * BN * Dv;
             a.out = dctxh_t; a.ldo = (long)NH * Dv;
+            nlaunch += asrk_div_up(B, 64);
             rc = launch_skinny<EPI_STORE>(a, s);
             if (rc) return rc;
             dctx_rows = dctxh_t;
             dctx_ld = Dv;
         }
-        {
-            DattnArgs a{dctx_rows, d->value, g->dattn_seq ? g->dattn_seq + (long)t * d->attn_step : nullptr,
-                        (loc && t + 1 < L) ? g->dprev : nullptr, d->lens, g->dattn, dctx_ld, d->attn_ld, (long)Te, Te, Dv};
+        const float *extra0 = g->dattn_seq ? g->dattn_seq + (long)t * d->attn_step : nullptr;
+        const float *extra1 = (loc && t + 1 < L) ? g->dprev : nullptr;
+        if (!fuse) {
+            DattnArgs a{dctx_rows, d->value, extra0, extra1, d->lens, g->dattn, dctx_ld, d->attn_ld, (long)Te, Te, Dv};
             a.stamps = sp_slot(t, 5);
             a.lens_div = NH - 1;
             const bool vec = al16(d->value) && al16(dctx_rows) && Dv % 4 == 0 && dctx_ld % 4 == 0;
             const dim3 grid(BN, asrk_div_up(Te, 8));
             if (vec) hipLaunchKernelGGL(dattn_kernel<true>, grid, dim3(512), 0, s, a);
             else hipLaunchKernelGGL(dattn_kernel<false>, grid, dim3(512), 0, s, a);
+            ++nlaunch;
         }
         const float *q_t = d->q + (long)t * BN * A;
         float *dq_pre_t = g->dq_pre + (long)t * BN * A;
@@ -1963,6 +2156,7 @@
                      0, 0};
             c.dq_only = 1;
             hipLaunchKernelGGL(conv_bwd_kernel, dim3(BN, 1), dim3(256), pl.lds_cb, s, c);
+            nlaunch += 2;
         } else {
         const float *conv_t = d->conv + (long)t * B * Te * K;
         {
@@ -1971,21 +2165,54 @@
                      pl.KP, 1.f / d->temperature};
             a.stamps = sp_slot(t, 6);
             const dim3 grid(B, pl.tc_b);
+            ++nlaunch;
+            if (fuse) {
+                a.dattn = nullptr;
+                a.dctx = dctx_rows; a.dctx_ld = dctx_ld;
+                a.value = d->value; a.ctx = d->ctx + (long)t * B * Dv; a.Dv = Dv;
+                a.extra0 = extra0 ? extra0 : attn_t; a.e0_ld = d->attn_ld; a.has0 = extra0 != nullptr;
+                a.extra1 = extra1 ? extra1 : attn_t; a.e1_ld = extra1 ? (long)Te : d->attn_ld; a.has1 = extra1 != nullptr;
+                a.tickets = fuse == 1 ? g->tickets : nullptr;
+                a.dq_pre = dq_pre_t;
+                if (pl.eb3_na == 2 && pl.eb3_km == 12) hipLaunchKernelGGL((energy_bwd_kernel3<2, 12, true>), grid, dim3(512), pl.lds_b3, s, a);
+                else if (pl.eb3_na == 2) hipLaunchKernelGGL((energy_bwd_kernel3<2, 16, true>), grid, dim3(512), pl.lds_b3, s, a);
+                else if (pl.eb3_km == 12) hipLaunchKernelGGL((energy_bwd_kernel3<5, 12, true>), grid, dim3(512), pl.lds_b3, s, a);
+                else hipLaunchKernelGGL((energy_bwd_kernel3<5, 16, true>), grid, dim3(512), pl.lds_b3, s, a);
+            } else
             if (!pl.eb3_na) hipLaunchKernelGGL(energy_bwd_kernel2, grid, dim3(512), pl.lds_b, s, a);
-            else if (pl.eb3_na == 2 && pl.eb3_km == 12) hipLaunchKernelGGL((energy_bwd_kernel3<2, 12>), grid, dim3(512), pl.lds_b3, s, a);
-            else if (pl.eb3_na == 2) hipLaunchKernelGGL((energy_bwd_kernel3<2, 16>), grid, dim3(512), pl.lds_b3, s, a);
-            else if (pl.eb3_km == 12) hipLaunchKernelGGL((energy_bwd_kernel3<5, 12>), grid, dim3(512), pl.lds_b3, s, a);
-            else hipLaunchKernelGGL((energy_bwd_kernel3<5, 16>), grid, dim3(512), pl.lds_b3, s, a);
+            else if (pl.eb3_na == 2 && pl.eb3_km == 12) hipLaunchKernelGGL((energy_bwd_kernel3<2, 12, false>), grid, dim3(512), pl.lds_b3, s, a);
+            else if (pl.eb3_na == 2) hipLaunchKernelGGL((energy_bwd_kernel3<2, 16, false>), grid, dim3(512), pl.lds_b3, s, a);
+            else if (pl.eb3_km == 12) hipLaunchKernelGGL((energy_bwd_kernel3<5, 12, false>), grid, dim3(512), pl.lds_b3, s, a);
+            else hipLaunchKernelGGL((energy_bwd_kernel3<5, 16, false>), grid, dim3(512), pl.lds_b3, s, a);
         }
         {
             const float *prev = t == 0 ? d->prev0 : d->attn + (long)(t - 1) * d->attn_step;
             CbArgs a{g->dconv, prev, d->Wc, g->dq_part, q_t, g->dprev, g->dWc_part, dq_pre_t,
                      t == 0 ? (long)Te : d->attn_ld, Te, K, d->ks, pl.tc_b, A, pl.nT, t > 0 ? 1 : 0};
             a.stamps = sp_slot(t, 7);
-            hipLaunchKernelGGL(conv_bwd_kernel, dim3(B, pl.nT + K + 1), dim3(256), pl.lds_cb, s, a);
-        }
-        }
-        if (t > 0) {
+            ++nlaunch;
+            if (fuse != 1) {
+                hipLaunchKernelGGL(conv_bwd_kernel, dim3(B, pl.nT + K + 1), dim3(256), pl.lds_cb, s, a);
+            } else if (t == 0) {
+                hipLaunchKernelGGL(conv_bwd_kernel, dim3(B, pl.nT + K), dim3(256), pl.lds_cb, s, a);
+            } else {
+                SkArgs p;
+                const SkArgs c = cell_args(0, t - 1, dq_pre_t, dxh_t + Dv, XH, t);
+                const bool vec = sk_pass_args<EPI_LSTM_BWD>(c, 0, p) && sk_vec_ok(c);
+                const dim3 grid(n_sk + B * (pl.nT + K));
+#define CC_LAUNCH(MT_)                                                                                              \
+    do {                                                                                                            \
+        if (vec) hipLaunchKernelGGL((cell_conv_kernel<MT_, 2>), grid, dim3(SK_THREADS), lds_cc, s, p, a, n_sk, B);   \
+        else hipLaunchKernelGGL((cell_conv_kernel<MT_, 0>), grid, dim3(SK_THREADS), pl.lds_cb, s, p, a, n_sk, B);    \
+    } while (0)
+                if (sk_mt_b == 1) CC_LAUNCH(1);
+                else if (sk_mt_b == 2) CC_LAUNCH(2);
+                else CC_LAUNCH(4);
+#undef CC_LAUNCH
+            }
+        }
+        }
+        if (t > 0 && !(fuse == 1 && loc)) {
             for (int l = top; l >= 0; --l) {
                 const float *hh = l == 0 ? dxh_t + Dv : g->dxu[l - 1] + (long)t * B * 2 * H + H;
                 rc = cell_bwd(l, t - 1, dq_pre_t, hh, l == 0 ? XH : 2L * H, t);
@@ -1999,6 +2226,6 @@
         ASRK_LAUNCH_CHECK();
     }
     asrk_prof_end_(PROF_SPELLER, s);
-    asrk_prof_launches_(PROF_SPELLER, (5L + 2 * (NL - 1) + (NH > 1)) * L - 1);
+    asrk_prof_launches_(PROF_SPELLER, nlaunch - 1);
     return ASRK_OK;
 }
diff --git a/end-to-end-asr-pytorch_amd/speller_ops.py b/end-to-end-asr-pytorch_amd/speller_ops.py
--- a/end-to-end-asr-pytorch_amd/speller_ops.py
+++ b/end-to-end-asr-pytorch_amd/speller_ops.py
@@ -30,7 +30,8 @@
                                      "dWc_part", "dc")]
                 + [("tc", c_int)]
                 + [(n, c_vp * 2) for n in ("WuT", "dxu", "dcu")]
-                + [("WmT", c_vp), ("dctxh", c_vp)])
+                + [("WmT", c_vp), ("dctxh", c_vp)]
+                + [("tickets", c_vp), ("no_fuse", c_int)])
 
 
 def _ptr(t):
@@ -38,6 +39,8 @@
 
 
 MAX_LOOP_LAYERS = 3
+BWD_NO_FUSE = 0
+_bwd_probe = None
 
 
 def supported_train_loop(attention, decoder, training):
@@ -217,11 +220,12 @@
         dxu = [torch.empty((L, B, 2 * H), **f) for _ in range(nu)]
         dcu = [torch.empty((B, H), **f) for _ in range(nu)]
         dkey = ops.zeros((BN, Te, A), dev)
-        dwe_part = dWp_part = dbe_part = dWc_part = None
+        dwe_part = dWp_part = dbe_part = dWc_part = tickets = None
         if not dot:
             dwe_part = ops.zeros((B * tc, A), dev)
             dWp_part = ops.zeros((B * tc, A * K), dev)
-            dbe_part = ops.zeros((B * tc,), dev)
+            dbe_buf = ops.zeros((B * tc + B,), dev)
+            dbe_part, tickets = dbe_buf[:B * tc], dbe_buf[B * tc:].view(torch.int32)
             dWc_part = ops.zeros((B, K * KW), dev)
         dxh = torch.empty((L, B, XH), **f)
         dq_pre = torch.empty((L, B, NA), **f)
@@ -231,7 +235,15 @@
                         _ptr(dwe_part), _ptr(dWp_part), _ptr(dbe_part), _ptr(dWc_part), _ptr(scratch[4]), tc)
         _set_slots(g.WuT, WuT); _set_slots(g.dxu, dxu); _set_slots(g.dcu, dcu)
         g.WmT, g.dctxh = _ptr(WmT), _ptr(dctxh)
-        _lib.check(lib.asrk_speller_bwd_f32(ctypes.byref(d), ctypes.byref(g), _stream()), "speller_bwd")
+        g.tickets, g.no_fuse = _ptr(tickets), int(BWD_NO_FUSE)
+
+        def run():
+            _lib.check(lib.asrk_speller_bwd_f32(ctypes.byref(d), ctypes.byref(g), _stream()), "speller_bwd")
+        if _bwd_probe is None:
+            run()
+        else:
+            _bwd_probe(run, dict(gates=gates, dkey=dkey, dxh=dxh, dq_pre=dq_pre, tickets=tickets, dwe_part=dwe_part,
+                                 dWp_part=dWp_part, dbe_part=dbe_part, dWc_part=dWc_part))
         dG = gates.view(L * B, 4 * H)
         LB = L * B
 
diff --git a/include/asrk.h b/include/asrk.h
--- a/include/asrk.h
+++ b/include/asrk.h
@@ -211,10 +211,13 @@
     float *dxu[2], *dcu[2];
     const float *WmT;
     float *dctxh;
+    int32_t *tickets;
+    int no_fuse;
 } asrk_speller_bwd_t;
 
 int asrk_speller_plan(const asrk_speller_t *dims, int *tc_fwd, int *tc_bwd);
 int asrk_speller_plan_info(const asrk_speller_t *dims, int *info);
+int asrk_speller_bwd_plan_info(const asrk_speller_t *dims, int *info);
 int asrk_speller_fwd_f32(const asrk_speller_t *p, void *stream);
 int asrk_speller_bwd_f32(const asrk_speller_t *p, const asrk_speller_bwd_t *g, void *stream);
 int asrk_speller_step_f32(const asrk_speller_t *p, int slot, const float *prev_att, int64_t prev_ld,
```
